# ActiveVisionLab/NeFeS

Hardware: AMD Instinct MI355X
Metric: rays/s (fwd+bwd) at 640x480x(64+128) samples, 8x256 MLP (higher is better)
Workload: dtype f32; 1 GPU; BASELINE configs[1]: 7-Scenes-stairs geometry, 64+128 samples, 8x256 MLP + 16-ch feature head; 640x480, random seed-0 weights, fwd + bwd to the 3x4 pose; parallelism=rows/1

## Files before the change

include/nefes_hip.h:

```cpp
#ifndef NEFES_HIP_H
#define NEFES_HIP_H
#include <stddef.h>
#include <stdint.h>

#ifdef __cplusplus
extern "C" {
#endif

#define NEFES_ABI_VERSION 15

#define NEFES_E_BADARG (-1)
#define NEFES_E_UNSUPPORTED (-2)
#define NEFES_E_BADBLOB (-3)

typedef struct NefesNetDesc {
    int32_t width;
    int32_t feat_dim;
    int32_t has_transient;
    int32_t xyz_encoding;
} NefesNetDesc;
#define NEFES_XYZ_FREQ10 0
#define NEFES_XYZ_EXTERNAL32 1

typedef struct NefesStreamInfo {
    uint64_t slab_off;
    uint32_t n_slabs;
    uint32_t bias_floats;
    uint64_t bias_off;
    uint32_t scale_off;
    uint32_t scale_count;
} NefesStreamInfo;

typedef struct NefesBlobInfo {
    uint64_t total_bytes;
    NefesStreamInfo stream[13];
} NefesBlobInfo;

#define NEFES_COMP_TRANSIENT 1u
#define NEFES_COMP_STATIC_ONLY 2u
#define NEFES_COMP_SIGMA_ONLY 4u
#define NEFES_COMP_WHITE_BKGD 8u
#define NEFES_COMP_FEAT_WEIGHTS_ONLY 16u

#define NEFES_FIELD_SIGMA 0
#define NEFES_FIELD_STATIC 1
#define NEFES_FIELD_FULL 2

int nefes_version(void);

int nefes_blob_info(const NefesNetDesc* desc, NefesBlobInfo* info);
size_t nefes_stream_slab_bytes(const NefesNetDesc* desc, int stream);
int nefes_pack_weights(const NefesNetDesc* desc, const float* const* tensors, int n_tensors, void* blob,
// ... 194 lines not shown
```

nefes_amd/csrc/field_bwd_h3.hip:

```cpp
#if defined(NEFES_TU_PART) && NEFES_TU_PART >= 2 && NEFES_TU_PART % 2 == 0
#define NEFES_SLAB_KIB 16
#define NEFES_ASM_READS_ACC
#define NEFES_ACC_VGPR_FORM
#define NEFES_FENCE_TILES
#else
#define NEFES_SLAB_KIB 32
#if !defined(NEFES_TU_PART) || NEFES_TU_PART == 0 || NEFES_TU_PART == 1 || NEFES_TU_PART == 5
#define H3B_WIDE
#define H3_ACC_READ_ASM
#define NEFES_ASM_READS_ACC
#define NEFES_FENCE_TILES
#define H3_WIDE_ENTRY_FENCE
#else
#define NEFES_H3_WIDE_MIN 99
#endif
#endif
#define NEFES_B_BATCH 2
#define NEFES_B_BATCH_NT8 4
#include "field_common.h"
#include "field_x6.h"
#include "field_h3.h"
#include "hashgrid.h"
#include "../../include/nefes_hip.h"
#define NEFES_XYZ_HASHGRID_FUSED 2
// ... 33 lines not shown
};

template <class Inner>
struct StoringSplitH {
    Inner in;
    float* p;
    float inv;
    __device__ __forceinline__ void stage_a(PairRegs& s, int q, int pp) const {
        in.stage_a(s, q, pp);
        const int e = 8 * q + 2 * pp;
#ifndef NEFES_TRAIN_NO_STORES
        __builtin_nontemporal_store(s.x0 * inv, &p[(e >> 4) * 4096 + nefes_rho(0, e & 15) * 16]);
        __builtin_nontemporal_store(s.x1 * inv, &p[((e + 1) >> 4) * 4096 + nefes_rho(0, (e + 1) & 15) * 16]);
#endif
    }
    __device__ __forceinline__ void stage_b(PairRegs& s) const { in.stage_b(s); }
    template <bool NOP>
    __device__ __forceinline__ void stage_c(Split2& o, int pp, const PairRegs& s) const { in.template stage_c<NOP>(o, pp, s); }
    __device__ __forceinline__ void stage_c1(Split2& o, int pp, const PairRegs& s) const { in.stage_c1(o, pp, s); }
    template <bool NOP>
    __device__ __forceinline__ void stage_c2(Split2& o, int pp, const PairRegs& s) const { in.template stage_c2<NOP>(o, pp, s); }
};
template <bool ON, class Inner>
__device__ __forceinline__ auto wrap_store_h3(const Inner& in, float* p, float inv) {
    if constexpr (ON) return StoringSplitH<Inner>{in, p, inv};
    else return in;
}

template <typename T>
__device__ __forceinline__ T ld_stream(const T* p) {
    return __builtin_nontemporal_load(p);
}

template <int W, int KR16, int ENC, bool HAS_T = true, bool TRAIN = false, bool FH = false>
__global__ __launch_bounds__(256, NEFES_H3B_WG_PER_CU(W)) void field_bwd_h3_kernel(FieldBwdH3Args a) {
    constexpr int NTW = W / 32, NTH = W / 64, HS = W / 2, GS = W / 4;
    constexpr int MW = 8 * (W / 64) + 4 * (W / 128);
    constexpr int WT = (NTW + 1) / 2, WH = (NTH + 1) / 2;
    constexpr int MW_TRUNK = 8 * WT;
    constexpr int NTR = KR16 <= 2 ? 1 : 5;
    constexpr int WIDE_LAYERS = ENC == NEFES_XYZ_HASHGRID_FUSED ? 0 : H3B_WIDE_LAYERS;
    static_assert(KR16 == 2 || KR16 == 9, "head classes of layout.h (nefes_head_kr16 / nefes_head_ntr)");
    const int C3 = 3 + a.C;
    static_assert(MW % 4 == 0, "mask words are staged as 16-byte groups");
    extern __shared__ __attribute__((aligned(16))) char smem[];
    const int lane = threadIdx.x & 63;
    const int wave = __builtin_amdgcn_readfirstlane(threadIdx.x >> 6);
    const int j = lane & 31, h = lane >> 5;
    constexpr int SX = ENC == NEFES_XYZ_HASHGRID_FUSED ? 24 : 8;
    int* tab_i = (int*)(smem + NEFES_H3B_SLOTS * NEFES_SLAB_BYTES + (size_t)4 * (MW + SX) * 256);
    const float* tab_f = (const float*)tab_i;
    if (threadIdx.x < 2 * (HAS_T ? NEFES_H3B_N : NEFES_H3B_N_STATIC)) tab_i[threadIdx.x] = a.tab[threadIdx.x];
    HgGeom* hg_lds = (HgGeom*)(tab_i + 64);
    if constexpr (ENC == NEFES_XYZ_HASHGRID_FUSED) {
        if (threadIdx.x == 0) *hg_lds = a.hg;
    }
    auto wexp = [&](int seg) { return tab_i[nefes_h3_tab_exp(nefes_h3b_seg(HAS_T, seg))]; };
    auto rowb = [&](int seg) { return tab_f[nefes_h3_tab_bound(nefes_h3b_seg(HAS_T, seg))]; };
    StagedRing ring;
    ring.init(a.stream, a.n_slabs, smem, wave, lane);
    const char* ring_lane = smem + lane * 16;
    ring.prime(ring_lane);
    uint32_t* mlds = (uint32_t*)(smem + NEFES_H3B_SLOTS * NEFES_SLAB_BYTES) + wave * ((MW + SX) * 64) + lane * 4;
    auto MASKW = [&](int w) { return mlds[(w >> 2) * 256 + (w & 3)]; };
    float* stash = (float*)mlds;
    auto STASH = [&](int k) -> float& { return stash[((MW + k) >> 2) * 256 + ((MW + k) & 3)]; };

#pragma unroll 1
    for (int tile = blockIdx.x; tile < a.n_tiles; tile += gridDim.x) {
        const long long m_raw = (long long)tile * 128 + wave * 32 + j;
        const bool valid = m_raw < a.M;
        const long long m = valid ? m_raw : a.M - 1;
        const int ray = (int)(m / a.S);
        const int smp = (int)(m - (long long)ray * a.S);
        const size_t chan0 = (size_t)ray * a.R * a.S + smp;

        float in_o[3] = {0.f, 0.f, 0.f}, in_d[3] = {0.f, 0.f, 0.f}, in_z = 0.f, v[3];
        if constexpr (ENC == NEFES_XYZ_EXTERNAL32) {
        } else if (a.pts) {
#pragma unroll
            for (int c = 0; c < 3; ++c) in_o[c] = a.pts[m * 3 + c];
        } else {
            in_z = a.z[m];
#pragma unroll
            for (int c = 0; c < 3; ++c) { in_o[c] = a.rays_o[ray * 3 + c]; in_d[c] = a.rays_d[ray * 3 + c]; }
        }
#pragma unroll
        for (int c = 0; c < 3; ++c) v[c] = a.viewdirs[ray * 3 + c];
        const int cT = C3 + 1;
        float y_th[3] = {0.f, 0.f, 0.f}, g_th[3] = {0.f, 0.f, 0.f}, y_sg, g_sg, dr[8 * KR16];
        if constexpr (HAS_T) {
// ... 123 lines not shown
            M_dg = pair_max(array_max(tmp));
        }
        int es_g2;
        {
            const int ew = wexp(NEFES_H3B_RGB), tau = tau_of(M_dr, ew);
            es_g2 = tau + ew;
            mma_run_h3<NTH, KR16, 0, true>(ring, ring_lane, ArraySplitH<8 * KR16>{dr, pow2i(tau)}, ZeroInit{}, G2);
        }
        const float M_g2 = rowb(NEFES_H3B_RGB) * M_dr + M_dg;
        float M = 0.f;
        int es3 = 0;
        if constexpr (HAS_T) {
        mma_run<NTH, 3, 0, true>(ring, ring_lane, ArrayIn<3>{dth}, ZeroInit{}, T3);
        M = rowb(NEFES_H3B_TH) * pair_max(array_max(dth));
        int es4;
        {
            load_bits(bh, MW_TRUNK + 3 * WH, WH);
            const int ew = wexp(NEFES_H3B_T2), tau = tau_of(M, ew);
            float mx = 0.f;
            es4 = tau + ew;
            mma_run_h3<NTH, GS / 8, 0, true>(ring, ring_lane, wrap_store_h3<TRAIN>(MaskedSplitH<NTH, WH, 0>{T3, bh, pow2i(tau), mx}, gptr(NEFES_TB_T2), 1.f), ZeroInit{}, T4);
            M = rowb(NEFES_H3B_T2) * pair_max(mx);
        }
        {
            load_bits(bh, MW_TRUNK + 2 * WH, WH);
            const int ew = wexp(NEFES_H3B_T1), tau = tau_of(M, ew);
            float mx = 0.f;
            es3 = tau + ew;
            mma_run_h3<NTH, GS / 8, 0, true>(ring, ring_lane, wrap_store_h3<TRAIN>(MaskedSplitH<NTH, WH, 0>{T4, bh, pow2i(tau - es4), mx}, gptr(NEFES_TB_T1), pow2i(-es4)), ZeroInit{}, T3);
            M = rowb(NEFES_H3B_T1) * (pair_max(mx) * pow2i(-es4));
        }
        }
        f32x16 XA[NTW + 2], XB[NTW + 2];
        int es_dt;
        {
            const int ew = wexp(NEFES_H3B_DIR);
            const int tau = tau_of(HAS_T ? fmaxf(M, M_g2) : M_g2, ew);
            float mt = 0.f, mg = 0.f;
            es_dt = tau + ew;
            float dgv[FH ? 16 * NTH : 1];
            load_dg(dgv);
            if constexpr (HAS_T) {
                load_bits(bh, MW_TRUNK + WH, WH);
                mma_run_h3<NTW + 1, GS / 8, 1, true>(ring, ring_lane, wrap_store_h3<TRAIN>(MaskedSplitH<NTH, WH, 0>{T3, bh, pow2i(tau - es3), mt}, gptr(NEFES_TB_T0), pow2i(-es3)), ZeroInit{}, XA);
            }
            load_bits(bh, MW_TRUNK, WH);
#ifdef NEFES_FH_VARIANT_VALU_UPDATE
            if constexpr (FH) {
#pragma unroll
                for (int e = 0; e < 16 * NTH; ++e) G2[e >> 4][e & 15] += dgv[e] * pow2i(es_g2);
                mma_run_h3<NTW + 1, GS / 8, 1, !HAS_T>(ring, ring_lane, MaskedSplitH<NTH, WH, 0>{G2, bh, pow2i(tau - es_g2), mg}, ZeroInit{}, XA);
            } else
#else
            if constexpr (FH)
                mma_run_h3<NTW + 1, GS / 8, 1, !HAS_T>(ring, ring_lane, MaskedAddSplitH<NTH, WH, 0, 16 * NTH>{G2, bh, pow2i(tau - es_g2), mg, dgv, pow2i(es_g2)}, ZeroInit{}, XA);
            else
#endif
            mma_run_h3<NTW + 1, GS / 8, 1, !HAS_T>(ring, ring_lane, wrap_store_h3<TRAIN>(MaskedSplitH<NTH, WH, 0>{G2, bh, pow2i(tau - es_g2), mg}, gptr(NEFES_TB_DIR), pow2i(-es_g2)), ZeroInit{}, XA);
            M = (HAS_T ? rowb(NEFES_H3B_T0) * (pair_max(mt) * pow2i(-es3)) : 0.f) + rowb(NEFES_H3B_DIR) * (pair_max(mg) * pow2i(-es_g2));
        }
        float gv[3];
        {
            float dDv[16], v3[3];
            const float inv = pow2i(-es_dt);
#pragma unroll
            for (int r = 0; r < 16; ++r) dDv[r] = XA[1][r] * inv;
#pragma unroll
            for (int c = 0; c < 3; ++c) v3[c] = STASH(3 + c);
            embed_slots_bwd<NEFES_N_FREQ_DIR>(gv, dDv, v3, h);
            if constexpr (ENC == NEFES_XYZ_HASHGRID_FUSED) {
#pragma unroll
                for (int c = 0; c < 3; ++c) STASH(3 + c) = gv[c];
            }
        }
        int es_b;
        {
            const int ew = wexp(NEFES_H3B_FINAL), tau = tau_of(M, ew);
            float mx = 0.f;
            es_b = tau + ew;
            mma_run_h3<NTW, W / 16, 2, true, 2, (WIDE_LAYERS & 1) != 0>(ring, ring_lane, wrap_store_h3<TRAIN>(IdentSplitH<NTW + 2, 2>{XA, pow2i(tau - es_dt), mx}, gptr(NEFES_TB_FINAL), pow2i(-es_dt)), ZeroInit{}, XB);
            const float dsig = STASH(6);
            float dsg[1];
            dsg[0] = dsig * pow2i(es_b);
#if defined(H3B_WIDE) && defined(H3_WIDE_ENTRY_FENCE)
            mma_run<NTW, 1, 2, false, ((WIDE_LAYERS >> 8) & 1) == 0 || (NTW < NEFES_H3_WIDE_MIN)>(ring, ring_lane, ArrayIn<1>{dsg}, ZeroInit{}, XB);
#else
            mma_run<NTW, 1, 2, false>(ring, ring_lane, ArrayIn<1>{dsg}, ZeroInit{}, XB);
#endif
            M = rowb(NEFES_H3B_FINAL) * (pair_max(mx) * pow2i(-es_dt)) + rowb(NEFES_H3B_SIG) * pair_max(fabsf(dsig));
        }
        int es_a = 0, es_e = 0;
#define NEFES_BWD_LAYER(L, SRC, DST, ES_SRC, ES_DST, NTILES, T0)                                                       \
        {                                                                                                           \
            load_bits(bt, ((L) - 1) * WT, WT);                                                                      \
            const int ew = wexp(NEFES_H3B_L8 + 8 - (L)), tau = tau_of(M, ew);                                       \
            float mx = 0.f;                                                                                         \
            ES_DST = tau + ew;                                                                                      \
            mma_run_h3<NTILES, W / 16, T0, true, 2, ((WIDE_LAYERS >> (L)) & 1) != 0>(ring, ring_lane, wrap_store_h3<TRAIN>(MaskedSplitH<NTW + 2, WT, 2>{SRC, bt, pow2i(tau - ES_SRC), mx}, gptr(NEFES_TB_L1 + (L) - 1), pow2i(-(ES_SRC))), ZeroInit{}, DST); \
            M = rowb(NEFES_H3B_L8 + 8 - (L)) * (pair_max(mx) * pow2i(-(ES_SRC)));                                   \
        }
        NEFES_BWD_LAYER(8, XB, XA, es_b, es_a, NTW, 2)
        NEFES_BWD_LAYER(7, XA, XB, es_a, es_b, NTW, 2)
        NEFES_BWD_LAYER(6, XB, XA, es_b, es_a, NTW, 2)
        NEFES_BWD_LAYER(5, XA, XB, es_a, es_b, NTW + 2, 0)
        es_e = es_b;
        float gx[3] = {0.f, 0.f, 0.f};
        float ge[ENC != NEFES_XYZ_FREQ10 ? NEFES_X_STEPS : 1];
        {
            const float inv = pow2i(-es_e);
// ... 42 lines not shown
                float* gp = a.g_enc + m * 32 + h;
#pragma unroll
                for (int s_ = 0; s_ < NEFES_X_STEPS; ++s_) gp[2 * s_] = ge[s_];
            }
        } else {
            float dE[32], x3[3], g1[3];
#pragma unroll
            for (int t = 0; t < 2; ++t)
#pragma unroll
                for (int r = 0; r < 16; ++r) dE[t * 16 + r] = XB[t][r] * inv1;
#pragma unroll
            for (int c = 0; c < 3; ++c) x3[c] = STASH(c);
            embed_slots_bwd<NEFES_N_FREQ_XYZ>(g1, dE, x3, h);
#pragma unroll
            for (int c = 0; c < 3; ++c) gx[c] += g1[c];
        }
#pragma unroll
        for (int c = 0; c < 3; ++c) {
            gx[c] += __shfl_xor(gx[c], 32);
            gv[c] += __shfl_xor(gv[c], 32);
        }
        if (valid && h == 0) {
#pragma unroll
            for (int c = 0; c < 3; ++c) {
                if (ENC != NEFES_XYZ_EXTERNAL32) a.g_pts[m * 3 + c] = gx[c];
                a.g_vs[m * 3 + c] = gv[c];
            }
        }
    }
    ring.drain();
}

template <int W, int KR16, int ENC, bool HAS_T = true, bool TRAIN = false, bool FH = false>
static int launch_bwd_h3(const FieldBwdH3Args& a, hipStream_t st) {
    const size_t lds = (size_t)NEFES_H3B_SLOTS * NEFES_SLAB_BYTES
                       + (size_t)4 * (8 * (W / 64) + 4 * (W / 128) + (ENC == NEFES_XYZ_HASHGRID_FUSED ? 24 : 8)) * 256 + 256
                       + (ENC == NEFES_XYZ_HASHGRID_FUSED ? 512 : 0);
    static_assert(sizeof(HgGeom) <= 512 && 2 * NEFES_H3B_N <= 64, "scale table (256 bytes) + the level geometry's LDS slot");
    auto k = field_bwd_h3_kernel<W, KR16, ENC, HAS_T, TRAIN, FH>;
    hipError_t e = hipFuncSetAttribute((const void*)k, hipFuncAttributeMaxDynamicSharedMemorySize, (int)lds);
    if (e != hipSuccess) return (int)e;
    int dev = 0, cus = 256;
    (void)hipGetDevice(&dev);
    (void)hipDeviceGetAttribute(&cus, hipDeviceAttributeMultiprocessorCount, dev);
    const int slots = cus * NEFES_H3B_WG_PER_CU(W);
    int grid = a.n_tiles < slots ? a.n_tiles : slots;
    if (grid < 1) grid = 1;
    hipLaunchKernelGGL(k, dim3(grid), dim3(256), lds, st, a);
    return (int)hipGetLastError();
}

#ifndef NEFES_TU_PART
#define NEFES_TU_PART 0
#endif
enum { BWD_H3_EXT = 0, BWD_H3_FULL, BWD_H3_TRAIN_STATIC, BWD_H3_TRAIN_FULL, BWD_H3_STATIC, BWD_H3_HG, BWD_H3_FH, BWD_H3_TRAIN_EXT_STATIC,
       BWD_H3_TRAIN_EXT_FULL };
int nefes_bwd_h3_launch_part1(int which, const FieldBwdH3Args& a, hipStream_t st);
int nefes_bwd_h3_launch_part2(int which, const FieldBwdH3Args& a, hipStream_t st);
int nefes_bwd_h3_launch_part3(int which, const FieldBwdH3Args& a, hipStream_t st);
int nefes_bwd_h3_launch_part4(int which, const FieldBwdH3Args& a, hipStream_t st);
int nefes_bwd_h3_launch_part5(int which, const FieldBwdH3Args& a, hipStream_t st);
int nefes_bwd_h3_launch_part6(int which, const FieldBwdH3Args& a, hipStream_t st);
int nefes_bwd_h3_launch_part7(int which, const FieldBwdH3Args& a, hipStream_t st);
int nefes_bwd_h3_launch_part8(int which, const FieldBwdH3Args& a, hipStream_t st);

#if NEFES_TU_PART == 1
int nefes_bwd_h3_launch_part1(int which, const FieldBwdH3Args& a, hipStream_t st) {
    if (which == BWD_H3_EXT) return launch_bwd_h3<256, 2, NEFES_XYZ_EXTERNAL32>(a, st);
    if (which == BWD_H3_STATIC) return launch_bwd_h3<256, 2, NEFES_XYZ_FREQ10, false>(a, st);
    if (which == BWD_H3_HG) return launch_bwd_h3<256, 2, NEFES_XYZ_HASHGRID_FUSED>(a, st);
    return NEFES_E_UNSUPPORTED;
}
#elif NEFES_TU_PART == 2
int nefes_bwd_h3_launch_part2(int which, const FieldBwdH3Args& a, hipStream_t st) {
    if (which == BWD_H3_FULL) return launch_bwd_h3<128, 9, NEFES_XYZ_FREQ10>(a, st);
    if (which == BWD_H3_STATIC) return launch_bwd_h3<128, 9, NEFES_XYZ_FREQ10, false>(a, st);
    return NEFES_E_UNSUPPORTED;
}
#elif NEFES_TU_PART == 3
int nefes_bwd_h3_launch_part3(int which, const FieldBwdH3Args& a, hipStream_t st) {
    if (which == BWD_H3_TRAIN_STATIC) return launch_bwd_h3<256, 2, NEFES_XYZ_FREQ10, false, true>(a, st);
    if (which == BWD_H3_TRAIN_FULL) return launch_bwd_h3<256, 2, NEFES_XYZ_FREQ10, true, true>(a, st);
    if (which == BWD_H3_TRAIN_EXT_STATIC) return launch_bwd_h3<256, 2, NEFES_XYZ_EXTERNAL32, false, true>(a, st);
    if (which == BWD_H3_TRAIN_EXT_FULL) return launch_bwd_h3<256, 2, NEFES_XYZ_EXTERNAL32, true, true>(a, st);
    return NEFES_E_UNSUPPORTED;
}
#elif NEFES_TU_PART == 4
int nefes_bwd_h3_launch_part4(int which, const FieldBwdH3Args& a, hipStream_t st) {
    if (which == BWD_H3_TRAIN_STATIC) return launch_bwd_h3<128, 9, NEFES_XYZ_FREQ10, false, true>(a, st);
    if (which == BWD_H3_TRAIN_FULL) return launch_bwd_h3<128, 9, NEFES_XYZ_FREQ10, true, true>(a, st);
    return NEFES_E_UNSUPPORTED;
}
#elif NEFES_TU_PART == 5
int nefes_bwd_h3_launch_part5(int which, const FieldBwdH3Args& a, hipStream_t st) {
    if (which == BWD_H3_FULL) return launch_bwd_h3<256, 9, NEFES_XYZ_FREQ10>(a, st);
    if (which == BWD_H3_STATIC) return launch_bwd_h3<256, 9, NEFES_XYZ_FREQ10, false>(a, st);
    return NEFES_E_UNSUPPORTED;
}
#elif NEFES_TU_PART == 6
int nefes_bwd_h3_launch_part6(int which, const FieldBwdH3Args& a, hipStream_t st) {
    if (which == BWD_H3_FULL) return launch_bwd_h3<128, 2, NEFES_XYZ_FREQ10>(a, st);
    if (which == BWD_H3_STATIC) return launch_bwd_h3<128, 2, NEFES_XYZ_FREQ10, false>(a, st);
    if (which == BWD_H3_FH) return launch_bwd_h3<128, 2, NEFES_XYZ_FREQ10, true, false, true>(a, st);
    return NEFES_E_UNSUPPORTED;
}
#elif NEFES_TU_PART == 7
int nefes_bwd_h3_launch_part7(int which, const FieldBwdH3Args& a, hipStream_t st) {
    if (which == BWD_H3_TRAIN_STATIC) return launch_bwd_h3<256, 9, NEFES_XYZ_FREQ10, false, true>(a, st);
    if (which == BWD_H3_TRAIN_FULL) return launch_bwd_h3<256, 9, NEFES_XYZ_FREQ10, true, true>(a, st);
    return NEFES_E_UNSUPPORTED;
}
#elif NEFES_TU_PART == 8
int nefes_bwd_h3_launch_part8(int which, const FieldBwdH3Args& a, hipStream_t st) {
    if (which == BWD_H3_TRAIN_STATIC) return launch_bwd_h3<128, 2, NEFES_XYZ_FREQ10, false, true>(a, st);
    if (which == BWD_H3_TRAIN_FULL) return launch_bwd_h3<128, 2, NEFES_XYZ_FREQ10, true, true>(a, st);
    return NEFES_E_UNSUPPORTED;
}
#else

extern "C" int nefes_field_bwd_train_h3(const NefesNetDesc* desc, const void* packed, int mode, int N, int S, const float* rays_o,
                                        const float* rays_d, const float* z, const float* viewdirs, const float* raw_t,
                                        const float* g_raw_t, const uint32_t* masks, float* dacts, float* g_pts,
                                        float* g_viewdirs_s, void* stream) {
    if (!desc || !packed || !viewdirs || !raw_t || !g_raw_t || !masks || !dacts || !g_pts || !g_viewdirs_s || N <= 0 || S <= 0)
        return NEFES_E_BADARG;
    if (!(rays_o && rays_d && z)) return NEFES_E_BADARG;
    if (mode != NEFES_FIELD_STATIC && mode != NEFES_FIELD_FULL) return NEFES_E_BADARG;
    const bool full = mode == NEFES_FIELD_FULL;
    if (full && !desc->has_transient) return NEFES_E_UNSUPPORTED;
    const int cls = nefes_head_class(desc->feat_dim);
    if ((desc->width != 256 && desc->width != 128) || cls < 0 || desc->xyz_encoding != NEFES_XYZ_FREQ10) return NEFES_E_UNSUPPORTED;
    NefesBlobInfo info;
    int rc = nefes_blob_info(desc, &info);
    if (rc) return rc;
    const NefesStreamInfo& si = info.stream[full ? NEFES_STREAM_BWD_FULL_H3 : NEFES_STREAM_BWD_STATIC_H3];
    if (si.n_slabs == 0 || si.scale_count < 2 * (uint32_t)(full ? NEFES_H3B_N : NEFES_H3B_N_STATIC)) return NEFES_E_UNSUPPORTED;
    FieldBwdH3Args a;
    a.stream = (const char*)packed + si.slab_off;
    a.tab = (const int*)((const char*)packed + si.bias_off) + si.scale_off;
    a.n_slabs = si.n_slabs;
    a.rays_o = rays_o; a.rays_d = rays_d; a.z = z; a.pts = nullptr; a.viewdirs = viewdirs;
    a.raw_t = raw_t; a.g_raw_t = g_raw_t; a.masks = masks; a.g_pts = g_pts; a.g_enc = nullptr; a.g_vs = g_viewdirs_s;
    a.N = N; a.S = S; a.C = desc->feat_dim; a.R = 3 + a.C + (full ? 6 : 1);
    a.M = (long long)N * S;
    a.n_tiles = (int)((a.M + 127) / 128);
    a.dacts = dacts; a.gout = 0; a.hg_table = nullptr; a.g_gmap = nullptr;
    a.rows = nefes_train_row(desc->width, desc->feat_dim, NEFES_TB_END);
    const int which = full ? BWD_H3_TRAIN_FULL : BWD_H3_TRAIN_STATIC;
    hipStream_t st = (hipStream_t)stream;
    if (desc->width == 256) return cls == 0 ? nefes_bwd_h3_launch_part3(which, a, st) : nefes_bwd_h3_launch_part7(which, a, st);
    return cls == 1 ? nefes_bwd_h3_launch_part4(which, a, st) : nefes_bwd_h3_launch_part8(which, a, st);
}

extern "C" int nefes_field_bwd_train_h3_ext(const NefesNetDesc* desc, const void* packed, int mode, int N, int S, const float* viewdirs,
                                            const float* raw_t, const float* g_raw_t, const uint32_t* masks, float* dacts,
                                            float* g_xyz_enc, float* g_viewdirs_s, void* stream) {
    if (!desc || !packed || !viewdirs || !raw_t || !g_raw_t || !masks || !dacts || !g_xyz_enc || !g_viewdirs_s || N <= 0 || S <= 0)
        return NEFES_E_BADARG;
    if (mode != NEFES_FIELD_STATIC && mode != NEFES_FIELD_FULL) return NEFES_E_BADARG;
    const bool full = mode == NEFES_FIELD_FULL;
    if (full && !desc->has_transient) return NEFES_E_UNSUPPORTED;
    if (desc->width != 256 || nefes_head_class(desc->feat_dim) != 0 || desc->xyz_encoding != NEFES_XYZ_EXTERNAL32) return NEFES_E_UNSUPPORTED;
    NefesBlobInfo info;
    int rc = nefes_blob_info(desc, &info);
    if (rc) return rc;
    const NefesStreamInfo& si = info.stream[full ? NEFES_STREAM_BWD_FULL_H3 : NEFES_STREAM_BWD_STATIC_H3];
    if (si.n_slabs == 0 || si.scale_count < 2 * (uint32_t)(full ? NEFES_H3B_N : NEFES_H3B_N_STATIC)) return NEFES_E_UNSUPPORTED;
    FieldBwdH3Args a;
    a.stream = (const char*)packed + si.slab_off;
    a.tab = (const int*)((const char*)packed + si.bias_off) + si.scale_off;
    a.n_slabs = si.n_slabs;
    a.rays_o = nullptr; a.rays_d = nullptr; a.z = nullptr; a.pts = nullptr; a.viewdirs = viewdirs;
    a.raw_t = raw_t; a.g_raw_t = g_raw_t; a.masks = masks; a.g_pts = nullptr; a.g_enc = g_xyz_enc; a.g_vs = g_viewdirs_s;
    a.N = N; a.S = S; a.C = desc->feat_dim; a.R = 3 + a.C + (full ? 6 : 1);
    a.M = (long long)N * S;
    a.n_tiles = (int)((a.M + 127) / 128);
    a.dacts = dacts; a.gout = 0; a.hg_table = nullptr; a.g_gmap = nullptr;
    a.rows = nefes_train_row(desc->width, desc->feat_dim, NEFES_TB_END);
    return nefes_bwd_h3_launch_part3(full ? BWD_H3_TRAIN_EXT_FULL : BWD_H3_TRAIN_EXT_STATIC, a, (hipStream_t)stream);
}

extern "C" int nefes_field_bwd_static_h3(const NefesNetDesc* desc, const void* packed, int N, int S, const float* rays_o,
                                         const float* rays_d, const float* z, const float* pts, const float* viewdirs,
                                         const float* raw_t, const float* g_raw_t, const uint32_t* masks, float* g_pts,
                                         float* g_viewdirs_s, void* stream) {
    if (!desc || !packed || !viewdirs || !raw_t || !g_raw_t || !masks || !g_pts || !g_viewdirs_s || N <= 0 || S <= 0)
        return NEFES_E_BADARG;
    if (!pts && !(rays_o && rays_d && z)) return NEFES_E_BADARG;
    const int cls = nefes_head_class(desc->feat_dim);
    if ((desc->width != 256 && desc->width != 128) || cls < 0 || desc->xyz_encoding != NEFES_XYZ_FREQ10) return NEFES_E_UNSUPPORTED;
    NefesBlobInfo info;
    int rc = nefes_blob_info(desc, &info);
    if (rc) return rc;
    const NefesStreamInfo& si = info.stream[NEFES_STREAM_BWD_STATIC_H3];
    if (si.n_slabs == 0 || si.scale_count < 2 * (uint32_t)NEFES_H3B_N_STATIC) return NEFES_E_UNSUPPORTED;
    FieldBwdH3Args a;
    a.stream = (const char*)packed + si.slab_off;
    a.tab = (const int*)((const char*)packed + si.bias_off) + si.scale_off;
    a.n_slabs = si.n_slabs;
    a.rays_o = rays_o; a.rays_d = rays_d; a.z = z; a.pts = pts; a.viewdirs = viewdirs;
    a.raw_t = raw_t; a.g_raw_t = g_raw_t; a.masks = masks; a.g_pts = g_pts; a.g_enc = nullptr; a.g_vs = g_viewdirs_s;
    a.N = N; a.S = S; a.C = desc->feat_dim; a.R = 3 + a.C + 1;
    a.M = (long long)N * S;
    a.n_tiles = (int)((a.M + 127) / 128);
    a.dacts = nullptr; a.rows = 0; a.gout = 0; a.hg_table = nullptr; a.g_gmap = nullptr;
    hipStream_t st = (hipStream_t)stream;
    if (desc->width == 256) return cls == 0 ? nefes_bwd_h3_launch_part1(BWD_H3_STATIC, a, st) : nefes_bwd_h3_launch_part5(BWD_H3_STATIC, a, st);
    return cls == 1 ? nefes_bwd_h3_launch_part2(BWD_H3_STATIC, a, st) : nefes_bwd_h3_launch_part6(BWD_H3_STATIC, a, st);
}

static int field_bwd_h3_impl(const NefesNetDesc* desc, const void* packed, int N, int S, const float* rays_o,
                                  const float* rays_d, const float* z, const float* pts, const float* viewdirs,
                                  const float* raw_t, const float* g_raw_t, const uint32_t* masks, float* g_pts,
                                  float* g_xyz_enc, float* g_viewdirs_s, void* stream, const NefesHashGridDesc* grid, const float* table,
                                  bool fh = false, const float* g_gmap = nullptr) {
    if (!desc || !packed || !viewdirs || !raw_t || !g_raw_t || !masks || !g_viewdirs_s || N <= 0 || S <= 0)
        return NEFES_E_BADARG;
    const bool ext = desc->xyz_encoding == NEFES_XYZ_EXTERNAL32;
    const bool fused_grid = ext && table != nullptr;
    if (fused_grid ? !(g_pts && grid && rays_o && rays_d && z) : (ext ? !g_xyz_enc : (!g_pts || (!pts && !(rays_o && rays_d && z))))) return NEFES_E_BADARG;
    if (!desc->has_transient) return NEFES_E_UNSUPPORTED;
    NefesBlobInfo info;
    int rc = nefes_blob_info(desc, &info);
    if (rc) return rc;
    const NefesStreamInfo& si = info.stream[NEFES_STREAM_BWD_FULL_H3];
    if (si.n_slabs == 0 || si.scale_count < 2 * NEFES_H3B_N) return NEFES_E_UNSUPPORTED;
    FieldBwdH3Args a;
    a.stream = (const char*)packed + si.slab_off;
    a.tab = (const int*)((const char*)packed + si.bias_off) + si.scale_off;
    a.n_slabs = si.n_slabs;
    a.rays_o = rays_o; a.rays_d = rays_d; a.z = z; a.pts = pts; a.viewdirs = viewdirs;
    a.raw_t = raw_t; a.g_raw_t = g_raw_t; a.masks = masks; a.g_pts = g_pts; a.g_enc = g_xyz_enc; a.g_vs = g_viewdirs_s;
    a.N = N; a.S = S; a.C = desc->feat_dim; a.R = 3 + a.C + 6;
    a.gout = 0; a.g_gmap = g_gmap;
    if (fh) {
        if (desc->feat_dim != 0 || desc->width != 128 || ext) return NEFES_E_UNSUPPORTED;
        a.gout = desc->width / 2;
        a.C = a.gout + 1;
        a.R = 3 + a.C + 6;
    }
    a.M = (long long)N * S;
    a.n_tiles = (int)((a.M + 127) / 128);
    a.dacts = nullptr; a.rows = 0;
    a.hg_table = (const float2*)table;
    if (fused_grid) {
        rc = hg_geometry(grid, &a.hg, nullptr);
        if (rc) return rc;
        if (a.hg.n_levels != 16) return NEFES_E_UNSUPPORTED;
    }
    hipStream_t st = (hipStream_t)stream;
    const int cls = nefes_head_class(desc->feat_dim);
    if (cls < 0) return NEFES_E_UNSUPPORTED;
    if (fh) return nefes_bwd_h3_launch_part6(BWD_H3_FH, a, st);
    if (desc->width == 256 && fused_grid) return cls == 0 ? nefes_bwd_h3_launch_part1(BWD_H3_HG, a, st) : NEFES_E_UNSUPPORTED;
    if (desc->width == 256 && ext) return cls == 0 ? nefes_bwd_h3_launch_part1(BWD_H3_EXT, a, st) : NEFES_E_UNSUPPORTED;
    if (desc->width == 256) return cls == 0 ? launch_bwd_h3<256, 2, NEFES_XYZ_FREQ10>(a, st) : nefes_bwd_h3_launch_part5(BWD_H3_FULL, a, st);
    if (desc->width == 128 && !ext) return cls == 1 ? nefes_bwd_h3_launch_part2(BWD_H3_FULL, a, st) : nefes_bwd_h3_launch_part6(BWD_H3_FULL, a, st);
    return NEFES_E_UNSUPPORTED;
}

extern "C" int nefes_field_bwd_h3(const NefesNetDesc* desc, const void* packed, int N, int S, const float* rays_o,
                                  const float* rays_d, const float* z, const float* pts, const float* viewdirs,
                                  const float* raw_t, const float* g_raw_t, const uint32_t* masks, float* g_pts,
                                  float* g_xyz_enc, float* g_viewdirs_s, void* stream) {
    return field_bwd_h3_impl(desc, packed, N, S, rays_o, rays_d, z, pts, viewdirs, raw_t, g_raw_t, masks, g_pts, g_xyz_enc, g_viewdirs_s, stream,
                             nullptr, nullptr);
}

extern "C" int nefes_field_bwd_h3_fh(const NefesNetDesc* desc, const void* packed, int N, int S, const float* rays_o, const float* rays_d,
                                     const float* z, const float* viewdirs, const float* raw_t, const float* g_raw_t, const float* g_gmap,
                                     const uint32_t* masks, float* g_pts, float* g_viewdirs_s, void* stream) {
    if (!rays_o || !rays_d || !z) return NEFES_E_BADARG;
    return field_bwd_h3_impl(desc, packed, N, S, rays_o, rays_d, z, nullptr, viewdirs, raw_t, g_raw_t, masks, g_pts, nullptr, g_viewdirs_s, stream,
                             nullptr, nullptr, true, g_gmap);
}

extern "C" int nefes_field_bwd_h3_hashgrid(const NefesNetDesc* desc, const void* packed, const NefesHashGridDesc* grid,
                                           const float* table, int N, int S, const float* rays_o, const float* rays_d, const float* z,
                                           const float* viewdirs, const float* raw_t, const float* g_raw_t, const uint32_t* masks,
                                           float* g_pts, float* g_viewdirs_s, void* stream) {
    if (!desc || desc->xyz_encoding != NEFES_XYZ_EXTERNAL32 || !grid || !table) return NEFES_E_BADARG;
    return field_bwd_h3_impl(desc, packed, N, S, rays_o, rays_d, z, nullptr, viewdirs, raw_t, g_raw_t, masks, g_pts, nullptr, g_viewdirs_s, stream,
                             grid, table);
}
#endif
```

nefes_amd/csrc/field_fwd_h3.hip:

```cpp
#if defined(NEFES_TU_PART) && NEFES_TU_PART >= 2 && NEFES_TU_PART % 2 == 0
#define NEFES_TU_W128
#define NEFES_SLAB_KIB 16
#else
#define NEFES_SLAB_KIB 32
#endif
#include <stdlib.h>
#if defined(NEFES_TU_W128) || !defined(H3_NO_ACC_READ_ASM)
#define NEFES_ASM_READS_ACC
#define NEFES_FENCE_TILES
#endif
#if defined(NEFES_TU_W128)
#define NEFES_ACC_VGPR_FORM
#endif

#ifndef NEFES_FWD_CONSUMER_BIAS
#define NEFES_FWD_CONSUMER_BIAS 1
#endif
#include "field_common.h"
#include "../../include/nefes_hip.h"

#include "field_x6.h"
#include "hashgrid.h"
#define NEFES_XYZ_HASHGRID_FUSED 2
#if !defined(NEFES_TU_W128) && !defined(H3_NO_ACC_READ_ASM)
// ... 9 lines not shown
    const float* rays_o;
    const float* rays_d;
    const float* z;
    const float* pts;
    const float* xyz_enc;
    const float* viewdirs;
    float* raw_t;
    uint32_t* masks;
    int N, S, R, C;
    long long M;
    int n_tiles;
    uint32_t s_magic, s_shift;
    float* acts;
    int rows;
    int z_row;
    const float2* hg_table;
    HgGeom hg;
    int gout;
};

template <int NT, int T0, int NX>
__device__ __forceinline__ void train_save_h3(float* tile_base, uint32_t voff, int row0, const f32x16 (&X)[NX], float inv) {
    float* p = tile_base + (size_t)(row0 >> 5) * 4096 + voff;
#pragma unroll
    for (int t = 0; t < NT; ++t)
#pragma unroll
        for (int r = 0; r < 16; ++r) {
#ifndef NEFES_TRAIN_NO_STORES
            __builtin_nontemporal_store(X[T0 + t][r] * inv, &p[t * 4096 + nefes_rho(0, r) * 16]);
#endif
        }
}

template <int MODE, int ENC, int W = 256, int NTR = 1, bool TRAIN = false, bool FH = false>
__global__ __launch_bounds__(256, W == 128 ? 2 : 1) void field_fwd_h3_kernel(FieldFwdH3Args a) {
    static_assert(NEFES_SLAB_KIB == (W == 128 ? NEFES_H3_FWD_SLAB_KIB_128 : NEFES_H3_FWD_SLAB_KIB), "ring slab size != the packer's for this width");
    constexpr int NTW = W / 32, NTH = W / 64;
    constexpr int ES = ENC != NEFES_XYZ_FREQ10 ? NEFES_X_STEPS : NEFES_E_STEPS;
    constexpr int MW = 8 * (W / 64) + 4 * (W / 128), WT = (NTW + 1) / 2, WH = (NTH + 1) / 2;
    constexpr int NSEG = MODE == NEFES_FIELD_SIGMA ? NEFES_H3F_SIG + 1 : (MODE == NEFES_FIELD_STATIC ? NEFES_H3F_N_STATIC : NEFES_H3F_N);
    extern __shared__ __attribute__((aligned(16))) char smem[];
    char* ring_base = smem;
    float* bias_lds = (float*)(smem + NEFES_H3_SLOTS * NEFES_SLAB_BYTES);
    float* e_lds = bias_lds + ((a.bias_floats + 63) / 64) * 64 + (threadIdx.x >> 6) * (ES * 64) + (threadIdx.x & 63);
    const int lane = threadIdx.x & 63;
    const int wave = __builtin_amdgcn_readfirstlane(threadIdx.x >> 6);
    const int j = lane & 31, h = lane >> 5;
    for (uint32_t i = threadIdx.x; i < a.bias_floats; i += 256) bias_lds[i] = a.bias[i];
    HgGeom* hg_lds = (HgGeom*)(bias_lds + ((a.bias_floats + 63) / 64) * 64 + 4 * ES * 64);
    if constexpr (ENC == NEFES_XYZ_HASHGRID_FUSED) {
        if (threadIdx.x == 0) *hg_lds = a.hg;
    }
    StagedRing ring;
    ring.init(a.stream, a.n_slabs, ring_base, wave, lane);
    const char* ring_lane = ring_base + lane * 16;
    const char* bias_half = (const char*)bias_lds + 16 * h;
    const int* tab_i = (const int*)(bias_lds + a.scale_off);
    const float* tab_f = bias_lds + a.scale_off;
    auto wexp = [&](int seg) { return tab_i[nefes_h3_tab_exp(seg)]; };
    auto rowb = [&](int seg) { return tab_f[nefes_h3_tab_bound(seg)]; };
    auto bmax = [&](int blk) { return tab_f[nefes_h3_tab_bias(NSEG, blk)]; };
    ring.prime(ring_lane);
    constexpr int B_SIG = 8 * W, B_FINAL = B_SIG + 32, B_DIR = B_FINAL + W, B_RGB = B_DIR + W / 2,
                  B_T0 = B_RGB + 32 * NTR, B_T1 = B_T0 + W / 2, B_T2 = B_T1 + W / 2, B_TH = B_T2 + W / 2;
#pragma unroll 1
    for (int tile = blockIdx.x; tile < a.n_tiles; tile += gridDim.x) {
        auto locate = [&](uint32_t& m, uint32_t& ray, uint32_t& smp) {
            const uint32_t m_raw = (uint32_t)tile * 128u + (uint32_t)(wave * 32 + j);
            const bool ok = m_raw < (uint32_t)a.M;
            m = ok ? m_raw : (uint32_t)a.M - 1u;
            ray = a.s_magic ? __umulhi(m, a.s_magic) >> a.s_shift : m;
            smp = m - ray * (uint32_t)a.S;
            return ok;
        };
        uint32_t m, ray, smp;
        locate(m, ray, smp);
        float in_o[3] = {0.f, 0.f, 0.f}, in_d[3] = {0.f, 0.f, 0.f}, in_z = 0.f;
        float E[ES];
        if constexpr (ENC == NEFES_XYZ_EXTERNAL32) {
#pragma unroll
            for (int s = 0; s < ES; ++s) E[s] = a.xyz_enc[(size_t)m * 32 + 2 * s + h];
        } else if (ENC != NEFES_XYZ_HASHGRID_FUSED && a.pts) {
#pragma unroll
            for (int c = 0; c < 3; ++c) in_o[c] = a.pts[(size_t)m * 3 + c];
        } else {
            in_z = a.z[a.z_row ? smp : m];
#pragma unroll
            for (int c = 0; c < 3; ++c) { in_o[c] = a.rays_o[ray * 3 + c]; in_d[c] = a.rays_d[ray * 3 + c]; }
        }
        float mE;
        if constexpr (ENC == NEFES_XYZ_EXTERNAL32) {
            mE = pair_max(array_max(E));
        } else if constexpr (ENC == NEFES_XYZ_HASHGRID_FUSED) {
            float x[3];
#pragma unroll
            for (int c = 0; c < 3; ++c) x[c] = add_rn(in_o[c], mul_rn(in_d[c], in_z));
// ... 63 lines not shown
                const int ch = (MODE == NEFES_FIELD_SIGMA) ? 0 : 3 + a.C;
                __builtin_nontemporal_store(softplus_ref(sg[0][0] * pow2i(-es)), &col[(size_t)ch * a.S]);
            }
        };
        int es_a, es_b = 0;
        float M;
        {
            const int tau = tau_of(mE, wexp(NEFES_H3F_L1));
            es_a = tau + wexp(NEFES_H3F_L1);
            if constexpr (CB) mma_run_h3<NTW, ES / 8, 0, true>(ring, ring_lane, LdsSplitH{e_lds, pow2i(tau)}, ZeroInit{}, A);
            else mma_run_h3<NTW, ES / 8, 0, true>(ring, ring_lane, LdsSplitH{e_lds, pow2i(tau)}, bias_at(0, es_a), A);
            M = rowb(NEFES_H3F_L1) * mE + bmax(NEFES_H3BB_L1);
            save_trunk(1, A, es_a);
        }
#define NEFES_FWD_EVEN_LAYER(L1_, SEG1_)                                                                                       \
        clear_bits();                                                                                                          \
        {                                                                                                                      \
            const int ew = wexp(SEG1_), tau = tau_of(M, ew);                                                                   \
            const float rb_ = rowb(SEG1_), bm_ = bmax((L1_) - 1);           \
            float mx = 0.f;                                                                                                    \
            if constexpr (CB) {                                                                                                \
                const char* bps = bias_half + ((L1_) - 2) * W * 4;                           \
                nbias = ReluBiasSplitH<CAP, NTW, WT>::prime(bps);                                                              \
                mma_run_h3<NTW, W / 16, 0, true>(ring, ring_lane, ReluBiasSplitH<CAP, NTW, WT>{A, bits, pow2i(tau - es_a), mx, bps, pow2i(es_a), nbias}, \
                                                 ZeroInit{}, B);                                                               \
            } else                                                                                                             \
            mma_run_h3<NTW, W / 16, 0, true>(ring, ring_lane, ReluSplitH<CAP, NTW, WT>{A, bits, pow2i(tau - es_a), mx},        \
                                             bias_at(((L1_) - 1) * W, tau + ew), B);                                           \
            M = rb_ * (pair_max(mx) * pow2i(-es_a)) + bm_;                                                                     \
            es_b = tau + ew;                                                                                                   \
            save_trunk(L1_, B, es_b);                                                                                          \
        }                                                                                                                      \
        put_masks(bits, WT);
        constexpr int NPAIRS = MODE == NEFES_FIELD_SIGMA ? 3 : 4;
#pragma unroll 1
        for (int p = 0; p < NPAIRS; ++p) {
            const int l1 = 2 + 2 * p, l2 = l1 + 1;
            const int seg1 = l1 <= 5 ? l1 - 1 : l1;
            const int seg2 = l2 <= 5 ? l2 - 1 : (l2 <= 8 ? l2 : NEFES_H3F_FINAL);
            NEFES_FWD_EVEN_LAYER(l1, seg1)
            clear_bits();
            {
                const int ew = wexp(seg2);
                const int tau = tau_of(p == 1 ? fmaxf(M, mE) : M, ew);
                if (p == 3) sigma_head(B, es_b, tau_of(M, wexp(NEFES_H3F_SIG)));
                const float rb_ = rowb(seg2), bm_ = bmax(l2 <= 8 ? l2 - 1 : NEFES_H3BB_FINAL);
                const float rbe_ = p == 1 ? rowb(NEFES_H3F_L5E) : 0.f;
                float mx = 0.f;
                if constexpr (CB) {
                    const char* bps = bias_half + (l1 - 1) * W * 4;
                    nbias = ReluBiasSplitH<CAP, NTW, WT>::prime(bps);
                    const ReluBiasSplitH<CAP, NTW, WT> src{B, bits, pow2i(tau - es_b), mx, bps, pow2i(es_b), nbias};
                    mma_run_h3<NTW, W / 16, 0, true>(ring, ring_lane, src, ZeroInit{}, A);
                } else
                mma_run_h3<NTW, W / 16, 0, true>(ring, ring_lane, ReluSplitH<CAP, NTW, WT>{B, bits, pow2i(tau - es_b), mx},
                                                 bias_at(l2 <= 8 ? (l2 - 1) * W : B_FINAL, tau + ew), A);
                if (p == 1) mma_run_h3<NTW, ES / 8, 0, false>(ring, ring_lane, LdsSplitH{e_lds, pow2i(tau)}, ZeroInit{}, A);
                M = rb_ * (pair_max(mx) * pow2i(-es_b)) + (p == 1 ? rbe_ * mE : 0.f) + bm_;
                es_a = tau + ew;
                save_trunk(l2, A, es_a);
            }
            put_masks(bits, WT);
        }
        if constexpr (MODE == NEFES_FIELD_SIGMA) { NEFES_FWD_EVEN_LAYER(8, NEFES_H3F_L8) }
#undef NEFES_FWD_EVEN_LAYER
        if constexpr (MODE == NEFES_FIELD_SIGMA) sigma_head(B, es_b, tau_of(M, wexp(NEFES_H3F_SIG)));
        if constexpr (MODE != NEFES_FIELD_SIGMA) {
            constexpr bool FULL = MODE == NEFES_FIELD_FULL;
            constexpr int NDT = FULL ? 2 * NTH : NTH;
            float v[3];
            {
                uint32_t mm, rr, ss;
                locate(mm, rr, ss);
#pragma unroll
                for (int c = 0; c < 3; ++c) v[c] = a.viewdirs[(size_t)rr * 3 + c];
            }
            float Dv[16];
            {
                float d14[NEFES_D_STEPS];
                embed_slots<NEFES_N_FREQ_DIR>(d14, v, h);
#pragma unroll
                for (int s = 0; s < 16; ++s) Dv[s] = s < NEFES_D_STEPS ? d14[s] : 0.f;
            }
            if constexpr (TRAIN) {
                float* pd = act_tile + (size_t)(nefes_train_row(W, 0, NEFES_TB_DV) >> 5) * 4096 + emb_off;
#pragma unroll
                for (int s = 0; s < NEFES_D_STEPS; ++s) __builtin_nontemporal_store(Dv[s], &pd[2 * s * 16]);
            }
            f32x16 dt[NDT];
            uint32_t bits2[WH];
            auto clear2 = [&]() {
#pragma unroll
                for (int w = 0; w < WH; ++w) bits2[w] = 0u;
            };
            struct Bias2 {
                BiasInitScaled a, b;
                __device__ __forceinline__ f32x16 operator()(int t) const { return t < NTH ? a(t) : b(t - NTH); }
            };
            int es_dt;
            {
                const int ew = wexp(NEFES_H3F_DT_H);
                const float mD = pair_max(array_max(Dv));
                const int tau = tau_of(fmaxf(M, mD), ew);
                float mx = 0.f;
                es_dt = tau + ew;
                if constexpr (CB) {
                    const char* bpf = bias_half + B_FINAL * 4;
                    nbias = ReluBiasSplitH<false, 1, 1>::prime(bpf);
                    const IdentBiasSplitH<NTW> srcf{A, pow2i(tau - es_a), mx, bpf, pow2i(es_a), nbias};
                    if constexpr (FULL) mma_run_h3<NDT, W / 16, 0, true>(ring, ring_lane, srcf, Bias2{bias_at(B_DIR, es_dt), bias_at(B_T0, es_dt)}, dt);
                    else mma_run_h3<NDT, W / 16, 0, true>(ring, ring_lane, srcf, bias_at(B_DIR, es_dt), dt);
                } else if constexpr (FULL)
                    mma_run_h3<NDT, W / 16, 0, true>(ring, ring_lane, IdentSplitH<NTW, 0>{A, pow2i(tau - es_a), mx},
                                                     Bias2{bias_at(B_DIR, es_dt), bias_at(B_T0, es_dt)}, dt);
                else
                    mma_run_h3<NDT, W / 16, 0, true>(ring, ring_lane, IdentSplitH<NTW, 0>{A, pow2i(tau - es_a), mx}, bias_at(B_DIR, es_dt), dt);
                mma_run_h3<NDT, 2, 0, false>(ring, ring_lane, ArraySplitH<16>{Dv, pow2i(tau)}, ZeroInit{}, dt);
                M = rowb(NEFES_H3F_DT_H) * (pair_max(mx) * pow2i(-es_a)) + rowb(NEFES_H3F_DT_D) * mD
                    + (FULL ? fmaxf(bmax(NEFES_H3BB_DIR), bmax(NEFES_H3BB_T0)) : bmax(NEFES_H3BB_DIR));
                if constexpr (TRAIN) {
                    train_save_h3<NTH, 0>(act_tile, act_voff, nefes_train_row(W, 0, NEFES_TB_DIR), dt, pow2i(-es_dt));
                    if constexpr (FULL) train_save_h3<NTH, NTH>(act_tile, act_voff, nefes_train_row(W, 0, NEFES_TB_T0), dt, pow2i(-es_dt));
                }
            }
            if constexpr (FH) {
                float* col = raw_col();
                if (col) {
                    int S_g = a.S;
                    asm volatile("" : "+s"(S_g));
                    const float inv = pow2i(-es_dt);
                    float* pg = col + (size_t)(3 + 4 * h) * S_g;
#pragma unroll
                    for (int t = 0; t < NTH; ++t)
#pragma unroll
                        for (int r = 0; r < 16; ++r)
                            __builtin_nontemporal_store(fmaxf(dt[t][r] * inv, 0.f), &pg[(size_t)(32 * t + nefes_rho(0, r)) * S_g]);
                    if (h == 0) __builtin_nontemporal_store(1.f, &col[(size_t)(3 + W / 2) * S_g]);
                }
            }
            {
                f32x16 ar[NTR];
                clear2();
                const int ew = wexp(NEFES_H3F_RGB), tau = tau_of(M, ew), es = tau + ew;
                float mdummy = 0.f;
                mma_run_h3<NTR, W / 32, 0, true>(ring, ring_lane, ReluSplitH<true, NDT, WH>{dt, bits2, pow2i(tau - es_dt), mdummy},
                                                 bias_at(B_RGB, es), ar);
                put_masks(bits2, WH);
                float* col = raw_col();
                if (col) {
                    float* ph = col + (size_t)(4 * h) * a.S;
                    const float inv = pow2i(-es);
// ... 39 lines not shown
                                                 bias_at(B_T2, es2), acc2);
                M = rowb(NEFES_H3F_T2) * (pair_max(mx) * pow2i(-es3)) + bmax(NEFES_H3BB_T2);
                if constexpr (TRAIN) train_save_h3<NTH, 0>(act_tile, act_voff, nefes_train_row(W, 0, NEFES_TB_T2), acc2, pow2i(-es2));
            }
            put_masks(bits2, WH);
            f32x16 th[1];
            clear2();
            {
                const int ew = wexp(NEFES_H3F_TH), tau = tau_of(M, ew);
                float mdummy = 0.f;
                es_th = tau + ew;
                mma_run_h3<1, W / 32, 0, true>(ring, ring_lane, ReluSplitH<true, NTH, WH>{acc2, bits2, pow2i(tau - es2), mdummy},
                                               bias_at(B_TH, es_th), th);
            }
            put_masks(bits2, WH);
            float* col = raw_col();
            if (col) {
                float* o = col + (size_t)(3 + a.C + 1) * a.S;
                const float inv = pow2i(-es_th);
                if (h == 0) {
                    __builtin_nontemporal_store(sigmoid_ref(th[0][0] * inv), &o[0]);
                    __builtin_nontemporal_store(sigmoid_ref(th[0][1] * inv), &o[(size_t)a.S]);
                    __builtin_nontemporal_store(sigmoid_ref(th[0][2] * inv), &o[(size_t)2 * a.S]);
                    __builtin_nontemporal_store(softplus_ref(th[0][3] * inv), &o[(size_t)3 * a.S]);
                } else {
                    __builtin_nontemporal_store(softplus_ref(th[0][0] * inv), &o[(size_t)4 * a.S]);
                }
            }
            }
        }
    }
}

static void magic_div(uint32_t d, uint32_t& magic, uint32_t& shift) {
    if (d == 1) { magic = 0; shift = 0; return; }
    uint32_t l = 0;
    while ((1ull << l) < d) ++l;
    const uint64_t p = 31 + l;
    magic = (uint32_t)(((1ull << p) + d - 1) / d);
    shift = (uint32_t)(p - 32);
}

template <int MODE, int ENC, int W = 256, int NTR = 1, bool TRAIN = false, bool FH = false>
static int launch_h3(const FieldFwdH3Args& a, hipStream_t st) {
    constexpr int ES_ = ENC != NEFES_XYZ_FREQ10 ? NEFES_X_STEPS : NEFES_E_STEPS;
    const size_t lds = (size_t)NEFES_H3_SLOTS * NEFES_SLAB_BYTES + ((a.bias_floats + 63) / 64) * 256 + (size_t)4 * ES_ * 64 * 4
                       + (ENC == NEFES_XYZ_HASHGRID_FUSED ? 512 : 0);
    static_assert(sizeof(HgGeom) <= 512, "the level geometry's LDS slot");
    auto k = field_fwd_h3_kernel<MODE, ENC, W, NTR, TRAIN, FH>;
    hipError_t e = hipFuncSetAttribute((const void*)k, hipFuncAttributeMaxDynamicSharedMemorySize, (int)lds);
    if (e != hipSuccess) return (int)e;
    int dev = 0, cus = 256;
    (void)hipGetDevice(&dev);
    (void)hipDeviceGetAttribute(&cus, hipDeviceAttributeMultiprocessorCount, dev);
    const int per_cu = W == 128 ? 2 : 1;
    int grid = a.n_tiles < cus * per_cu ? a.n_tiles : cus * per_cu;
    if (const char* cap = getenv("NEFES_DEBUG_MAX_GRID")) {
        const int c = atoi(cap);
        if (c > 0 && c < grid) grid = c;
    }
    hipLaunchKernelGGL(k, dim3(grid), dim3(256), lds, st, a);
    return (int)hipGetLastError();
}

#ifndef NEFES_TU_PART
#define NEFES_TU_PART 0
#endif
enum { H3_EXT_SIGMA = 0, H3_EXT_FULL, H3_SIGMA, H3_FULL, H3_TRAIN_STATIC, H3_TRAIN_FULL, H3_STATIC, H3_HG_SIGMA, H3_HG_FULL, H3_FH_FULL,
       H3_TRAIN_EXT_STATIC, H3_TRAIN_EXT_FULL };
int nefes_fwd_h3_launch_part1(int which, const FieldFwdH3Args& a, hipStream_t st);
int nefes_fwd_h3_launch_part2(int which, const FieldFwdH3Args& a, hipStream_t st);
int nefes_fwd_h3_launch_part3(int which, const FieldFwdH3Args& a, hipStream_t st);
int nefes_fwd_h3_launch_part4(int which, const FieldFwdH3Args& a, hipStream_t st);
int nefes_fwd_h3_launch_part5(int which, const FieldFwdH3Args& a, hipStream_t st);
int nefes_fwd_h3_launch_part6(int which, const FieldFwdH3Args& a, hipStream_t st);
int nefes_fwd_h3_launch_part7(int which, const FieldFwdH3Args& a, hipStream_t st);
int nefes_fwd_h3_launch_part8(int which, const FieldFwdH3Args& a, hipStream_t st);


#if NEFES_TU_PART == 1
int nefes_fwd_h3_launch_part1(int which, const FieldFwdH3Args& a, hipStream_t st) {
    switch (which) {
        case H3_EXT_SIGMA: return launch_h3<NEFES_FIELD_SIGMA, NEFES_XYZ_EXTERNAL32>(a, st);
        case H3_EXT_FULL: return launch_h3<NEFES_FIELD_FULL, NEFES_XYZ_EXTERNAL32>(a, st);
        case H3_STATIC: return launch_h3<NEFES_FIELD_STATIC, NEFES_XYZ_FREQ10, 256, 1>(a, st);
        case H3_HG_SIGMA: return launch_h3<NEFES_FIELD_SIGMA, NEFES_XYZ_HASHGRID_FUSED>(a, st);
        case H3_HG_FULL: return launch_h3<NEFES_FIELD_FULL, NEFES_XYZ_HASHGRID_FUSED>(a, st);
    }
    return NEFES_E_UNSUPPORTED;
}
#elif NEFES_TU_PART == 2
int nefes_fwd_h3_launch_part2(int which, const FieldFwdH3Args& a, hipStream_t st) {
    switch (which) {
        case H3_SIGMA: return launch_h3<NEFES_FIELD_SIGMA, NEFES_XYZ_FREQ10, 128, 5>(a, st);
        case H3_FULL: return launch_h3<NEFES_FIELD_FULL, NEFES_XYZ_FREQ10, 128, 5>(a, st);
        case H3_STATIC: return launch_h3<NEFES_FIELD_STATIC, NEFES_XYZ_FREQ10, 128, 5>(a, st);
    }
    return NEFES_E_UNSUPPORTED;
}
#elif NEFES_TU_PART == 3
int nefes_fwd_h3_launch_part3(int which, const FieldFwdH3Args& a, hipStream_t st) {
    switch (which) {
        case H3_TRAIN_STATIC: return launch_h3<NEFES_FIELD_STATIC, NEFES_XYZ_FREQ10, 256, 1, true>(a, st);
        case H3_TRAIN_FULL: return launch_h3<NEFES_FIELD_FULL, NEFES_XYZ_FREQ10, 256, 1, true>(a, st);
        case H3_TRAIN_EXT_STATIC: return launch_h3<NEFES_FIELD_STATIC, NEFES_XYZ_EXTERNAL32, 256, 1, true>(a, st);
        case H3_TRAIN_EXT_FULL: return launch_h3<NEFES_FIELD_FULL, NEFES_XYZ_EXTERNAL32, 256, 1, true>(a, st);
    }
    return NEFES_E_UNSUPPORTED;
}
#elif NEFES_TU_PART == 4
int nefes_fwd_h3_launch_part4(int which, const FieldFwdH3Args& a, hipStream_t st) {
    switch (which) {
        case H3_TRAIN_STATIC: return launch_h3<NEFES_FIELD_STATIC, NEFES_XYZ_FREQ10, 128, 5, true>(a, st);
        case H3_TRAIN_FULL: return launch_h3<NEFES_FIELD_FULL, NEFES_XYZ_FREQ10, 128, 5, true>(a, st);
    }
    return NEFES_E_UNSUPPORTED;
}
#elif NEFES_TU_PART == 5
int nefes_fwd_h3_launch_part5(int which, const FieldFwdH3Args& a, hipStream_t st) {
    if (which == H3_FULL) return launch_h3<NEFES_FIELD_FULL, NEFES_XYZ_FREQ10, 256, 5>(a, st);
    if (which == H3_STATIC) return launch_h3<NEFES_FIELD_STATIC, NEFES_XYZ_FREQ10, 256, 5>(a, st);
    return NEFES_E_UNSUPPORTED;
}
#elif NEFES_TU_PART == 6
int nefes_fwd_h3_launch_part6(int which, const FieldFwdH3Args& a, hipStream_t st) {
    if (which == H3_FULL) return launch_h3<NEFES_FIELD_FULL, NEFES_XYZ_FREQ10, 128, 1>(a, st);
    if (which == H3_STATIC) return launch_h3<NEFES_FIELD_STATIC, NEFES_XYZ_FREQ10, 128, 1>(a, st);
    if (which == H3_FH_FULL) return launch_h3<NEFES_FIELD_FULL, NEFES_XYZ_FREQ10, 128, 1, false, true>(a, st);
    return NEFES_E_UNSUPPORTED;
}
#elif NEFES_TU_PART == 7
int nefes_fwd_h3_launch_part7(int which, const FieldFwdH3Args& a, hipStream_t st) {
    switch (which) {
        case H3_TRAIN_STATIC: return launch_h3<NEFES_FIELD_STATIC, NEFES_XYZ_FREQ10, 256, 5, true>(a, st);
        case H3_TRAIN_FULL: return launch_h3<NEFES_FIELD_FULL, NEFES_XYZ_FREQ10, 256, 5, true>(a, st);
    }
    return NEFES_E_UNSUPPORTED;
}
#elif NEFES_TU_PART == 8
int nefes_fwd_h3_launch_part8(int which, const FieldFwdH3Args& a, hipStream_t st) {
    switch (which) {
        case H3_TRAIN_STATIC: return launch_h3<NEFES_FIELD_STATIC, NEFES_XYZ_FREQ10, 128, 1, true>(a, st);
        case H3_TRAIN_FULL: return launch_h3<NEFES_FIELD_FULL, NEFES_XYZ_FREQ10, 128, 1, true>(a, st);
    }
    return NEFES_E_UNSUPPORTED;
}
#else

extern "C" int nefes_field_fwd_train_h3(const NefesNetDesc* desc, const void* packed, int mode, int N, int S, const float* rays_o,
                                        const float* rays_d, const float* z, const float* pts, const float* viewdirs,
                                        float* raw_t, float* acts, uint32_t* masks, void* stream) {
    if (!desc || !packed || !raw_t || !acts || !viewdirs || N <= 0 || S <= 0) return NEFES_E_BADARG;
    if (!pts && !(rays_o && rays_d && z)) return NEFES_E_BADARG;
    if (mode != NEFES_FIELD_STATIC && mode != NEFES_FIELD_FULL) return NEFES_E_UNSUPPORTED;
    if (mode == NEFES_FIELD_FULL && !desc->has_transient) return NEFES_E_BADARG;
    const int cls = nefes_head_class(desc->feat_dim);
    if ((desc->width != 256 && desc->width != 128) || cls < 0 || desc->xyz_encoding != NEFES_XYZ_FREQ10) return NEFES_E_UNSUPPORTED;
    NefesBlobInfo info;
    int rc = nefes_blob_info(desc, &info);
    if (rc) return rc;
    const NefesStreamInfo& si = info.stream[mode == NEFES_FIELD_STATIC ? NEFES_STREAM_FWD_STATIC_H3 : NEFES_STREAM_FWD_FULL_H3];
    if (si.n_slabs == 0) return NEFES_E_UNSUPPORTED;
    FieldFwdH3Args a;
    a.stream = (const char*)packed + si.slab_off;
    a.bias = (const float*)((const char*)packed + si.bias_off);
    a.n_slabs = si.n_slabs; a.bias_floats = si.bias_floats; a.scale_off = si.scale_off;
    a.rays_o = rays_o; a.rays_d = rays_d; a.z = z; a.pts = pts; a.xyz_enc = nullptr; a.viewdirs = viewdirs; a.raw_t = raw_t; a.masks = masks;
    a.N = N; a.S = S; a.C = desc->feat_dim; a.R = 3 + a.C + (mode == NEFES_FIELD_STATIC ? 1 : 6);
    a.M = (long long)N * S;
    if (a.M >= (1ll << 31) - 256) return NEFES_E_UNSUPPORTED;
    a.n_tiles = (int)((a.M + 127) / 128);
    a.acts = acts;
    a.rows = nefes_train_row(desc->width, desc->feat_dim, NEFES_TB_END);
    a.z_row = 0; a.gout = 0; a.hg_table = nullptr;
    magic_div((uint32_t)S, a.s_magic, a.s_shift);
    const int which = mode == NEFES_FIELD_STATIC ? H3_TRAIN_STATIC : H3_TRAIN_FULL;
    hipStream_t st = (hipStream_t)stream;
    if (desc->width == 256) return cls == 0 ? nefes_fwd_h3_launch_part3(which, a, st) : nefes_fwd_h3_launch_part7(which, a, st);
    return cls == 1 ? nefes_fwd_h3_launch_part4(which, a, st) : nefes_fwd_h3_launch_part8(which, a, st);
}

extern "C" int nefes_field_fwd_train_h3_ext(const NefesNetDesc* desc, const void* packed, int mode, int N, int S, const float* xyz_enc,
                                            const float* viewdirs, float* raw_t, float* acts, uint32_t* masks, void* stream) {
    if (!desc || !packed || !xyz_enc || !raw_t || !acts || !viewdirs || N <= 0 || S <= 0) return NEFES_E_BADARG;
    if (mode != NEFES_FIELD_STATIC && mode != NEFES_FIELD_FULL) return NEFES_E_UNSUPPORTED;
    if (mode == NEFES_FIELD_FULL && !desc->has_transient) return NEFES_E_BADARG;
    if (desc->width != 256 || nefes_head_class(desc->feat_dim) != 0 || desc->xyz_encoding != NEFES_XYZ_EXTERNAL32) return NEFES_E_UNSUPPORTED;
    NefesBlobInfo info;
    int rc = nefes_blob_info(desc, &info);
    if (rc) return rc;
    const NefesStreamInfo& si = info.stream[mode == NEFES_FIELD_STATIC ? NEFES_STREAM_FWD_STATIC_H3 : NEFES_STREAM_FWD_FULL_H3];
    if (si.n_slabs == 0) return NEFES_E_UNSUPPORTED;
    FieldFwdH3Args a;
    a.stream = (const char*)packed + si.slab_off;
    a.bias = (const float*)((const char*)packed + si.bias_off);
    a.n_slabs = si.n_slabs; a.bias_floats = si.bias_floats; a.scale_off = si.scale_off;
    a.rays_o = nullptr; a.rays_d = nullptr; a.z = nullptr; a.pts = nullptr; a.xyz_enc = xyz_enc; a.viewdirs = viewdirs; a.raw_t = raw_t;
    a.masks = masks;
    a.N = N; a.S = S; a.C = desc->feat_dim; a.R = 3 + a.C + (mode == NEFES_FIELD_STATIC ? 1 : 6);
    a.M = (long long)N * S;
    if (a.M >= (1ll << 31) - 256) return NEFES_E_UNSUPPORTED;
    a.n_tiles = (int)((a.M + 127) / 128);
    a.acts = acts;
    a.rows = nefes_train_row(desc->width, desc->feat_dim, NEFES_TB_END);
    a.z_row = 0; a.gout = 0; a.hg_table = nullptr;
    magic_div((uint32_t)S, a.s_magic, a.s_shift);
    return nefes_fwd_h3_launch_part3(mode == NEFES_FIELD_STATIC ? H3_TRAIN_EXT_STATIC : H3_TRAIN_EXT_FULL, a, (hipStream_t)stream);
}

static int field_fwd_h3_impl(const NefesNetDesc* desc, const void* packed, int mode, int N, int S, const float* rays_o,
                             const float* rays_d, const float* z, int z_row, const float* pts, const float* xyz_enc,
                             const float* viewdirs, float* raw_t, uint32_t* masks, void* stream,
                             const NefesHashGridDesc* grid = nullptr, const float* table = nullptr, bool fh = false) {
    if (!desc || !packed || !raw_t || N <= 0 || S <= 0) return NEFES_E_BADARG;
    const bool ext = desc->xyz_encoding == NEFES_XYZ_EXTERNAL32;
    const bool fused_grid = ext && table != nullptr;
    if (fused_grid ? !(rays_o && rays_d && z && grid) : (ext ? !xyz_enc : (!pts && !(rays_o && rays_d && z)))) return NEFES_E_BADARG;
    if (mode != NEFES_FIELD_SIGMA && mode != NEFES_FIELD_FULL && mode != NEFES_FIELD_STATIC) return NEFES_E_UNSUPPORTED;
// ... 3 lines not shown
    const bool big = desc->width == 256, small = desc->width == 128 && !ext;
    if (!(big || small) || cls < 0 || (ext && cls != 0) || (desc->xyz_encoding != NEFES_XYZ_FREQ10 && !ext)) return NEFES_E_UNSUPPORTED;
    NefesBlobInfo info;
    int rc = nefes_blob_info(desc, &info);
    if (rc) return rc;
    const NefesStreamInfo& si = info.stream[mode == NEFES_FIELD_SIGMA ? NEFES_STREAM_FWD_SIGMA_H3
                                            : (mode == NEFES_FIELD_STATIC ? NEFES_STREAM_FWD_STATIC_H3 : NEFES_STREAM_FWD_FULL_H3)];
    if (si.n_slabs == 0) return NEFES_E_UNSUPPORTED;
    FieldFwdH3Args a;
    a.stream = (const char*)packed + si.slab_off;
    a.bias = (const float*)((const char*)packed + si.bias_off);
    a.n_slabs = si.n_slabs; a.bias_floats = si.bias_floats; a.scale_off = si.scale_off;
    a.rays_o = rays_o; a.rays_d = rays_d; a.z = z; a.pts = pts; a.xyz_enc = xyz_enc; a.viewdirs = viewdirs; a.raw_t = raw_t; a.masks = masks;
    a.acts = nullptr; a.rows = 0; a.z_row = z_row;
    a.hg_table = (const float2*)table;
    if (fused_grid) {
        rc = hg_geometry(grid, &a.hg, nullptr);
        if (rc) return rc;
        if (a.hg.n_levels != 16) return NEFES_E_UNSUPPORTED;
    }
    a.N = N; a.S = S; a.C = desc->feat_dim; a.R = mode == NEFES_FIELD_SIGMA ? 1 : 3 + a.C + (mode == NEFES_FIELD_STATIC ? 1 : 6);
    a.gout = 0;
    if (fh) {
        if (desc->feat_dim != 0 || desc->width != 128 || ext || mode != NEFES_FIELD_FULL) return NEFES_E_UNSUPPORTED;
        a.gout = desc->width / 2;
        a.C = a.gout + 1;
        a.R = 3 + a.C + 6;
    }
    a.M = (long long)N * S;
    if (a.M >= (1ll << 31) - 256) return NEFES_E_UNSUPPORTED;
    a.n_tiles = (int)((a.M + 127) / 128);
    magic_div((uint32_t)S, a.s_magic, a.s_shift);
    hipStream_t st = (hipStream_t)stream;
    if (fh) return nefes_fwd_h3_launch_part6(H3_FH_FULL, a, st);
    if (mode == NEFES_FIELD_STATIC) {
        if (big) return cls == 0 ? nefes_fwd_h3_launch_part1(H3_STATIC, a, st) : nefes_fwd_h3_launch_part5(H3_STATIC, a, st);
        return cls == 1 ? nefes_fwd_h3_launch_part2(H3_STATIC, a, st) : nefes_fwd_h3_launch_part6(H3_STATIC, a, st);
    }
    if (fused_grid) return nefes_fwd_h3_launch_part1(mode == NEFES_FIELD_SIGMA ? H3_HG_SIGMA : H3_HG_FULL, a, st);
    if (ext) return nefes_fwd_h3_launch_part1(mode == NEFES_FIELD_SIGMA ? H3_EXT_SIGMA : H3_EXT_FULL, a, st);
    if (small) {
        if (mode == NEFES_FIELD_SIGMA) return nefes_fwd_h3_launch_part2(H3_SIGMA, a, st);
        return cls == 1 ? nefes_fwd_h3_launch_part2(H3_FULL, a, st) : nefes_fwd_h3_launch_part6(H3_FULL, a, st);
    }
    if (mode == NEFES_FIELD_SIGMA) return launch_h3<NEFES_FIELD_SIGMA, NEFES_XYZ_FREQ10>(a, st);
    return cls == 0 ? launch_h3<NEFES_FIELD_FULL, NEFES_XYZ_FREQ10>(a, st) : nefes_fwd_h3_launch_part5(H3_FULL, a, st);
}

extern "C" int nefes_field_fwd_h3(const NefesNetDesc* desc, const void* packed, int mode, int N, int S, const float* rays_o,
                                  const float* rays_d, const float* z, const float* pts, const float* xyz_enc,
                                  const float* viewdirs, float* raw_t, uint32_t* masks, void* stream) {
    return field_fwd_h3_impl(desc, packed, mode, N, S, rays_o, rays_d, z, 0, pts, xyz_enc, viewdirs, raw_t, masks, stream);
}

extern "C" int nefes_field_fwd_h3_hashgrid(const NefesNetDesc* desc, const void* packed, const NefesHashGridDesc* grid,
                                           const float* table, int mode, int N, int S, const float* rays_o, const float* rays_d,
                                           const float* z, int z_is_row, const float* viewdirs, float* raw_t, uint32_t* masks,
                                           void* stream) {
    if (!desc || desc->xyz_encoding != NEFES_XYZ_EXTERNAL32 || !grid || !table) return NEFES_E_BADARG;
    return field_fwd_h3_impl(desc, packed, mode, N, S, rays_o, rays_d, z, z_is_row ? 1 : 0, nullptr, nullptr, viewdirs, raw_t, masks, stream,
                             grid, table);
}

extern "C" int nefes_field_fwd_h3_fh(const NefesNetDesc* desc, const void* packed, int mode, int N, int S, const float* rays_o,
                                     const float* rays_d, const float* z, const float* viewdirs, float* raw_t, uint32_t* masks,
                                     void* stream) {
    if (!rays_o || !rays_d || !z) return NEFES_E_BADARG;
    return field_fwd_h3_impl(desc, packed, mode, N, S, rays_o, rays_d, z, 0, nullptr, nullptr, viewdirs, raw_t, masks, stream, nullptr, nullptr, true);
}

extern "C" int nefes_field_fwd_h3_zrow(const NefesNetDesc* desc, const void* packed, int mode, int N, int S, const float* rays_o,
                                       const float* rays_d, const float* z_row, const float* viewdirs, float* raw_t, uint32_t* masks,
                                       void* stream) {
    if (!rays_o || !rays_d || !z_row) return NEFES_E_BADARG;
    if (desc && desc->xyz_encoding != NEFES_XYZ_FREQ10) return NEFES_E_UNSUPPORTED;
    return field_fwd_h3_impl(desc, packed, mode, N, S, rays_o, rays_d, z_row, 1, nullptr, nullptr, viewdirs, raw_t, masks, stream);
}
#endif
```

nefes_amd/csrc/layout.h:

```cpp
#pragma once
#include <stdint.h>

#if defined(__HIP__)
#define NEFES_HD __host__ __device__ inline __attribute__((always_inline))
#else
#define NEFES_HD inline
#endif

#ifndef NEFES_FWD_SLAB_KIB
#define NEFES_FWD_SLAB_KIB 32
#endif
#ifndef NEFES_BWD_SLAB_KIB
#define NEFES_BWD_SLAB_KIB 32
#endif
#define NEFES_FRAGS_OF_KIB(kib) ((kib) * 4)
#define NEFES_SLAB_BYTES (NEFES_SLAB_KIB * 1024)
#define NEFES_SLAB_FRAGS NEFES_FRAGS_OF_KIB(NEFES_SLAB_KIB)
#define NEFES_SLAB_PIECES (NEFES_SLAB_BYTES / 4096)
#define NEFES_RING_SLOTS (128 / NEFES_FWD_SLAB_KIB)
#define NEFES_BWD_SLOTS (96 / NEFES_BWD_SLAB_KIB)
#define NEFES_N_FREQ_XYZ 10
#define NEFES_N_FREQ_DIR 4
#define NEFES_E_STEPS 32
#define NEFES_D_STEPS 14
// ... 23 lines not shown
       NEFES_STREAM_FWD_SIGMA_X6 = 4, NEFES_STREAM_FWD_FULL_X6 = 5, NEFES_STREAM_BWD_FULL_X6 = 6, NEFES_STREAM_BWD_STATIC = 7,
       NEFES_STREAM_FWD_SIGMA_H3 = 8, NEFES_STREAM_FWD_FULL_H3 = 9, NEFES_STREAM_BWD_FULL_H3 = 10,
       NEFES_STREAM_FWD_STATIC_H3 = 11, NEFES_STREAM_BWD_STATIC_H3 = 12,
       NEFES_N_STREAMS = 13 };
#define NEFES_X6_SLAB_KIB 48
#define NEFES_H3_FWD_SLAB_KIB 32
#define NEFES_H3_FWD_SLAB_KIB_128 16
#define NEFES_H3_BWD_SLAB_KIB 32
#define NEFES_H3_BWD_SLAB_KIB_128 16
#define NEFES_H3_TARGET_EXP 14
NEFES_HD int nefes_stream_slab_kib(int stream, int width) {
    if (stream == NEFES_STREAM_BWD_FULL || stream == NEFES_STREAM_BWD_FULL_X6 || stream == NEFES_STREAM_BWD_STATIC) return NEFES_BWD_SLAB_KIB;
    if (stream == NEFES_STREAM_BWD_FULL_H3 || stream == NEFES_STREAM_BWD_STATIC_H3) return width == 128 ? NEFES_H3_BWD_SLAB_KIB_128 : NEFES_H3_BWD_SLAB_KIB;
    if (stream == NEFES_STREAM_FWD_SIGMA_H3 || stream == NEFES_STREAM_FWD_FULL_H3 || stream == NEFES_STREAM_FWD_STATIC_H3)
        return width == 128 ? NEFES_H3_FWD_SLAB_KIB_128 : NEFES_H3_FWD_SLAB_KIB;
    return stream >= NEFES_STREAM_FWD_SIGMA_X6 ? NEFES_X6_SLAB_KIB : NEFES_FWD_SLAB_KIB;
}
#define NEFES_PACK_KEEP 0xffffffffu
#define NEFES_BLOB_HEADER_BYTES 512

enum { NEFES_H3F_L1 = 0, NEFES_H3F_L2, NEFES_H3F_L3, NEFES_H3F_L4, NEFES_H3F_L5H, NEFES_H3F_L5E, NEFES_H3F_L6, NEFES_H3F_L7,
       NEFES_H3F_L8, NEFES_H3F_SIG, NEFES_H3F_FINAL, NEFES_H3F_DT_H, NEFES_H3F_DT_D, NEFES_H3F_RGB, NEFES_H3F_T1, NEFES_H3F_T2,
       NEFES_H3F_TH, NEFES_H3F_N };
NEFES_HD int nefes_h3_tab_exp(int seg) { return 2 * seg; }
NEFES_HD int nefes_h3_tab_bound(int seg) { return 2 * seg + 1; }
NEFES_HD int nefes_h3_tab_bias(int n_segs, int block) { return 2 * n_segs + block; }
enum { NEFES_H3BB_L1 = 0, NEFES_H3BB_SIG = 8, NEFES_H3BB_FINAL, NEFES_H3BB_DIR, NEFES_H3BB_RGB, NEFES_H3BB_T0, NEFES_H3BB_T1,
       NEFES_H3BB_T2, NEFES_H3BB_TH };
enum { NEFES_H3B_RGB = 0, NEFES_H3B_TH, NEFES_H3B_T2, NEFES_H3B_T1, NEFES_H3B_T0, NEFES_H3B_DIR, NEFES_H3B_FINAL, NEFES_H3B_SIG,
       NEFES_H3B_L8, NEFES_H3B_L7, NEFES_H3B_L6, NEFES_H3B_L5, NEFES_H3B_L4, NEFES_H3B_L3, NEFES_H3B_L2, NEFES_H3B_L1,
       NEFES_H3B_N };
#define NEFES_H3F_N_STATIC (NEFES_H3F_RGB + 1)
#define NEFES_H3B_N_STATIC (NEFES_H3B_N - 4)
NEFES_HD int nefes_h3b_seg(int has_transient, int seg) { return (has_transient || seg == NEFES_H3B_RGB) ? seg : seg - 4; }

NEFES_HD int nefes_mask_words(int W) { return 8 * (W / 64) + 4 * (W / 128); }

enum { NEFES_TB_E = 0, NEFES_TB_DV = 1, NEFES_TB_L1 = 2 , NEFES_TB_FINAL = 10, NEFES_TB_DIR = 11,
       NEFES_TB_T0 = 12, NEFES_TB_T1 = 13, NEFES_TB_T2 = 14, NEFES_TB_RGB = 15, NEFES_TB_SIG = 16, NEFES_TB_TH = 17,
       NEFES_TB_END = 18 };
NEFES_HD size_t nefes_train_off(int row, int sample) {
    return ((size_t)(row >> 5) * 8 + (size_t)(sample >> 4)) * 512 + (size_t)(row & 31) * 16 + (size_t)(sample & 15);
}
NEFES_HD uint32_t nefes_train_lane_off(int wave, int j, int h) { return (uint32_t)(((wave * 32 + j) >> 4) * 512 + 4 * h * 16 + (j & 15)); }
NEFES_HD int nefes_train_row(int W, int C, int block) {
    const int ntr = nefes_head_ntr(C);
    int r = 0;
    if (block == NEFES_TB_E) return r;
    r += 2 * NEFES_E_STEPS;
    if (block == NEFES_TB_DV) return r;
    r += 32;
    if (block >= NEFES_TB_L1 && block <= NEFES_TB_FINAL) return r + (block - NEFES_TB_L1) * W;
    r += 9 * W;
    if (block >= NEFES_TB_DIR && block <= NEFES_TB_T2) return r + (block - NEFES_TB_DIR) * (W / 2);
    r += 4 * (W / 2);
    if (block == NEFES_TB_RGB) return r;
    r += 32 * ntr;
    if (block == NEFES_TB_SIG) return r;
    r += 32;
    if (block == NEFES_TB_TH) return r;
    return r + 32;
}
```

nefes_amd/csrc/pack.cpp:

```cpp
#include <math.h>
#include <string.h>

#include <vector>

#include "../../include/nefes_hip.h"
#include "layout.h"

namespace {

enum { L_XYZ1 = 0, L_FINAL = 8, L_DIR = 9, L_SIGMA = 10, L_RGB = 11, L_T0 = 12, L_T1 = 13, L_T2 = 14, L_TSIGMA = 15,
       L_TRGB = 16, L_TBETA = 17 };

struct Seg {
    int nt = 0, ks = 0;
    std::vector<int> kidx;
    std::vector<int> ridx;
    const float* W = nullptr;
    int ld = 0;
    bool transposed = false;
    bool x6 = false;
    bool h3 = false;
    int wexp = 0;
    float at(int s, int t, int lane) const {
        const int i = lane & 31, h = lane >> 5;
// ... 120 lines not shown
    return k;
}
std::vector<int> k_emb(int L, int ks, int base) {
    std::vector<int> k(ks * 2);
    for (int s = 0; s < ks; ++s)
        for (int h = 0; h < 2; ++h) {
            const int e = nefes_emb_slot(L, s, h);
            k[s * 2 + h] = e < 0 ? -1 : base + e;
        }
    return k;
}
std::vector<int> k_compact(int ks, int limit) {
    std::vector<int> k(ks * 2);
    for (int i = 0; i < ks * 2; ++i) k[i] = i < limit ? i : -1;
    return k;
}
std::vector<int> rows_emb(int L, int ntiles, int base) {
    std::vector<int> r(ntiles * 32);
    for (int t = 0; t < ntiles; ++t)
        for (int i = 0; i < 32; ++i) {
            const int e = nefes_emb_slot(L, 16 * t + nefes_row_reg(i), nefes_row_half(i));
            r[t * 32 + i] = e < 0 ? -1 : base + e;
        }
    return r;
}
std::vector<int> concat(std::vector<int> a, const std::vector<int>& b) {
    a.insert(a.end(), b.begin(), b.end());
    return a;
}

struct Net {
    int W, W2, C, NTW, NTH, NTR;
    bool transient;
    bool ext;
    int in_xyz, e_steps;
    const float* const* t;
    std::vector<float> th_w, th_b;
    std::vector<float> dt_w;
    const float* w(int l) const { return t[2 * l]; }
    const float* b(int l) const { return t[2 * l + 1]; }
};

Seg seg(int nt, int ks, std::vector<int> kidx, std::vector<int> ridx, const float* W, int ld, bool tr = false) {
    Seg s;
    s.nt = nt; s.ks = ks; s.kidx = std::move(kidx); s.ridx = std::move(ridx); s.W = W; s.ld = ld; s.transposed = tr;
    return s;
}

std::vector<int> k_xyz(const Net& n, int base) {
    return n.ext ? [&] { auto k = k_compact(n.e_steps, n.in_xyz); for (auto& v : k) if (v >= 0) v += base; return k; }()
                 : k_emb(10, n.e_steps, base);
}
std::vector<int> rows_xyz(const Net& n, int base) {
    if (!n.ext) return rows_emb(10, 2, base);
    std::vector<int> r(64, -1);
    for (int i = 0; i < 32; ++i) r[i] = base + 2 * nefes_row_reg(i) + nefes_row_half(i);
    return r;
}

static void mark(Seg& s, int kind) {
    s.x6 = kind != 0;
    s.h3 = kind == 2;
}

void add_trunk(const Net& n, Stream& st, int x6 = 0) {
    const int W = n.W, NT = n.NTW;
// ... 2 lines not shown
            st.segs.push_back(seg(NT, n.e_steps, k_xyz(n, 0), rows_natural(NT, W), n.w(0), n.in_xyz));
            mark(st.segs.back(), x6);
        } else if (l == 4) {
            st.segs.push_back(seg(NT, W / 2, k_natural(W / 2, n.in_xyz), rows_natural(NT, W), n.w(4), n.in_xyz + W));
            mark(st.segs.back(), x6);
            st.segs.push_back(seg(NT, n.e_steps, k_xyz(n, 0), rows_natural(NT, W), n.w(4), n.in_xyz + W));
            mark(st.segs.back(), x6);
        } else {
            st.segs.push_back(seg(NT, W / 2, k_natural(W / 2, 0), rows_natural(NT, W), n.w(l), W));
            mark(st.segs.back(), x6);
        }
        st.bias.push_back({n.b(l), rows_natural(NT, W)});
    }
    st.segs.push_back(seg(1, W / 2, k_natural(W / 2, 0), rows_natural(1, 1), n.w(L_SIGMA), W));
    mark(st.segs.back(), x6);
    st.bias.push_back({n.b(L_SIGMA), rows_natural(1, 1)});
}

void add_static_head(const Net& n, Stream& st, int x6 = 0) {
    const int W = n.W, W2 = n.W2;
    st.segs.push_back(seg(n.NTW, W / 2, k_natural(W / 2, 0), rows_natural(n.NTW, W), n.w(L_FINAL), W));
    mark(st.segs.back(), x6);
    st.bias.push_back({n.b(L_FINAL), rows_natural(n.NTW, W)});
    st.segs.push_back(seg(n.NTH, W / 2, k_natural(W / 2, 0), rows_natural(n.NTH, W2), n.w(L_DIR), W + 27));
    mark(st.segs.back(), x6);
    st.segs.push_back(seg(n.NTH, NEFES_D_STEPS, k_emb(4, NEFES_D_STEPS, W), rows_natural(n.NTH, W2), n.w(L_DIR), W + 27));
    st.bias.push_back({n.b(L_DIR), rows_natural(n.NTH, W2)});
    st.segs.push_back(seg(n.NTR, W2 / 2, k_natural(W2 / 2, 0), rows_natural(n.NTR, 3 + n.C), n.w(L_RGB), W2));
    st.bias.push_back({n.b(L_RGB), rows_natural(n.NTR, 3 + n.C)});
}

void add_static_head_h3(const Net& n, Stream& st) {
    const int W = n.W, W2 = n.W2;
    st.segs.push_back(seg(n.NTW, W / 2, k_natural(W / 2, 0), rows_natural(n.NTW, W), n.w(L_FINAL), W));
    mark(st.segs.back(), 2);
    st.bias.push_back({n.b(L_FINAL), rows_natural(n.NTW, W)});
    st.segs.push_back(seg(n.NTH, W / 2, k_natural(W / 2, 0), rows_natural(n.NTH, W2), n.w(L_DIR), W + 27));
    mark(st.segs.back(), 2);
    st.segs.push_back(seg(n.NTH, 16, k_emb(4, 16, W), rows_natural(n.NTH, W2), n.w(L_DIR), W + 27));
    mark(st.segs.back(), 2);
    st.bias.push_back({n.b(L_DIR), rows_natural(n.NTH, W2)});
    st.segs.push_back(seg(n.NTR, W2 / 2, k_natural(W2 / 2, 0), rows_natural(n.NTR, 3 + n.C), n.w(L_RGB), W2));
    mark(st.segs.back(), 2);
    st.bias.push_back({n.b(L_RGB), rows_natural(n.NTR, 3 + n.C)});
}

void add_heads_x6(const Net& n, Stream& st, int kind = 1) {
    const int W = n.W, W2 = n.W2;
    st.segs.push_back(seg(n.NTW, W / 2, k_natural(W / 2, 0), rows_natural(n.NTW, W), n.w(L_FINAL), W));
    mark(st.segs.back(), kind);
    st.bias.push_back({n.b(L_FINAL), rows_natural(n.NTW, W)});
    st.segs.push_back(seg(2 * n.NTH, W / 2, k_natural(W / 2, 0), rows_natural(2 * n.NTH, 2 * W2), n.dt_w.data(), W + 27));
    mark(st.segs.back(), kind);
    st.segs.push_back(seg(2 * n.NTH, 16, k_emb(4, 16, W), rows_natural(2 * n.NTH, 2 * W2), n.dt_w.data(), W + 27));
    mark(st.segs.back(), kind);
    st.bias.push_back({n.b(L_DIR), rows_natural(n.NTH, W2)});
    st.segs.push_back(seg(n.NTR, W2 / 2, k_natural(W2 / 2, 0), rows_natural(n.NTR, 3 + n.C), n.w(L_RGB), W2));
    mark(st.segs.back(), kind);
    st.bias.push_back({n.b(L_RGB), rows_natural(n.NTR, 3 + n.C)});
    st.bias.push_back({n.b(L_T0), rows_natural(n.NTH, W2)});
    for (int l = L_T1; l <= L_T2; ++l) {
        st.segs.push_back(seg(n.NTH, W2 / 2, k_natural(W2 / 2, 0), rows_natural(n.NTH, W2), n.w(l), W2));
        mark(st.segs.back(), kind);
        st.bias.push_back({n.b(l), rows_natural(n.NTH, W2)});
    }
    st.segs.push_back(seg(1, W2 / 2, k_natural(W2 / 2, 0), rows_natural(1, 5), n.th_w.data(), W2));
    mark(st.segs.back(), kind);
    st.bias.push_back({n.th_b.data(), rows_natural(1, 5)});
}

void add_transient_head(const Net& n, Stream& st, int x6 = 0) {
    const int W = n.W, W2 = n.W2;
    st.segs.push_back(seg(n.NTH, W / 2, k_natural(W / 2, 0), rows_natural(n.NTH, W2), n.w(L_T0), W + 27));
    st.segs.push_back(seg(n.NTH, NEFES_D_STEPS, k_emb(4, NEFES_D_STEPS, W), rows_natural(n.NTH, W2), n.w(L_T0), W + 27));
    st.bias.push_back({n.b(L_T0), rows_natural(n.NTH, W2)});
    for (int l = L_T1; l <= L_T2; ++l) {
        st.segs.push_back(seg(n.NTH, W2 / 2, k_natural(W2 / 2, 0), rows_natural(n.NTH, W2), n.w(l), W2));
        mark(st.segs.back(), x6);
        st.bias.push_back({n.b(l), rows_natural(n.NTH, W2)});
    }
    st.segs.push_back(seg(1, W2 / 2, k_natural(W2 / 2, 0), rows_natural(1, 5), n.th_w.data(), W2));
    st.bias.push_back({n.th_b.data(), rows_natural(1, 5)});
}

void add_backward(const Net& n, Stream& st, int x6 = 0, bool transient = true) {
    const int W = n.W, W2 = n.W2, NTW = n.NTW, NTH = n.NTH;
    if (x6 == 2) {
        const int ks = 8 * nefes_head_kr16(n.C);
        std::vector<int> k = k_natural(ks, 0);
        for (auto& v : k) if (v >= 3 + n.C) v = -1;
        st.segs.push_back(seg(NTH, ks, k, rows_natural(NTH, W2), n.w(L_RGB), W2, true));
        mark(st.segs.back(), 2);
    } else {
        const int kr = (3 + n.C + 1) / 2;
        st.segs.push_back(seg(NTH, kr, k_compact(kr, 3 + n.C), rows_natural(NTH, W2), n.w(L_RGB), W2, true));
    }
    if (transient) {
    st.segs.push_back(seg(NTH, 3, k_compact(3, 5), rows_natural(NTH, W2), n.th_w.data(), W2, true));
    st.segs.push_back(seg(NTH, W2 / 2, k_natural(W2 / 2, 0), rows_natural(NTH, W2), n.w(L_T2), W2, true));
    mark(st.segs.back(), x6);
    st.segs.push_back(seg(NTH, W2 / 2, k_natural(W2 / 2, 0), rows_natural(NTH, W2), n.w(L_T1), W2, true));
    mark(st.segs.back(), x6);
    }
    std::vector<int> rows_fd = concat(rows_emb(4, 1, W), rows_natural(NTW, W));
    if (transient) {
        st.segs.push_back(seg(NTW + 1, W2 / 2, k_natural(W2 / 2, 0), rows_fd, n.w(L_T0), W + 27, true));
        mark(st.segs.back(), x6);
    }
    st.segs.push_back(seg(NTW + 1, W2 / 2, k_natural(W2 / 2, 0), rows_fd, n.w(L_DIR), W + 27, true));
    mark(st.segs.back(), x6);
    st.segs.push_back(seg(NTW, W / 2, k_natural(W / 2, 0), rows_natural(NTW, W), n.w(L_FINAL), W, true));
    mark(st.segs.back(), x6);
    st.segs.push_back(seg(NTW, 1, k_compact(1, 1), rows_natural(NTW, W), n.w(L_SIGMA), W, true));
    for (int l = 7; l >= 0; --l) {
        if (l == 4) {
            const std::vector<int> re = rows_xyz(n, 0);
            std::vector<int> rows = concat(re, rows_natural(NTW, W));
            for (int i = (int)re.size(); i < (int)rows.size(); ++i) rows[i] += n.in_xyz;
            st.segs.push_back(seg(NTW + (int)re.size() / 32, W / 2, k_natural(W / 2, 0), rows, n.w(4), n.in_xyz + W, true));
            mark(st.segs.back(), x6);
        } else if (l == 0) {
            const std::vector<int> re = rows_xyz(n, 0);
            st.segs.push_back(seg((int)re.size() / 32, W / 2, k_natural(W / 2, 0), re, n.w(0), n.in_xyz, true));
            mark(st.segs.back(), x6);
        } else {
            st.segs.push_back(seg(NTW, W / 2, k_natural(W / 2, 0), rows_natural(NTW, W), n.w(l), W, true));
            mark(st.segs.back(), x6);
        }
    }
}

static size_t matrix_elems(const Net& n, const float* Wm) {
    if (Wm == n.th_w.data()) return n.th_w.size();
    if (Wm == n.dt_w.data()) return n.dt_w.size();
    const int W = n.W, W2 = n.W2;
    for (int l = 0; l < 18; ++l) {
        if (n.t[2 * l] != Wm) continue;
        if (l < 8) return (size_t)W * (l == 0 ? n.in_xyz : (l == 4 ? n.in_xyz + W : W));
        if (l == L_FINAL) return (size_t)W * W;
        if (l == L_DIR || l == L_T0) return (size_t)W2 * (W + 27);
        if (l == L_SIGMA) return (size_t)W;
        if (l == L_RGB) return (size_t)(3 + n.C) * W2;
        if (l == L_T1 || l == L_T2) return (size_t)W2 * W2;
        if (l == L_TRGB) return (size_t)3 * W2;
        return (size_t)W2;
// ... 5 lines not shown
    for (size_t i = 0; i < cnt; ++i) {
        const float a = fabsf(p[i]);
        if (a > m) m = a;
    }
    return m;
}
static void assign_weight_exponents(const Net& n, Stream (&st)[NEFES_N_STREAMS]) {
    const int e_dt = n.transient ? scale_exp(abs_max(n.dt_w.data(), n.dt_w.size())) : 0;
    for (auto& stream : st)
        for (auto& sg : stream.segs) {
            if (!sg.h3 || !sg.W) continue;
            const bool dt = sg.W == n.dt_w.data() || (n.transient && (sg.W == n.w(L_DIR) || sg.W == n.w(L_T0)));
            sg.wexp = dt ? e_dt : scale_exp(abs_max(sg.W, matrix_elems(n, sg.W)));
        }
}

static int group_of(const Net& n, const float* Wm) {
    if (!Wm) return -1;
    if (Wm == n.th_w.data()) return L_TRGB;
    if (Wm == n.dt_w.data()) return L_DIR;
    for (int l = 0; l < 18; ++l)
        if (n.t[2 * l] == Wm) return (n.transient && l == L_T0) ? (int)L_DIR : ((l == L_TSIGMA || l == L_TBETA) ? (int)L_TRGB : l);
    return -1;
}

bool build(const NefesNetDesc* d, const float* const* tensors, Net& n, Stream (&st)[NEFES_N_STREAMS]) {
    if (!d) return false;
    if (d->width != 128 && d->width != 256) return false;
    if (nefes_head_class(d->feat_dim) < 0) return false;
    n.W = d->width; n.W2 = n.W / 2; n.C = d->feat_dim;
    n.NTW = n.W / 32; n.NTH = n.W2 / 32; n.NTR = nefes_head_ntr(n.C);
    n.transient = d->has_transient != 0;
    n.ext = d->xyz_encoding == NEFES_XYZ_EXTERNAL32;
    if (d->xyz_encoding != NEFES_XYZ_FREQ10 && !n.ext) return false;
    n.in_xyz = n.ext ? 32 : 63;
    n.e_steps = n.ext ? NEFES_X_STEPS : NEFES_E_STEPS;
    n.t = tensors;
    if (tensors && n.transient) {
        n.th_w.assign((size_t)5 * n.W2, 0.f);
        n.th_b.assign(5, 0.f);
        memcpy(&n.th_w[0], n.w(L_TRGB), sizeof(float) * 3 * n.W2);
        memcpy(&n.th_w[(size_t)3 * n.W2], n.w(L_TSIGMA), sizeof(float) * n.W2);
        memcpy(&n.th_w[(size_t)4 * n.W2], n.w(L_TBETA), sizeof(float) * n.W2);
        memcpy(&n.th_b[0], n.b(L_TRGB), sizeof(float) * 3);
        n.th_b[3] = n.b(L_TSIGMA)[0];
        n.th_b[4] = n.b(L_TBETA)[0];
        n.dt_w.resize((size_t)2 * n.W2 * (n.W + 27));
        memcpy(&n.dt_w[0], n.w(L_DIR), sizeof(float) * n.W2 * (n.W + 27));
        memcpy(&n.dt_w[(size_t)n.W2 * (n.W + 27)], n.w(L_T0), sizeof(float) * n.W2 * (n.W + 27));
    } else {
        n.dt_w.assign((size_t)2 * n.W2 * (n.W + 27), 0.f);
        n.th_w.assign((size_t)5 * n.W2, 0.f);
        n.th_b.assign(5, 0.f);
    }
    static const float* dummy[36] = {nullptr};
    if (!tensors) n.t = dummy;
    add_trunk(n, st[NEFES_STREAM_FWD_SIGMA]);
    add_trunk(n, st[NEFES_STREAM_FWD_STATIC]);
    add_static_head(n, st[NEFES_STREAM_FWD_STATIC]);
    add_backward(n, st[NEFES_STREAM_BWD_STATIC], false, false);
    if (n.transient) {
        add_trunk(n, st[NEFES_STREAM_FWD_FULL]);
        add_static_head(n, st[NEFES_STREAM_FWD_FULL]);
        add_transient_head(n, st[NEFES_STREAM_FWD_FULL]);
        add_backward(n, st[NEFES_STREAM_BWD_FULL]);
    }
    const bool big = n.W == 256, small = n.W == 128 && n.C == 128 && !n.ext;
    const bool h3_shape = !n.ext || (n.W == 256 && nefes_head_class(n.C) == 0);
    if (big || small) add_trunk(n, st[NEFES_STREAM_FWD_SIGMA_X6], 1);
    if (n.transient && (big || small) && (small || n.C == 16)) {
        add_trunk(n, st[NEFES_STREAM_FWD_FULL_X6], 1);
        add_heads_x6(n, st[NEFES_STREAM_FWD_FULL_X6]);
        add_backward(n, st[NEFES_STREAM_BWD_FULL_X6], 1);
    }
    if (h3_shape) {
        add_trunk(n, st[NEFES_STREAM_FWD_SIGMA_H3], 2);
        st[NEFES_STREAM_FWD_SIGMA_H3].h3 = true;
        {
            add_trunk(n, st[NEFES_STREAM_FWD_STATIC_H3], 2);
            add_static_head_h3(n, st[NEFES_STREAM_FWD_STATIC_H3]);
            add_backward(n, st[NEFES_STREAM_BWD_STATIC_H3], 2, false);
            st[NEFES_STREAM_FWD_STATIC_H3].h3 = st[NEFES_STREAM_BWD_STATIC_H3].h3 = true;
        }
        if (n.transient) {
            add_trunk(n, st[NEFES_STREAM_FWD_FULL_H3], 2);
            add_heads_x6(n, st[NEFES_STREAM_FWD_FULL_H3], 2);
            add_backward(n, st[NEFES_STREAM_BWD_FULL_H3], 2);
            st[NEFES_STREAM_FWD_FULL_H3].h3 = st[NEFES_STREAM_BWD_FULL_H3].h3 = true;
        }
    }
    if (tensors) assign_weight_exponents(n, st);
    return true;
}

const uint64_t kHeaderBytes = NEFES_BLOB_HEADER_BYTES;
static_assert(sizeof(NefesBlobInfo) <= NEFES_BLOB_HEADER_BYTES, "blob header too small");
uint64_t align_up(uint64_t x, uint64_t a) { return (x + a - 1) / a * a; }

void fill_info(const Stream (&st)[NEFES_N_STREAMS], int width, NefesBlobInfo* info) {
    uint64_t off = kHeaderBytes;
    for (int k = 0; k < NEFES_N_STREAMS; ++k) {
        NefesStreamInfo& si = info->stream[k];
        const int kib = nefes_stream_slab_kib(k, width);
        si.n_slabs = (uint32_t)st[k].n_slabs(NEFES_FRAGS_OF_KIB(kib));
        si.bias_floats = (uint32_t)st[k].bias_floats();
        si.scale_off = (uint32_t)st[k].bias_only();
// ... 178 lines not shown
    const float* ptrs[36] = {nullptr};
    int64_t off[37] = {0};
    int need = 0;
    Net n;
    Stream st[NEFES_N_STREAMS];
    NefesBlobInfo info;
};
static int build_indexed(const NefesNetDesc* desc, Indexed& x, int64_t* tensor_elems_out) {
    {
        Stream tmp[NEFES_N_STREAMS];
        if (!build(desc, nullptr, x.n, tmp)) return NEFES_E_UNSUPPORTED;
    }
    x.need = desc->has_transient ? 36 : 24;
    x.idx.resize(x.need);
    int64_t flat = 0;
    for (int i = 0; i < x.need; ++i) {
        const int64_t ne = tensor_elems(x.n, i);
        if (tensor_elems_out) tensor_elems_out[i] = ne;
        x.idx[i].resize((size_t)ne);
        for (int64_t e = 0; e < ne; ++e) x.idx[i][(size_t)e] = (float)(flat + e + 1);
        x.off[i] = flat;
        flat += ne;
        x.ptrs[i] = x.idx[i].data();
    }
    x.off[x.need] = flat;
    if (flat + 1 >= (1 << 24)) return NEFES_E_UNSUPPORTED;
    if (!build(desc, x.ptrs, x.n, x.st)) return NEFES_E_UNSUPPORTED;
    fill_info(x.st, desc->width, &x.info);
    return 0;
}

extern "C" int nefes_pack_map(const NefesNetDesc* desc, uint32_t* map, size_t n_entries, int64_t* tensor_elems_out) {
    if (!desc || !map) return NEFES_E_BADARG;
    Indexed x;
    const int rc = build_indexed(desc, x, tensor_elems_out);
    if (rc) return rc;
    if (n_entries < x.info.total_bytes / 2) return NEFES_E_BADBLOB;
    memset(map, 0, sizeof(uint32_t) * (x.info.total_bytes / 2));
    return pack_walk(desc, x.n, nullptr, map, x.info, x.st);
}

extern "C" int nefes_pack_h3_plan(const NefesNetDesc* desc, int32_t* plan, size_t n_ints, size_t* needed) {
    if (!desc) return NEFES_E_BADARG;
    Indexed x;
    const int rc = build_indexed(desc, x, nullptr);
    if (rc) return rc;
    const Net& n = x.n;
    std::vector<int32_t> jobs, pool;
    auto job = [&](int kind, int out, const int (&arg)[6]) {
        jobs.push_back(kind); jobs.push_back(out);
        for (int v : arg) jobs.push_back(v);
    };
    const int n_layers = x.need / 2;
    for (int g = 0; g < n_layers; ++g) {
        if (group_of(n, n.t[2 * g]) != g) continue;
        int arg[6] = {0, 0, 0, 0, 0, 0}, cnt = 0;
        for (int l = 0; l < n_layers && cnt < 3; ++l)
            if (group_of(n, n.t[2 * l]) == g) { arg[2 * cnt] = (int)x.off[2 * l]; arg[2 * cnt + 1] = (int)(x.off[2 * l + 1] - x.off[2 * l]); ++cnt; }
        job(0, g, arg);
    }
    auto tensor_range = [&](const float* p, int& o, int& c) {
        for (int i = 0; i < x.need; ++i)
            if (n.t[i] == p) { o = (int)x.off[i]; c = (int)(x.off[i + 1] - x.off[i]); return true; }
        return false;
    };
    for (int k = 0; k < NEFES_N_STREAMS; ++k) {
        const NefesStreamInfo& si = x.info.stream[k];
        if (!x.st[k].h3 || si.n_slabs == 0) continue;
        const int ns = (int)x.st[k].segs.size(), nb = (int)x.st[k].bias.size();
        const int tab = (int)(si.bias_off / 4) + (int)si.scale_off;
        for (int i = 0; i < ns; ++i) {
            const Seg& sg = x.st[k].segs[i];
            int arg[6] = {0, 0, (int)pool.size(), 0, 0, 0};
            std::vector<int> rows, ks;
            for (int r : sg.ridx) if (r >= 0) rows.push_back(r);
            for (int kk : sg.kidx) if (kk >= 0) ks.push_back(kk);
// ... 33 lines not shown
```

nefes_amd/field.py:

```python
import os

import torch
import torch.nn as nn

from . import lib as L
from . import ops

FEATURE_DIM = 128


class FusionNet(nn.Module):
    mean = [0.485, 0.456, 0.406]
    std = [0.229, 0.224, 0.225]

    def __init__(self, f_dim, fusion_residule=False, no_BN=False):
        super().__init__()
        self.fusion_residule, self.no_BN = fusion_residule, no_BN
        layers = [nn.Conv2d(3 + f_dim, 64, 3, 1, 1), nn.ReLU(), nn.Conv2d(64, 64, 3, 1, 1), nn.ReLU(),
                  nn.Conv2d(64, 64, 3, 1, 1), nn.ReLU(), nn.Conv2d(64, f_dim, 5, 1, 2)]
        if not no_BN:
            layers.append(nn.BatchNorm2d(f_dim))
        self.net = nn.Sequential(*layers)
        self._norm = {}

# ... 172 lines not shown

    def invalidate_packed(self):
        self._pk_key = None

    def packed(self) -> ops.PackedField:
        if not self._supported():
            raise RuntimeError(f"nefes_amd: the HIP field kernels are built for D=8, skips=[4], frequency encodings of up to 10 / 4 "
                               f"octaves (3 + 6k inputs, k <= 10 / 4) and a feature head (f_dim>0); got D={self.D}, skips={self.skips}, "
                               f"W={self.W}, f_dim={self.W_features}, in_channels_xyz={self.in_channels_xyz}, "
                               f"in_channels_dir={self.in_channels_dir}.  Compiled: {ops.COMPILED_SET}")
        names = ops.PackedField.LAYERS_FINE if self.encode_transient else ops.PackedField.LAYERS_COARSE
        sd = dict(self.named_parameters())
        prm = [sd[n + s] for n in names for s in (".weight", ".bias")]
        key = tuple((p.data_ptr(), p._version, str(p.device)) for p in prm)
        pad = bool(self._embedding_columns())
        if os.environ.get("NEFES_DEBUG_PACK_CHECKSUM", "0") == "1":
            key += (float(sum(p.detach().double().sum() for p in prm)),)
        if (self._pk is not None and key != self._pk_key and any(p.requires_grad for p in prm)
                and all(p.is_cuda and p.device == self._pk.blob.device for p in prm)):
            if pad:
                ksd = self._kernel_params(sd)
                self._pk.repack([ksd[n + s_] for n in names for s_ in (".weight", ".bias")])
            else:
                self._pk.repack(prm)
            self._pk_key = key
        elif self._pk is None or key != self._pk_key:
            dev = prm[0].device if prm[0].is_cuda else torch.device("cuda")
            enc = L.XYZ_EXTERNAL32 if self.in_channels_xyz == 32 else L.XYZ_FREQ10
            self._pk = ops.PackedField(self._kernel_params({n: p.detach() for n, p in sd.items()}), self.W, self.W_features,
                                       self.encode_transient, dev, enc)
            self._pk_key = key
        return self._pk

    def factored_head_ok(self):
        return (ops.FACTORED_HEAD and self.encode_transient and self.W == 128 and self.in_channels_xyz != 32 and self._supported()
                and 3 + self.W_features > 3 + self.W // 2 + 1 and ops.SPLIT == "h3"
                and not any(p.requires_grad for n, p in self.named_parameters()
                            if not n.startswith(("fusion_net", "exposure_embedding"))))

    def packed_fh(self):
        names = ops.PackedField.LAYERS_FINE
        sd = dict(self.named_parameters())
        prm = [sd[n + s] for n in names for s in (".weight", ".bias")]
        key = tuple((p.data_ptr(), p._version, str(p.device)) for p in prm)
        if getattr(self, "_pk_fh", None) is None or key != self._pk_fh_key:
            dev = prm[0].device if prm[0].is_cuda else torch.device("cuda")
            ksd = dict(self._kernel_params({n: p.detach() for n, p in sd.items()}))
            w, b = ksd["static_rgb.0.weight"], ksd["static_rgb.0.bias"]
            ksd["static_rgb.0.weight"], ksd["static_rgb.0.bias"] = w[:3].contiguous(), b[:3].contiguous()
            pk = ops.PackedField(ksd, self.W, 0, True, dev, L.XYZ_FREQ10)
            w_f = w[3:].to(dev, torch.float32).contiguous()
            self._pk_fh = (pk, w_f, w_f.t().contiguous(), b[3:].to(dev, torch.float32).contiguous())
            self._pk_fh_key = key
        return self._pk_fh

    def forward(self, x, sigma_only=False, output_transient=True):
        if sigma_only:
            input_xyz = x
        else:
            input_xyz, input_dir_a = torch.split(x, [self.in_channels_xyz, self.in_channels_dir], dim=-1)
        h = input_xyz
        for i in range(self.D):
            if i in self.skips:
                h = torch.cat([input_xyz, h], 1)
            h = getattr(self, f"xyz_encoding_{i + 1}")(h)
        static_sigma = self.static_sigma(h)
        if sigma_only:
            return static_sigma
        final = self.xyz_encoding_final(h)
        head_in = torch.cat([final, input_dir_a], 1)
        static = torch.cat([self.static_rgb(self.dir_encoding(head_in)), static_sigma], 1)
        if not output_transient:
            return static
        t = self.transient_encoding(head_in)
        return torch.cat([static, self.transient_rgb(t), self.transient_sigma(t), self.transient_beta(t)], 1)

    def run_fusion_net(self, rgb, feature, H, W, B, per_image_norm=False):
        render_rgb = rgb.reshape(B, H, W, 3).permute(0, 3, 1, 2)
        render_feature = feature.reshape(B, H, W, self.W_features).permute(0, 3, 1, 2)
        fused = self.fusion_net.forward_parts(render_rgb, render_feature, per_image_norm)
        return render_rgb, render_feature, fused

    def exposure_coefficients(self, hist):
        return self.exposure_embedding(hist.long()).float()

    def apply_affine(self, a_embedded, rgb, batch_size):
        kernel = a_embedded[:, :9].reshape(-1, 3, 3)
        bias = a_embedded[:, 9:].reshape(-1, 3, 1)
        rgb = rgb.reshape(batch_size, -1, 3)
        rgb = torch.bmm(kernel, rgb.transpose(1, 2)) + bias
        return self.sigmoid(rgb.transpose(1, 2).reshape(-1, 3))

    def affine_color_transform(self, args, rgb, hist, batch_size):
        assert args.encode_hist and self.typ == 'coarse'
        self.a_embedded = self.exposure_coefficients(hist)
        return self.apply_affine(self.a_embedded, rgb, batch_size)


def run_network_NeRFH_NFF(inputs, viewdirs, ts, fn, embed_fn=None, embeddirs_fn=None, typ='coarse', output_transient=False,
                          netchunk=1024 * 64, test_time=False, store_rgb=False):
    pk = fn.packed()
    if typ == 'coarse' and test_time:
        mode = L.FIELD_SIGMA
    elif typ == 'coarse' or not output_transient:
        mode = L.FIELD_STATIC
    else:
        mode = L.FIELD_FULL
    dev = pk.blob.device
    raw_t = ops.FieldFromPoints.apply(inputs.to(dev), None if viewdirs is None else viewdirs.to(dev), pk, mode)
    return raw_t.permute(0, 2, 1)


class _Embedder:

    def __init__(self, num_freqs, max_freq_log2=None):
        max_freq_log2 = num_freqs - 1 if max_freq_log2 is None else max_freq_log2
        self.N_freqs, self.max_freq_log2 = num_freqs, max_freq_log2
        self.freq_bands = 2. ** torch.linspace(0., max_freq_log2, steps=num_freqs) if num_freqs > 0 else torch.zeros(0)
        self.out_dim = 3 * (1 + 2 * num_freqs)

    def embed(self, x):
        if self.max_freq_log2 == 0:
            return x
        parts = [x]
        for f in self.freq_bands:
            parts += [torch.sin(x * f), torch.cos(x * f)]
        return torch.cat(parts, -1)


def get_embedder(multires, i=0, reduce_mode=-1, epochToMaxFreq=-1):
    if i == -1:
        return nn.Identity(), 3
    if reduce_mode == 2:
        raise NotImplementedError("nefes_amd: reduce_embedding=2 (DNeRF window) is not built; the reference's NeRFH_NFF path cannot "
                                  "run it either (embed_fn is called without the epoch argument, nerfh_nff.py:197)")
    if reduce_mode == 0:
        eo = _Embedder(multires // 2, (multires - 1) // 2)
    elif reduce_mode == 1:
        eo = _Embedder(0, 0)
    else:
# ... 6 lines not shown
```

nefes_amd/lib.py:

```python
import ctypes as C
import os

import torch

_HERE = os.path.dirname(os.path.abspath(__file__))
LIB_PATH = os.environ.get("NEFES_HIP_LIB") or os.path.join(_HERE, "libnefes_hip.so")


class NefesNetDesc(C.Structure):
    _fields_ = [("width", C.c_int32), ("feat_dim", C.c_int32), ("has_transient", C.c_int32), ("xyz_encoding", C.c_int32)]


class NefesStreamInfo(C.Structure):
    _fields_ = [("slab_off", C.c_uint64), ("n_slabs", C.c_uint32), ("bias_floats", C.c_uint32), ("bias_off", C.c_uint64),
                ("scale_off", C.c_uint32), ("scale_count", C.c_uint32)]


class NefesBlobInfo(C.Structure):
    _fields_ = [("total_bytes", C.c_uint64), ("stream", NefesStreamInfo * 13)]


class NefesHashGridDesc(C.Structure):
    _fields_ = [("n_levels", C.c_int32), ("n_features", C.c_int32), ("log2_hashmap_size", C.c_int32),
                ("base_resolution", C.c_int32), ("per_level_scale", C.c_float), ("bound", C.c_float)]


ABI_VERSION = 15
STREAM_FWD_SIGMA, STREAM_FWD_STATIC, STREAM_FWD_FULL, STREAM_BWD_FULL, STREAM_FWD_SIGMA_X6, STREAM_FWD_FULL_X6, STREAM_BWD_FULL_X6, STREAM_BWD_STATIC = 0, 1, 2, 3, 4, 5, 6, 7
STREAM_FWD_SIGMA_H3, STREAM_FWD_FULL_H3, STREAM_BWD_FULL_H3, STREAM_FWD_STATIC_H3, STREAM_BWD_STATIC_H3 = 8, 9, 10, 11, 12
FIELD_SIGMA, FIELD_STATIC, FIELD_FULL = 0, 1, 2
XYZ_FREQ10, XYZ_EXTERNAL32 = 0, 1
(TB_E, TB_DV, TB_L1, TB_FINAL, TB_DIR, TB_T0, TB_T1, TB_T2, TB_RGB, TB_SIG, TB_TH, TB_END) = (0, 1, 2, 10, 11, 12, 13, 14, 15, 16,
                                                                                              17, 18)
COMP_TRANSIENT, COMP_STATIC_ONLY, COMP_SIGMA_ONLY, COMP_WHITE_BKGD, COMP_FEAT_WEIGHTS_ONLY = 1, 2, 4, 8, 16

_p, _i, _f, _u32, _sz = C.c_void_p, C.c_int, C.c_float, C.c_uint32, C.c_size_t
_desc = C.POINTER(NefesNetDesc)

SIGNATURES = {
    "nefes_version": (_i, []),
    "nefes_blob_info": (_i, [_desc, C.POINTER(NefesBlobInfo)]),
    "nefes_stream_slab_bytes": (_sz, [_desc, _i]),
    "nefes_fusion_input_fwd": (_i, [_i, _i, _i, _p, _p, _p, C.POINTER(_f), C.POINTER(_f), _p, _p, _p]),
    "nefes_fusion_input_bwd": (_i, [_i, _i, _i, _p, _p, _p, C.POINTER(_f), _p, _p, _p]),
    "nefes_upcos_loss_fwd": (_i, [_i, _i, _i, _i, _i, _i, _p, _p, _p, _p, _p]),
    "nefes_upcos_loss_bwd": (_i, [_i, _i, _i, _i, _i, _i, _p, _p, _p, _p, _p, _p, _p, _p, _p, _p, _i, _p, _p, _p]),
    "nefes_bicubic_gather_table": (_i, [_i, _i, _i, _i, _i, _p, _p, _p, _p]),
    "nefes_bicubic_gram": (_i, [_i, _i, _i, _i, _p, _p]),
    "nefes_bn_train_fwd": (_i, [_i, _i, C.c_int64, _i, _p, _p, _p, C.c_double, C.c_double, _p, _p, _p, _p, _p, _p]),
    "nefes_bn_train_bwd": (_i, [_i, _i, C.c_int64, _i, _p, _p, _p, _p, _p, _p]),
    "nefes_svd_reg_fwd": (_i, [_i, _p, _p, _p, _p]),
    "nefes_svd_reg_bwd": (_i, [_i, _p, _p, _p, _p]),
    "nefes_regressed_pose_fwd": (_i, [_i, _p, _i, _f, _f, _f, _f, _p, _p, _p]),
    "nefes_regressed_pose_bwd": (_i, [_i, _p, _i, _f, _p, _p, _p]),
    "nefes_upcos_prepare": (_i, [_i, _i, _i, _i, _i, _i, _p, _p, _p, _p, _p, _p, _p, _i, _p, _p, _p, _p]),
    "nefes_upcos_gram_fwd": (_i, [_i, _i, _i, _p, _p, _p, _p, _p, _i, _p, _p, _p, _p]),
    "nefes_upcos_gram_bwd": (_i, [_i, _i, _i, _p, _p, _p, _p, _p, _p]),
    "nefes_upcos_gram_lds_bytes": (_sz, [_i, _i, _i]),
    "nefes_adam_step": (_i, [_i, _p, _p, _p, _p, _p, _p, C.c_double, C.c_double, C.c_double, _p]),
    "nefes_pack_weights": (_i, [_desc, C.POINTER(_p), _i, _p, _sz]),
# ... 97 lines not shown
```

nefes_amd/ops.py:

```python
import ctypes as C
from typing import Optional

import os

import torch

from . import lib as L


def _stream():
    return C.c_void_p(torch.cuda.current_stream().cuda_stream)


TIMERS = None


class _timed:
    def __init__(self, name):
        self.name = name

    def __enter__(self):
        if TIMERS is not None:
            self.t0 = torch.cuda.Event(enable_timing=True)
            self.t1 = torch.cuda.Event(enable_timing=True)
# ... 169 lines not shown
    with _timed("field_fwd[sigma,h3]"):
        L.check(L.load().nefes_field_fwd_h3_zrow(pk.desc, _chk(pk.blob, "blob", torch.uint8), L.FIELD_SIGMA, N, S, _chk(rays_o, "rays_o"),
                                                 _chk(rays_d, "rays_d"), _chk(z_row, "z_row"), None, _chk(raw_t, "raw_t"), None, _stream()),
                "nefes_field_fwd_h3_zrow")
    return raw_t


def coarse_sample(sigma, z, Ni, u=None, want_samples=True, want_weights=False):
    sigma, z = _f32(sigma), _f32(z)
    N, Nc = sigma.shape[0], sigma.shape[-1]
    dev = sigma.device
    if u is None:
        u = _linspace01(Ni, dev)
    u = _f32(u)
    z_fine = torch.empty(N, Nc + Ni, device=dev)
    z_samples = torch.empty(N, Ni, device=dev) if want_samples else None
    weights = torch.empty(N, Nc, device=dev) if want_weights else None
    with _timed("coarse_sample"):
        L.check(L.load().nefes_coarse_sample(N, Nc, Ni, _chk(sigma, "sigma"), _chk(z, "z"), 1 if z.dim() == 1 else 0, _chk(u, "u"),
                                             1 if u.dim() == 2 else 0, _chk(z_fine, "z_fine"), _chk(z_samples, "z_samples"),
                                             _chk(weights, "weights"), _stream()), "nefes_coarse_sample")
    _tap("z_fine", z_fine)
    _tap("z_samples", z_samples)
    return (z_fine, z_samples, weights) if want_weights else (z_fine, z_samples)


class PackedField:

    LAYERS_COARSE = [f"xyz_encoding_{i}.0" for i in range(1, 9)] + ["xyz_encoding_final", "dir_encoding.0",
                                                                    "static_sigma.0", "static_rgb.0"]
    LAYERS_FINE = LAYERS_COARSE + ["transient_encoding.0", "transient_encoding.2", "transient_encoding.4",
                                   "transient_sigma.0", "transient_rgb.0", "transient_beta.0"]

    def __init__(self, state_dict, width, feat_dim, has_transient, device, xyz_encoding=0):
        lib = L.load()
        self.desc = L.NefesNetDesc(int(width), int(feat_dim), 1 if has_transient else 0, int(xyz_encoding))
        self.xyz_encoding = int(xyz_encoding)
        self.width, self.feat_dim, self.has_transient = int(width), int(feat_dim), bool(has_transient)
        info = L.NefesBlobInfo()
        L.check(lib.nefes_blob_info(self.desc, info), "nefes_blob_info")
        names = self.LAYERS_FINE if has_transient else self.LAYERS_COARSE
        host = []
        for n in names:
            host.append(state_dict[n + ".weight"].detach().to("cpu", torch.float32).contiguous())
            host.append(state_dict[n + ".bias"].detach().to("cpu", torch.float32).contiguous())
        ptrs = (C.c_void_p * len(host))(*[t.data_ptr() for t in host])
        blob = torch.zeros(info.total_bytes, dtype=torch.uint8)
        L.check(lib.nefes_pack_weights(self.desc, ptrs, len(host), C.c_void_p(blob.data_ptr()), blob.numel()),
                "nefes_pack_weights")
        self.blob = blob.to(device)
        self.info = info
        self.generation = 0
        self.h3_valid = True
        self._map = None

    def repack(self, params):
        lib = L.load()
        if self._map is None:
            n = self.info.total_bytes // 2
            host_map = torch.zeros(n, dtype=torch.int32)
            elems = (C.c_int64 * 36)()
            L.check(lib.nefes_pack_map(self.desc, C.c_void_p(host_map.data_ptr()), n, C.cast(elems, C.c_void_p)), "nefes_pack_map")
            self._map = host_map.to(self.blob.device)
            self._elems = list(elems)[:36 if self.has_transient else 24]
            need = C.c_size_t(0)
            L.check(lib.nefes_pack_h3_plan(self.desc, None, 0, C.byref(need)), "nefes_pack_h3_plan")
            plan = torch.zeros(int(need.value), dtype=torch.int32)
            L.check(lib.nefes_pack_h3_plan(self.desc, C.c_void_p(plan.data_ptr()), plan.numel(), None), "nefes_pack_h3_plan")
            self._plan_jobs = int(plan[0])
            self._plan = plan.to(self.blob.device)
            self._plan_scratch = torch.zeros(32, dtype=torch.int32, device=self.blob.device)
        if [int(p.numel()) for p in params] != self._elems:
            raise RuntimeError("nefes_amd: parameter shapes do not match the packed network description")
        flat = torch.cat([p.detach().reshape(-1) for p in params]).to(torch.float32)
        h3 = REPACK_H3 and self._plan_jobs > 0
        L.check(lib.nefes_pack_device(flat.data_ptr(), flat.numel(), self._map.data_ptr(), self._map.numel(),
                                      self._plan.data_ptr() if h3 else None, self._plan_jobs if h3 else 0,
                                      self._plan_scratch.data_ptr() if h3 else None, self.blob.data_ptr(), _stream()),
                "nefes_pack_device")
        self.generation += 1
        if not h3:
            self.h3_valid = False

    def h3_byte_ranges(self):
        out = []
        for k in (L.STREAM_FWD_SIGMA_H3, L.STREAM_FWD_FULL_H3, L.STREAM_BWD_FULL_H3, L.STREAM_FWD_STATIC_H3, L.STREAM_BWD_STATIC_H3):
            si = self.info.stream[k]
            if si.n_slabs:
                slab = int(L.load().nefes_stream_slab_bytes(self.desc, k))
                out.append((int(si.slab_off), int(si.slab_off + si.n_slabs * slab)))
                out.append((int(si.bias_off + 4 * si.scale_off), int(si.bias_off + 4 * si.bias_floats)))
        return out

    def check_generation(self, gen):
        if gen != self.generation:
            raise RuntimeError("nefes_amd: the network weights were modified (re-packed) between this forward pass and its "
                               "backward pass")

    def mask_bytes(self, M):
        return L.load().nefes_field_mask_bytes(self.desc, M)

    def n_raw(self, mode):
        return 1 if mode == L.FIELD_SIGMA else (3 + self.feat_dim + (1 if mode == L.FIELD_STATIC else 6))


def field_fwd(pk: PackedField, mode, N, S, rays_o=None, rays_d=None, z=None, pts=None, viewdirs=None, want_masks=False,
              xyz_enc=None):
    dev = pk.blob.device
    if not canonical_shape(pk):
        raise RuntimeError(f"nefes_amd: the {('sigma', 'static', 'full')[mode]} forward of W={pk.width}, f_dim={pk.feat_dim} was routed to "
                           f"the fp32-MFMA instances (NEFES_SPLIT={SPLIT}; or a frozen network's static head with test_time=False), "
                           f"which exist for the canonical shapes only.  Compiled: {COMPILED_SET}")
    raw_t = torch.empty(N, pk.n_raw(mode), S, device=dev)
    masks = torch.empty(pk.mask_bytes(N * S) // 4, dtype=torch.int32, device=dev) if want_masks else None
    with _timed(f"field_fwd[{('sigma', 'static', 'full')[mode]}]"):
      L.check(L.load().nefes_field_fwd(pk.desc, _chk(pk.blob, "blob", torch.uint8), mode, N, S, _chk(rays_o, "rays_o"),
                                     _chk(rays_d, "rays_d"), _chk(z, "z"), _chk(pts, "pts"), _chk(xyz_enc, "xyz_enc"),
                                     _chk(viewdirs, "viewdirs"), _chk(raw_t, "raw_t"), _chk(masks, "masks", torch.int32),
                                     _stream()), "nefes_field_fwd")
    if masks is not None:
        _tap("masks", (masks, N, S, pk.width, mode))
    return raw_t, masks


SPLIT = os.environ.get("NEFES_SPLIT", "h3")
REPACK_H3 = os.environ.get("NEFES_REPACK_H3", "1") != "0"
USE_X6 = os.environ.get("NEFES_X6", "1") != "0"
FUSED_COARSE = os.environ.get("NEFES_FUSED_COARSE", "1") != "0"


HEAD_MAX_C = 141
COMPILED_SET = L.COMPILED_SET


def head_class(C):
    return -1 if C < 0 else (0 if 3 + C <= 32 else (1 if 3 + C <= 144 else -1))


def canonical_shape(pk: PackedField):
    return (pk.width == 256 and pk.feat_dim == 16) or (pk.width == 128 and pk.feat_dim == 128 and pk.xyz_encoding == L.XYZ_FREQ10)


def h3_shape(pk: PackedField):
    cls = head_class(pk.feat_dim)
    if pk.width not in (128, 256) or cls < 0:
        return False
    return True if pk.xyz_encoding == L.XYZ_FREQ10 else (pk.width == 256 and cls == 0)


def x6_supported(pk: PackedField, mode, forward=True):
    if mode == L.FIELD_STATIC:
        return static_h3(pk)
    ok = canonical_shape(pk) or (_h3(pk) and h3_shape(pk))
    return ok and (mode == L.FIELD_SIGMA or (mode == L.FIELD_FULL and pk.has_transient))


def static_h3(pk: PackedField):
    return _h3(pk) and h3_shape(pk) and pk.xyz_encoding == L.XYZ_FREQ10


def _h3(pk):
    if SPLIT not in ("h3", "x6", "f32"):
        raise ValueError("nefes_amd.ops.SPLIT must be 'h3', 'x6' or 'f32'")
    return SPLIT == "h3" and pk.h3_valid


def require_instance(pk: PackedField, what):
    if canonical_shape(pk) or (_h3(pk) and h3_shape(pk)):
        return
    raise RuntimeError(f"nefes_amd: no kernel instance serves {what} for W={pk.width}, f_dim={pk.feat_dim}, "
                       f"xyz_encoding={pk.xyz_encoding} with NEFES_SPLIT={SPLIT}"
                       f"{'' if pk.h3_valid else ' (fp16 streams stale: NEFES_REPACK_H3=0)'}.  Compiled: {COMPILED_SET}")


def field_fwd_x6(pk: PackedField, mode, N, S, rays_o=None, rays_d=None, z=None, viewdirs=None, want_masks=False, xyz_enc=None,
                 pts=None):
    dev = pk.blob.device
    raw_t = torch.empty(N, pk.n_raw(mode), S, device=dev)
    masks = torch.empty(pk.mask_bytes(N * S) // 4, dtype=torch.int32, device=dev) if want_masks else None
    h3 = _h3(pk) and h3_shape(pk) and N * S < (1 << 31) - 256
    if mode == L.FIELD_STATIC and not h3:
        return field_fwd(pk, mode, N, S, rays_o=rays_o, rays_d=rays_d, z=z, pts=pts, viewdirs=viewdirs, want_masks=want_masks, xyz_enc=xyz_enc)
    if not h3 and not canonical_shape(pk):
        raise RuntimeError(f"nefes_amd: {N * S} samples in one launch exceed the fp16 two-part kernels' 32-bit sample index and "
                           f"W={pk.width}, f_dim={pk.feat_dim} has no other instance; render fewer rays per launch")
    fn = L.load().nefes_field_fwd_h3 if h3 else L.load().nefes_field_fwd_x6
    with _timed(f"field_fwd[{('sigma', 'static', 'full')[mode]},{'h3' if h3 else 'x6'}]"):
        L.check(fn(pk.desc, _chk(pk.blob, "blob", torch.uint8), mode, N, S, _chk(rays_o, "rays_o"),
                                            _chk(rays_d, "rays_d"), _chk(z, "z"), _chk(pts, "pts"), _chk(xyz_enc, "xyz_enc"),
                                            _chk(viewdirs, "viewdirs"),
                                            _chk(raw_t, "raw_t"), _chk(masks, "masks", torch.int32), _stream()),
                "nefes_field_fwd_x6")
    if masks is not None:
        _tap("masks", (masks, N, S, pk.width, mode))
    return raw_t, masks


def field_bwd(pk: PackedField, N, S, raw_t, g_raw_t, masks, rays_o=None, rays_d=None, z=None, pts=None, viewdirs=None,
              mode=L.FIELD_FULL):
    dev = pk.blob.device
    ext = pk.xyz_encoding == L.XYZ_EXTERNAL32
    if mode == L.FIELD_STATIC and USE_X6 and SPLIT != "f32" and static_h3(pk) and N * S < (1 << 31) - 256:
        g_pts, g_vs = torch.empty(N * S, 3, device=dev), torch.empty(N * S, 3, device=dev)
        with _timed("field_bwd[static,h3]"):
            L.check(L.load().nefes_field_bwd_static_h3(pk.desc, _chk(pk.blob, "blob", torch.uint8), N, S, _chk(rays_o, "rays_o"),
                                                       _chk(rays_d, "rays_d"), _chk(z, "z"), _chk(pts, "pts"), _chk(viewdirs, "viewdirs"),
                                                       _chk(raw_t, "raw_t"), _chk(g_raw_t, "g_raw_t"), _chk(masks, "masks", torch.int32),
                                                       _chk(g_pts, "g_pts"), _chk(g_vs, "g_vs"), _stream()), "nefes_field_bwd_static_h3")
        return g_pts, g_vs
    if mode == L.FIELD_STATIC:
        if not canonical_shape(pk):
            raise RuntimeError(f"nefes_amd: the static-head backward of W={pk.width}, f_dim={pk.feat_dim} was routed to the fp32-MFMA "
                               f"instances (NEFES_SPLIT={SPLIT}), which exist for the canonical shapes only.  Compiled: {COMPILED_SET}")
# ... 83 lines not shown
        ctx.F1 = F1
        return feat

    @staticmethod
    def backward(ctx, g_feat):
        w, b = ctx.saved_tensors
        g_feat = _f32(g_feat)
        N, C = g_feat.shape
        g_gmap = torch.empty(N, ctx.F1, device=g_feat.device)
        with _timed("feat_head_bwd"):
            L.check(L.load().nefes_feat_head_bwd(N, C, ctx.F1 - 1, _chk(g_feat, "g_feat"), _chk(w, "w"), _chk(b, "b"), _chk(g_gmap, "g_gmap"),
                                                 _stream()), "nefes_feat_head_bwd")
        return g_gmap, None, None, None


class FieldFromRaysFH(torch.autograd.Function):

    @staticmethod
    def forward(ctx, rays_o, rays_d, viewdirs, z, pk):
        rays_o, rays_d, viewdirs, z = _f32(rays_o), _f32(rays_d), _f32(viewdirs), _f32(z)
        N, S = z.shape
        if N * S >= (1 << 31) - 256:
            raise RuntimeError("nefes_amd: too many samples for one launch of the fp16 two-part kernels (32-bit sample index)")
        need = any(ctx.needs_input_grad[:3])
        R = 3 + pk.width // 2 + 1 + 6
        raw_t = torch.empty(N, R, S, device=z.device)
        masks = torch.empty(pk.mask_bytes(N * S) // 4, dtype=torch.int32, device=z.device) if need else None
        with _timed("field_fwd[full,h3,fh]"):
            L.check(L.load().nefes_field_fwd_h3_fh(pk.desc, _chk(pk.blob, "blob", torch.uint8), L.FIELD_FULL, N, S, _chk(rays_o, "rays_o"),
                                                   _chk(rays_d, "rays_d"), _chk(z, "z"), _chk(viewdirs, "viewdirs"), _chk(raw_t, "raw_t"),
                                                   _chk(masks, "masks", torch.int32), _stream()), "nefes_field_fwd_h3_fh")
        if masks is not None:
            _tap("masks", (masks, N, S, pk.width, L.FIELD_FULL))
        ctx.pk, ctx.have, ctx.pk_gen = pk, need, pk.generation
        if need:
            ctx.save_for_backward(rays_o, rays_d, viewdirs, z, raw_t, masks)
        return raw_t

    @staticmethod
    def backward(ctx, g_raw_t):
        if not ctx.have:
            return None, None, None, None, None
        rays_o, rays_d, viewdirs, z, raw_t, masks = ctx.saved_tensors
        N, S = z.shape
        pk = ctx.pk
        pk.check_generation(ctx.pk_gen)
        g_pts, g_vs = torch.empty(N * S, 3, device=z.device), torch.empty(N * S, 3, device=z.device)
        with _timed("field_bwd[h3,fh]"):
            L.check(L.load().nefes_field_bwd_h3_fh(pk.desc, _chk(pk.blob, "blob", torch.uint8), N, S, _chk(rays_o, "rays_o"),
                                                   _chk(rays_d, "rays_d"), _chk(z, "z"), _chk(viewdirs, "viewdirs"), _chk(raw_t, "raw_t"),
                                                   _chk(_f32(g_raw_t), "g_raw_t"), None, _chk(masks, "masks", torch.int32), _chk(g_pts, "g_pts"),
                                                   _chk(g_vs, "g_vs"), _stream()), "nefes_field_bwd_h3_fh")
        g_o, g_d, g_v = ray_grad_reduce(N, S, z, g_pts, g_vs)
        return g_o, g_d, g_v, None, None


class RenderFineFH(torch.autograd.Function):

    @staticmethod
    def forward(ctx, rays_o, rays_d, viewdirs, z, pk, w_f, w_f_t, b_f, flags, beta_min, emit_gmap=False):
        rays_o, rays_d, viewdirs, z = _f32(rays_o), _f32(rays_d), _f32(viewdirs), _f32(z)
        N, S = z.shape
        need = any(ctx.needs_input_grad[:3])
        Cg = pk.width // 2
        raw_t = torch.empty(N, 3 + Cg + 1 + 6, S, device=z.device)
        masks = torch.empty(pk.mask_bytes(N * S) // 4, dtype=torch.int32, device=z.device) if need else None
        with _timed("field_fwd[full,h3,fh]"):
            L.check(L.load().nefes_field_fwd_h3_fh(pk.desc, _chk(pk.blob, "blob", torch.uint8), L.FIELD_FULL, N, S, _chk(rays_o, "rays_o"),
                                                   _chk(rays_d, "rays_d"), _chk(z, "z"), _chk(viewdirs, "viewdirs"), _chk(raw_t, "raw_t"),
                                                   _chk(masks, "masks", torch.int32), _stream()), "nefes_field_fwd_h3_fh")
        if masks is not None:
            _tap("masks", (masks, N, S, pk.width, L.FIELD_FULL))
        rgb, gmap, disp, acc, _, _, _ = composite_fwd(raw_t, z, Cg + 1, flags, beta_min)
        if emit_gmap:
            feat = gmap
        else:
            C = w_f.shape[0]
            feat = torch.empty(N, C, device=z.device)
            with _timed("feat_head_fwd"):
                L.check(L.load().nefes_feat_head_fwd(N, C, Cg, _chk(gmap, "gmap"), _chk(w_f_t, "w_t"), _chk(b_f, "b"), _chk(feat, "feat"), _stream()),
                        "nefes_feat_head_fwd")
        ctx.set_materialize_grads(False)
        ctx.pk, ctx.have, ctx.pk_gen, ctx.cfg, ctx.emit_gmap = pk, need, pk.generation, (Cg, int(flags)), bool(emit_gmap)
        if need:
            ctx.save_for_backward(rays_o, rays_d, viewdirs, z, raw_t, masks, w_f, b_f)
        return rgb, feat, disp, acc

    @staticmethod
    def backward(ctx, g_rgb, g_feat, g_disp, g_acc):
        if not ctx.have:
            return (None,) * 11
        rays_o, rays_d, viewdirs, z, raw_t, masks, w_f, b_f = ctx.saved_tensors
        N, S = z.shape
        pk = ctx.pk
        pk.check_generation(ctx.pk_gen)
        Cg, flags = ctx.cfg
        fix = lambda g: None if (g is None or g.numel() == 0) else _f32(g)
        g_rgb, g_feat, g_disp, g_acc = fix(g_rgb), fix(g_feat), fix(g_disp), fix(g_acc)
        g_gmap = None
        if g_feat is not None and ctx.emit_gmap:
            g_gmap = g_feat
        elif g_feat is not None:
            g_gmap = torch.empty(N, Cg + 1, device=z.device)
            with _timed("feat_head_bwd"):
                L.check(L.load().nefes_feat_head_bwd(N, w_f.shape[0], Cg, _chk(g_feat, "g_feat"), _chk(w_f, "w"), _chk(b_f, "b"),
# ... 184 lines not shown
    @property
    def trainable(self):
        return torch.is_grad_enabled() and self.table.requires_grad


FUSED_HASHGRID = os.environ.get("NEFES_FUSED_HASHGRID", "1") != "0"


def hashgrid_fused_ok(pk, grid):
    return (FUSED_HASHGRID and isinstance(grid, HashGrid) and _h3(pk) and pk.xyz_encoding == L.XYZ_EXTERNAL32 and pk.width == 256
            and head_class(pk.feat_dim) == 0 and grid.desc.n_levels == 16 and grid.desc.n_features == 2)


class FieldFromRaysHashGrid(torch.autograd.Function):

    @staticmethod
    def forward(ctx, rays_o, rays_d, viewdirs, z, pk, mode, grid):
        rays_o, rays_d, viewdirs, z = _f32(rays_o), _f32(rays_d), _f32(viewdirs), _f32(z)
        N, S = z.shape
        if N * S >= (1 << 31) - 256:
            raise RuntimeError("nefes_amd: too many samples for one launch of the fp16 two-part kernels (32-bit sample index)")
        if mode not in (L.FIELD_SIGMA, L.FIELD_FULL):
            raise NotImplementedError("nefes_amd: the hash-grid field kernels evaluate the sigma-only or the full head")
        need = mode == L.FIELD_FULL and any(ctx.needs_input_grad[:3])
        raw_t = torch.empty(N, pk.n_raw(mode), S, device=z.device)
        masks = torch.empty(pk.mask_bytes(N * S) // 4, dtype=torch.int32, device=z.device) if need else None
        with _timed(f"field_fwd[{('sigma', 'static', 'full')[mode]},h3,hashgrid]"):
            L.check(L.load().nefes_field_fwd_h3_hashgrid(pk.desc, _chk(pk.blob, "blob", torch.uint8), grid.desc, _chk(grid.table, "table"), mode, N, S,
                                                         _chk(rays_o, "rays_o"), _chk(rays_d, "rays_d"), _chk(z, "z"), 0, _chk(viewdirs, "viewdirs"),
                                                         _chk(raw_t, "raw_t"), _chk(masks, "masks", torch.int32), _stream()),
                    "nefes_field_fwd_h3_hashgrid")
        if masks is not None:
            _tap("masks", (masks, N, S, pk.width, mode))
        ctx.pk, ctx.grid, ctx.have, ctx.pk_gen = pk, grid, need, pk.generation
        if need:
            ctx.save_for_backward(rays_o, rays_d, viewdirs, z, raw_t, masks)
        return raw_t

    @staticmethod
    def backward(ctx, g_raw_t):
        if not ctx.have:
            raise NotImplementedError("nefes_amd: the sigma-only field pass has no backward (nerfh_nff.py:192-202 runs it without gradients)")
        rays_o, rays_d, viewdirs, z, raw_t, masks = ctx.saved_tensors
        N, S = z.shape
        pk, grid = ctx.pk, ctx.grid
        pk.check_generation(ctx.pk_gen)
        g_pts, g_vs = torch.empty(N * S, 3, device=z.device), torch.empty(N * S, 3, device=z.device)
        with _timed("field_bwd[h3,hashgrid]"):
            L.check(L.load().nefes_field_bwd_h3_hashgrid(pk.desc, _chk(pk.blob, "blob", torch.uint8), grid.desc, _chk(grid.table, "table"), N, S,
                                                         _chk(rays_o, "rays_o"), _chk(rays_d, "rays_d"), _chk(z, "z"), _chk(viewdirs, "viewdirs"),
                                                         _chk(raw_t, "raw_t"), _chk(_f32(g_raw_t), "g_raw_t"), _chk(masks, "masks", torch.int32),
                                                         _chk(g_pts, "g_pts"), _chk(g_vs, "g_vs"), _stream()), "nefes_field_bwd_h3_hashgrid")
        g_o, g_d, g_v = ray_grad_reduce(N, S, z, g_pts, g_vs)
        return g_o, g_d, g_v, None, None, None, None


def hashgrid_bwd_table(grid, x, g_enc, g_table=None):
    lib = L.load()
    if g_table is None:
        g_table = torch.zeros_like(grid.table, dtype=torch.float32)
    ws = torch.empty(max(1, int(lib.nefes_hashgrid_bwd_table_workspace(grid.desc))), dtype=torch.uint8, device=g_table.device)
    with _timed("hashgrid_bwd_table"):
        L.check(lib.nefes_hashgrid_bwd_table(grid.desc, x.shape[0], _chk(x, "x"), _chk(g_enc, "g_enc"), _chk(g_table, "g_table"),
                                             C.c_void_p(ws.data_ptr()), _stream()), "nefes_hashgrid_bwd_table")
    return g_table

# ... 544 lines not shown
```

nefes_amd/render.py:

```python
import types

import torch

from . import lib as L
from . import ops

_DEV = "cuda"
MAX_RAYS_PER_LAUNCH = 1 << 22
MEMORY_FRACTION = 0.6


_STEP = {}
_PER_RAY = {}


def rays_per_launch(cfg, network_fn, network_fine, device, train=False):
    net = network_fine if (network_fine is not None and cfg.N_importance > 0) else network_fn
    S = cfg.N_samples + cfg.N_importance if not cfg.use_fine_only or cfg.N_importance == 0 else cfg.N_importance
    Wd, C = net.W, net.W_features
    dev = torch.device(device)
    key = (Wd, C, S, cfg.N_samples, bool(train), dev.type, dev.index)
    if key in _STEP:
        return _STEP[key]
    R = 3 + C + 6
# ... 42 lines not shown
def _trainable(net):
    return (torch.is_grad_enabled() and net is not None
            and any(p.requires_grad for n, p in net.named_parameters()
                    if not n.startswith(("fusion_net", "exposure_embedding"))))


def _grid_trainable(xyz_encoder):
    return xyz_encoder is not None and bool(getattr(xyz_encoder, "trainable", False))


def _field(pk, mode, rays_o, rays_d, viewdirs, z, xyz_encoder):
    if xyz_encoder is None:
        return ops.FieldFromRays.apply(rays_o, rays_d, viewdirs, z, pk, mode)
    if (mode != L.FIELD_STATIC and ops.hashgrid_fused_ok(pk, xyz_encoder) and z.shape[0] * z.shape[1] < (1 << 31) - 256
            and not _grid_trainable(xyz_encoder)):
        return ops.FieldFromRaysHashGrid.apply(rays_o, rays_d, viewdirs, z, pk, mode, xyz_encoder)
    pts = rays_o[:, None, :] + rays_d[:, None, :] * z[..., None]
    return ops.FieldFromEncoding.apply(xyz_encoder(pts), viewdirs, pk, mode)


def _render_core(rays_o, rays_d, viewdirs, near, far, network_fn, network_fine, cfg, bounds=None):
    N = rays_o.shape[0]
    dev = rays_o.device
    Nc, Ni = cfg.N_samples, cfg.N_importance
    trainable = _trainable

    def field(net, pk, mode, z_):
        grid_static = mode == L.FIELD_STATIC and _grid_trainable(cfg.xyz_encoder)
        if (trainable(net) or grid_static) and mode != L.FIELD_SIGMA:
            from . import train as T
            if cfg.xyz_encoder is not None:
                return T.field_train_encoded(net, mode, cfg.xyz_encoder, rays_o, rays_d, viewdirs, z_)
            return T.field_train(net, mode, rays_o, rays_d, viewdirs, z_)
        return _field(pk, mode, rays_o, rays_d, viewdirs, z_, cfg.xyz_encoder)

    pk_c = network_fn.packed()
    C = pk_c.feat_dim
    store_rgb = (Ni == 0)
    if (cfg.test_time and cfg.perturb == 0. and cfg.raw_noise_std == 0. and bounds is None
            and not cfg.use_fine_only and ops.fused_coarse_pass_ok(pk_c, Nc, Ni, N, cfg.xyz_encoder)):
        with torch.no_grad():
            z_row = ops.coarse_depth_row(Nc, near, far, cfg.lindisp, dev)
            raw_c = ops.field_sigma_row(pk_c, rays_o.detach(), rays_d.detach(), z_row, cfg.xyz_encoder)
            z_fine, z_samples = ops.coarse_sample(raw_c, z_row, Ni, want_samples=False)
        return _fine_pass(rays_o, rays_d, viewdirs, z_fine, z_samples, network_fine, cfg, C, field, None)
    t_rand = torch.rand(N, Nc, device=dev) if cfg.perturb > 0. else None
    z = ops.coarse_depths(N, Nc, near, far, cfg.lindisp, t_rand, device=dev, bounds=bounds)
    if cfg.test_time:
        with torch.no_grad():
            raw_c = _field(pk_c, L.FIELD_SIGMA, rays_o.detach(), rays_d.detach(), viewdirs.detach(), z, cfg.xyz_encoder)
            if cfg.raw_noise_std > 0.:
                raw_c = raw_c + _noise(raw_c.shape, dev) * cfg.raw_noise_std
            _, _, _, acc0, _, w0, _ = ops.composite_fwd(raw_c, z, C, L.COMP_SIGMA_ONLY)
        rgb0 = feat0 = disp0 = None
    else:
        raw_c = field(network_fn, pk_c, L.FIELD_STATIC, z)
        if cfg.raw_noise_std > 0.:
            raw_c = _with_density_noise(raw_c, C, cfg.raw_noise_std)
        rgb0, feat0, disp0, acc0, _, w0, _ = ops.Composite.apply(raw_c, z, C, 0, 0.1)
    if Ni == 0:
        if cfg.test_time:
            raise NotImplementedError("nefes_amd: N_importance == 0 at test time renders nothing in the reference "
                                      "either (sigma-only coarse branch, rendering.py:116-125)")
        ret = {"rgb_map": rgb0, "disp_map": disp0, "acc_map": acc0}
        if cfg.nerfh_nff:
            ret["feat_map"] = feat0
        return ret
# ... 155 lines not shown
```

Baseline: 713,800 rays/s.

## Fold xyz_encoding_final linear layer into downstream head weights for frozen inference

The linear xyz_encoding_final layer (no activation) is algebraically folded into the dir_encoding and transient_encoding input weights on the host, in double precision, at pack time. This removes one 256x256 matmul from both the forward and backward kernels. The backward feeds the sigma gradient straight into the trunk in place of the final-layer backward GEMM. It applies only to frozen, non-training networks and adds a new packed-blob flag, ABI bump and kernel template instances. It also changes rounding slightly and disables the wide-layer path in the folded backward with transient.

New measurement: 772,200 rays/s, median of 6. 1.08x the previous value.

```diff
diff --git a/include/nefes_hip.h b/include/nefes_hip.h
--- a/include/nefes_hip.h
+++ b/include/nefes_hip.h
@@ -7,7 +7,7 @@
 extern "C" {
 #endif
 
-#define NEFES_ABI_VERSION 15
+#define NEFES_ABI_VERSION 16
 
 #define NEFES_E_BADARG (-1)
 #define NEFES_E_UNSUPPORTED (-2)
@@ -18,6 +18,7 @@
     int32_t feat_dim;
     int32_t has_transient;
     int32_t xyz_encoding;
+    int32_t fold_final;
 } NefesNetDesc;
 #define NEFES_XYZ_FREQ10 0
 #define NEFES_XYZ_EXTERNAL32 1
diff --git a/nefes_amd/csrc/field_bwd_h3.hip b/nefes_amd/csrc/field_bwd_h3.hip
--- a/nefes_amd/csrc/field_bwd_h3.hip
+++ b/nefes_amd/csrc/field_bwd_h3.hip
@@ -89,14 +89,15 @@
     return __builtin_nontemporal_load(p);
 }
 
-template <int W, int KR16, int ENC, bool HAS_T = true, bool TRAIN = false, bool FH = false>
-__global__ __launch_bounds__(256, NEFES_H3B_WG_PER_CU(W)) void field_bwd_h3_kernel(FieldBwdH3Args a) {
+template <int W, int KR16, int ENC, bool HAS_T, bool TRAIN, bool FH, bool FOLD>
+__device__ __forceinline__ void field_bwd_h3_body(const FieldBwdH3Args& a) {
+    static_assert(!FOLD || !TRAIN, "the train-mode instances need both matrices' gradients");
     constexpr int NTW = W / 32, NTH = W / 64, HS = W / 2, GS = W / 4;
     constexpr int MW = 8 * (W / 64) + 4 * (W / 128);
     constexpr int WT = (NTW + 1) / 2, WH = (NTH + 1) / 2;
     constexpr int MW_TRUNK = 8 * WT;
     constexpr int NTR = KR16 <= 2 ? 1 : 5;
-    constexpr int WIDE_LAYERS = ENC == NEFES_XYZ_HASHGRID_FUSED ? 0 : H3B_WIDE_LAYERS;
+    constexpr int WIDE_LAYERS = (ENC == NEFES_XYZ_HASHGRID_FUSED || (FOLD && HAS_T)) ? 0 : H3B_WIDE_LAYERS;
     static_assert(KR16 == 2 || KR16 == 9, "head classes of layout.h (nefes_head_kr16 / nefes_head_ntr)");
     const int C3 = 3 + a.C;
     static_assert(MW % 4 == 0, "mask words are staged as 16-byte groups");
@@ -107,13 +108,13 @@
     constexpr int SX = ENC == NEFES_XYZ_HASHGRID_FUSED ? 24 : 8;
     int* tab_i = (int*)(smem + NEFES_H3B_SLOTS * NEFES_SLAB_BYTES + (size_t)4 * (MW + SX) * 256);
     const float* tab_f = (const float*)tab_i;
-    if (threadIdx.x < 2 * (HAS_T ? NEFES_H3B_N : NEFES_H3B_N_STATIC)) tab_i[threadIdx.x] = a.tab[threadIdx.x];
+    if (threadIdx.x < 2 * ((HAS_T ? NEFES_H3B_N : NEFES_H3B_N_STATIC) - (FOLD ? 1 : 0))) tab_i[threadIdx.x] = a.tab[threadIdx.x];
     HgGeom* hg_lds = (HgGeom*)(tab_i + 64);
     if constexpr (ENC == NEFES_XYZ_HASHGRID_FUSED) {
         if (threadIdx.x == 0) *hg_lds = a.hg;
     }
-    auto wexp = [&](int seg) { return tab_i[nefes_h3_tab_exp(nefes_h3b_seg(HAS_T, seg))]; };
-    auto rowb = [&](int seg) { return tab_f[nefes_h3_tab_bound(nefes_h3b_seg(HAS_T, seg))]; };
+    auto wexp = [&](int seg) { return tab_i[nefes_h3_tab_exp(nefes_h3b_seg(HAS_T, seg, FOLD))]; };
+    auto rowb = [&](int seg) { return tab_f[nefes_h3_tab_bound(nefes_h3b_seg(HAS_T, seg, FOLD))]; };
     StagedRing ring;
     ring.init(a.stream, a.n_slabs, smem, wave, lane);
     const char* ring_lane = smem + lane * 16;
@@ -303,6 +304,7 @@
         }
         }
         f32x16 XA[NTW + 2], XB[NTW + 2];
+        f32x16 (&XD)[NTW + 2] = *(FOLD ? &XB : &XA);
         int es_dt;
         {
             const int ew = wexp(NEFES_H3B_DIR);
@@ -313,21 +315,21 @@
             load_dg(dgv);
             if constexpr (HAS_T) {
                 load_bits(bh, MW_TRUNK + WH, WH);
-                mma_run_h3<NTW + 1, GS / 8, 1, true>(ring, ring_lane, wrap_store_h3<TRAIN>(MaskedSplitH<NTH, WH, 0>{T3, bh, pow2i(tau - es3), mt}, gptr(NEFES_TB_T0), pow2i(-es3)), ZeroInit{}, XA);
+                mma_run_h3<NTW + 1, GS / 8, 1, true>(ring, ring_lane, wrap_store_h3<TRAIN>(MaskedSplitH<NTH, WH, 0>{T3, bh, pow2i(tau - es3), mt}, gptr(NEFES_TB_T0), pow2i(-es3)), ZeroInit{}, XD);
             }
             load_bits(bh, MW_TRUNK, WH);
 #ifdef NEFES_FH_VARIANT_VALU_UPDATE
             if constexpr (FH) {
 #pragma unroll
                 for (int e = 0; e < 16 * NTH; ++e) G2[e >> 4][e & 15] += dgv[e] * pow2i(es_g2);
-                mma_run_h3<NTW + 1, GS / 8, 1, !HAS_T>(ring, ring_lane, MaskedSplitH<NTH, WH, 0>{G2, bh, pow2i(tau - es_g2), mg}, ZeroInit{}, XA);
+                mma_run_h3<NTW + 1, GS / 8, 1, !HAS_T>(ring, ring_lane, MaskedSplitH<NTH, WH, 0>{G2, bh, pow2i(tau - es_g2), mg}, ZeroInit{}, XD);
             } else
 #else
             if constexpr (FH)
-                mma_run_h3<NTW + 1, GS / 8, 1, !HAS_T>(ring, ring_lane, MaskedAddSplitH<NTH, WH, 0, 16 * NTH>{G2, bh, pow2i(tau - es_g2), mg, dgv, pow2i(es_g2)}, ZeroInit{}, XA);
+                mma_run_h3<NTW + 1, GS / 8, 1, !HAS_T>(ring, ring_lane, MaskedAddSplitH<NTH, WH, 0, 16 * NTH>{G2, bh, pow2i(tau - es_g2), mg, dgv, pow2i(es_g2)}, ZeroInit{}, XD);
             else
 #endif
-            mma_run_h3<NTW + 1, GS / 8, 1, !HAS_T>(ring, ring_lane, wrap_store_h3<TRAIN>(MaskedSplitH<NTH, WH, 0>{G2, bh, pow2i(tau - es_g2), mg}, gptr(NEFES_TB_DIR), pow2i(-es_g2)), ZeroInit{}, XA);
+            mma_run_h3<NTW + 1, GS / 8, 1, !HAS_T>(ring, ring_lane, wrap_store_h3<TRAIN>(MaskedSplitH<NTH, WH, 0>{G2, bh, pow2i(tau - es_g2), mg}, gptr(NEFES_TB_DIR), pow2i(-es_g2)), ZeroInit{}, XD);
             M = (HAS_T ? rowb(NEFES_H3B_T0) * (pair_max(mt) * pow2i(-es3)) : 0.f) + rowb(NEFES_H3B_DIR) * (pair_max(mg) * pow2i(-es_g2));
         }
         float gv[3];
@@ -335,7 +337,7 @@
             float dDv[16], v3[3];
             const float inv = pow2i(-es_dt);
 #pragma unroll
-            for (int r = 0; r < 16; ++r) dDv[r] = XA[1][r] * inv;
+            for (int r = 0; r < 16; ++r) dDv[r] = XD[1][r] * inv;
 #pragma unroll
             for (int c = 0; c < 3; ++c) v3[c] = STASH(3 + c);
             embed_slots_bwd<NEFES_N_FREQ_DIR>(gv, dDv, v3, h);
@@ -345,7 +347,18 @@
             }
         }
         int es_b;
-        {
+        if constexpr (FOLD) {
+            es_b = es_dt;
+            const float dsig = STASH(6);
+            float dsg[1];
+            dsg[0] = dsig * pow2i(es_b);
+#if defined(H3B_WIDE) && defined(H3_WIDE_ENTRY_FENCE)
+            mma_run<NTW, 1, 2, false, ((WIDE_LAYERS >> 8) & 1) == 0 || (NTW < NEFES_H3_WIDE_MIN)>(ring, ring_lane, ArrayIn<1>{dsg}, ZeroInit{}, XB);
+#else
+            mma_run<NTW, 1, 2, false>(ring, ring_lane, ArrayIn<1>{dsg}, ZeroInit{}, XB);
+#endif
+            M += rowb(NEFES_H3B_SIG) * pair_max(fabsf(dsig));
+        } else {
             const int ew = wexp(NEFES_H3B_FINAL), tau = tau_of(M, ew);
             float mx = 0.f;
             es_b = tau + ew;
@@ -454,12 +467,23 @@
 }
 
 template <int W, int KR16, int ENC, bool HAS_T = true, bool TRAIN = false, bool FH = false>
+__global__ __launch_bounds__(256, NEFES_H3B_WG_PER_CU(W)) void field_bwd_h3_kernel(FieldBwdH3Args a) {
+    field_bwd_h3_body<W, KR16, ENC, HAS_T, TRAIN, FH, false>(a);
+}
+template <int W, int KR16, int ENC, bool HAS_T = true, bool FH = false>
+__global__ __launch_bounds__(256, NEFES_H3B_WG_PER_CU(W)) void field_bwd_h3_fold_kernel(FieldBwdH3Args a) {
+    field_bwd_h3_body<W, KR16, ENC, HAS_T, false, FH, true>(a);
+}
+
+template <int W, int KR16, int ENC, bool HAS_T = true, bool TRAIN = false, bool FH = false, bool FOLD = false>
 static int launch_bwd_h3(const FieldBwdH3Args& a, hipStream_t st) {
     const size_t lds = (size_t)NEFES_H3B_SLOTS * NEFES_SLAB_BYTES
                        + (size_t)4 * (8 * (W / 64) + 4 * (W / 128) + (ENC == NEFES_XYZ_HASHGRID_FUSED ? 24 : 8)) * 256 + 256
                        + (ENC == NEFES_XYZ_HASHGRID_FUSED ? 512 : 0);
     static_assert(sizeof(HgGeom) <= 512 && 2 * NEFES_H3B_N <= 64, "scale table (256 bytes) + the level geometry's LDS slot");
-    auto k = field_bwd_h3_kernel<W, KR16, ENC, HAS_T, TRAIN, FH>;
+    void (*k)(FieldBwdH3Args);
+    if constexpr (FOLD) k = field_bwd_h3_fold_kernel<W, KR16, ENC, HAS_T, FH>;
+    else k = field_bwd_h3_kernel<W, KR16, ENC, HAS_T, TRAIN, FH>;
     hipError_t e = hipFuncSetAttribute((const void*)k, hipFuncAttributeMaxDynamicSharedMemorySize, (int)lds);
     if (e != hipSuccess) return (int)e;
     int dev = 0, cus = 256;
@@ -476,7 +500,10 @@
 #define NEFES_TU_PART 0
 #endif
 enum { BWD_H3_EXT = 0, BWD_H3_FULL, BWD_H3_TRAIN_STATIC, BWD_H3_TRAIN_FULL, BWD_H3_STATIC, BWD_H3_HG, BWD_H3_FH, BWD_H3_TRAIN_EXT_STATIC,
-       BWD_H3_TRAIN_EXT_FULL };
+       BWD_H3_TRAIN_EXT_FULL,
+       BWD_H3_FOLD = 0x100  };
+#define NEFES_H3B_FOLDED(fold, W, KR16, ENC, HAS_T, FH) \
+    ((fold) ? launch_bwd_h3<W, KR16, ENC, HAS_T, false, FH, true>(a, st) : launch_bwd_h3<W, KR16, ENC, HAS_T, false, FH>(a, st))
 int nefes_bwd_h3_launch_part1(int which, const FieldBwdH3Args& a, hipStream_t st);
 int nefes_bwd_h3_launch_part2(int which, const FieldBwdH3Args& a, hipStream_t st);
 int nefes_bwd_h3_launch_part3(int which, const FieldBwdH3Args& a, hipStream_t st);
@@ -488,15 +515,19 @@
 
 #if NEFES_TU_PART == 1
 int nefes_bwd_h3_launch_part1(int which, const FieldBwdH3Args& a, hipStream_t st) {
-    if (which == BWD_H3_EXT) return launch_bwd_h3<256, 2, NEFES_XYZ_EXTERNAL32>(a, st);
-    if (which == BWD_H3_STATIC) return launch_bwd_h3<256, 2, NEFES_XYZ_FREQ10, false>(a, st);
-    if (which == BWD_H3_HG) return launch_bwd_h3<256, 2, NEFES_XYZ_HASHGRID_FUSED>(a, st);
+    const bool fold = (which & BWD_H3_FOLD) != 0;
+    which &= ~BWD_H3_FOLD;
+    if (which == BWD_H3_EXT) return NEFES_H3B_FOLDED(fold, 256, 2, NEFES_XYZ_EXTERNAL32, true, false);
+    if (which == BWD_H3_STATIC) return NEFES_H3B_FOLDED(fold, 256, 2, NEFES_XYZ_FREQ10, false, false);
+    if (which == BWD_H3_HG) return NEFES_H3B_FOLDED(fold, 256, 2, NEFES_XYZ_HASHGRID_FUSED, true, false);
     return NEFES_E_UNSUPPORTED;
 }
 #elif NEFES_TU_PART == 2
 int nefes_bwd_h3_launch_part2(int which, const FieldBwdH3Args& a, hipStream_t st) {
-    if (which == BWD_H3_FULL) return launch_bwd_h3<128, 9, NEFES_XYZ_FREQ10>(a, st);
-    if (which == BWD_H3_STATIC) return launch_bwd_h3<128, 9, NEFES_XYZ_FREQ10, false>(a, st);
+    const bool fold = (which & BWD_H3_FOLD) != 0;
+    which &= ~BWD_H3_FOLD;
+    if (which == BWD_H3_FULL) return NEFES_H3B_FOLDED(fold, 128, 9, NEFES_XYZ_FREQ10, true, false);
+    if (which == BWD_H3_STATIC) return NEFES_H3B_FOLDED(fold, 128, 9, NEFES_XYZ_FREQ10, false, false);
     return NEFES_E_UNSUPPORTED;
 }
 #elif NEFES_TU_PART == 3
@@ -515,15 +546,19 @@
 }
 #elif NEFES_TU_PART == 5
 int nefes_bwd_h3_launch_part5(int which, const FieldBwdH3Args& a, hipStream_t st) {
-    if (which == BWD_H3_FULL) return launch_bwd_h3<256, 9, NEFES_XYZ_FREQ10>(a, st);
-    if (which == BWD_H3_STATIC) return launch_bwd_h3<256, 9, NEFES_XYZ_FREQ10, false>(a, st);
+    const bool fold = (which & BWD_H3_FOLD) != 0;
+    which &= ~BWD_H3_FOLD;
+    if (which == BWD_H3_FULL) return NEFES_H3B_FOLDED(fold, 256, 9, NEFES_XYZ_FREQ10, true, false);
+    if (which == BWD_H3_STATIC) return NEFES_H3B_FOLDED(fold, 256, 9, NEFES_XYZ_FREQ10, false, false);
     return NEFES_E_UNSUPPORTED;
 }
 #elif NEFES_TU_PART == 6
 int nefes_bwd_h3_launch_part6(int which, const FieldBwdH3Args& a, hipStream_t st) {
-    if (which == BWD_H3_FULL) return launch_bwd_h3<128, 2, NEFES_XYZ_FREQ10>(a, st);
-    if (which == BWD_H3_STATIC) return launch_bwd_h3<128, 2, NEFES_XYZ_FREQ10, false>(a, st);
-    if (which == BWD_H3_FH) return launch_bwd_h3<128, 2, NEFES_XYZ_FREQ10, true, false, true>(a, st);
+    const bool fold = (which & BWD_H3_FOLD) != 0;
+    which &= ~BWD_H3_FOLD;
+    if (which == BWD_H3_FULL) return NEFES_H3B_FOLDED(fold, 128, 2, NEFES_XYZ_FREQ10, true, false);
+    if (which == BWD_H3_STATIC) return NEFES_H3B_FOLDED(fold, 128, 2, NEFES_XYZ_FREQ10, false, false);
+    if (which == BWD_H3_FH) return NEFES_H3B_FOLDED(fold, 128, 2, NEFES_XYZ_FREQ10, true, true);
     return NEFES_E_UNSUPPORTED;
 }
 #elif NEFES_TU_PART == 7
@@ -548,6 +583,7 @@
         return NEFES_E_BADARG;
     if (!(rays_o && rays_d && z)) return NEFES_E_BADARG;
     if (mode != NEFES_FIELD_STATIC && mode != NEFES_FIELD_FULL) return NEFES_E_BADARG;
+    if (desc->fold_final) return NEFES_E_UNSUPPORTED;
     const bool full = mode == NEFES_FIELD_FULL;
     if (full && !desc->has_transient) return NEFES_E_UNSUPPORTED;
     const int cls = nefes_head_class(desc->feat_dim);
@@ -580,6 +616,7 @@
     if (!desc || !packed || !viewdirs || !raw_t || !g_raw_t || !masks || !dacts || !g_xyz_enc || !g_viewdirs_s || N <= 0 || S <= 0)
         return NEFES_E_BADARG;
     if (mode != NEFES_FIELD_STATIC && mode != NEFES_FIELD_FULL) return NEFES_E_BADARG;
+    if (desc->fold_final) return NEFES_E_UNSUPPORTED;
     const bool full = mode == NEFES_FIELD_FULL;
     if (full && !desc->has_transient) return NEFES_E_UNSUPPORTED;
     if (desc->width != 256 || nefes_head_class(desc->feat_dim) != 0 || desc->xyz_encoding != NEFES_XYZ_EXTERNAL32) return NEFES_E_UNSUPPORTED;
@@ -615,7 +652,8 @@
     int rc = nefes_blob_info(desc, &info);
     if (rc) return rc;
     const NefesStreamInfo& si = info.stream[NEFES_STREAM_BWD_STATIC_H3];
-    if (si.n_slabs == 0 || si.scale_count < 2 * (uint32_t)NEFES_H3B_N_STATIC) return NEFES_E_UNSUPPORTED;
+    const int F = desc->fold_final ? BWD_H3_FOLD : 0;
+    if (si.n_slabs == 0 || si.scale_count < 2 * (uint32_t)(NEFES_H3B_N_STATIC - (F ? 1 : 0))) return NEFES_E_UNSUPPORTED;
     FieldBwdH3Args a;
     a.stream = (const char*)packed + si.slab_off;
     a.tab = (const int*)((const char*)packed + si.bias_off) + si.scale_off;
@@ -627,8 +665,8 @@
     a.n_tiles = (int)((a.M + 127) / 128);
     a.dacts = nullptr; a.rows = 0; a.gout = 0; a.hg_table = nullptr; a.g_gmap = nullptr;
     hipStream_t st = (hipStream_t)stream;
-    if (desc->width == 256) return cls == 0 ? nefes_bwd_h3_launch_part1(BWD_H3_STATIC, a, st) : nefes_bwd_h3_launch_part5(BWD_H3_STATIC, a, st);
-    return cls == 1 ? nefes_bwd_h3_launch_part2(BWD_H3_STATIC, a, st) : nefes_bwd_h3_launch_part6(BWD_H3_STATIC, a, st);
+    if (desc->width == 256) return cls == 0 ? nefes_bwd_h3_launch_part1(BWD_H3_STATIC | F, a, st) : nefes_bwd_h3_launch_part5(BWD_H3_STATIC | F, a, st);
+    return cls == 1 ? nefes_bwd_h3_launch_part2(BWD_H3_STATIC | F, a, st) : nefes_bwd_h3_launch_part6(BWD_H3_STATIC | F, a, st);
 }
 
 static int field_bwd_h3_impl(const NefesNetDesc* desc, const void* packed, int N, int S, const float* rays_o,
@@ -646,7 +684,8 @@
     int rc = nefes_blob_info(desc, &info);
     if (rc) return rc;
     const NefesStreamInfo& si = info.stream[NEFES_STREAM_BWD_FULL_H3];
-    if (si.n_slabs == 0 || si.scale_count < 2 * NEFES_H3B_N) return NEFES_E_UNSUPPORTED;
+    const int F = desc->fold_final ? BWD_H3_FOLD : 0;
+    if (si.n_slabs == 0 || si.scale_count < 2 * (uint32_t)(NEFES_H3B_N - (F ? 1 : 0))) return NEFES_E_UNSUPPORTED;
     FieldBwdH3Args a;
     a.stream = (const char*)packed + si.slab_off;
     a.tab = (const int*)((const char*)packed + si.bias_off) + si.scale_off;
@@ -673,11 +712,12 @@
     hipStream_t st = (hipStream_t)stream;
     const int cls = nefes_head_class(desc->feat_dim);
     if (cls < 0) return NEFES_E_UNSUPPORTED;
-    if (fh) return nefes_bwd_h3_launch_part6(BWD_H3_FH, a, st);
-    if (desc->width == 256 && fused_grid) return cls == 0 ? nefes_bwd_h3_launch_part1(BWD_H3_HG, a, st) : NEFES_E_UNSUPPORTED;
-    if (desc->width == 256 && ext) return cls == 0 ? nefes_bwd_h3_launch_part1(BWD_H3_EXT, a, st) : NEFES_E_UNSUPPORTED;
-    if (desc->width == 256) return cls == 0 ? launch_bwd_h3<256, 2, NEFES_XYZ_FREQ10>(a, st) : nefes_bwd_h3_launch_part5(BWD_H3_FULL, a, st);
-    if (desc->width == 128 && !ext) return cls == 1 ? nefes_bwd_h3_launch_part2(BWD_H3_FULL, a, st) : nefes_bwd_h3_launch_part6(BWD_H3_FULL, a, st);
+    if (fh) return nefes_bwd_h3_launch_part6(BWD_H3_FH | F, a, st);
+    if (desc->width == 256 && fused_grid) return cls == 0 ? nefes_bwd_h3_launch_part1(BWD_H3_HG | F, a, st) : NEFES_E_UNSUPPORTED;
+    if (desc->width == 256 && ext) return cls == 0 ? nefes_bwd_h3_launch_part1(BWD_H3_EXT | F, a, st) : NEFES_E_UNSUPPORTED;
+    if (desc->width == 256 && cls != 0) return nefes_bwd_h3_launch_part5(BWD_H3_FULL | F, a, st);
+    if (desc->width == 256) return NEFES_H3B_FOLDED(F != 0, 256, 2, NEFES_XYZ_FREQ10, true, false);
+    if (desc->width == 128 && !ext) return cls == 1 ? nefes_bwd_h3_launch_part2(BWD_H3_FULL | F, a, st) : nefes_bwd_h3_launch_part6(BWD_H3_FULL | F, a, st);
     return NEFES_E_UNSUPPORTED;
 }
 
diff --git a/nefes_amd/csrc/field_fwd_h3.hip b/nefes_amd/csrc/field_fwd_h3.hip
--- a/nefes_amd/csrc/field_fwd_h3.hip
+++ b/nefes_amd/csrc/field_fwd_h3.hip
@@ -65,13 +65,15 @@
         }
 }
 
-template <int MODE, int ENC, int W = 256, int NTR = 1, bool TRAIN = false, bool FH = false>
-__global__ __launch_bounds__(256, W == 128 ? 2 : 1) void field_fwd_h3_kernel(FieldFwdH3Args a) {
+template <int MODE, int ENC, int W, int NTR, bool TRAIN, bool FH, bool FOLD>
+__device__ __forceinline__ void field_fwd_h3_body(const FieldFwdH3Args& a) {
+    static_assert(!FOLD || (MODE != NEFES_FIELD_SIGMA && !TRAIN), "the fold serves the inference instances that run the heads");
     static_assert(NEFES_SLAB_KIB == (W == 128 ? NEFES_H3_FWD_SLAB_KIB_128 : NEFES_H3_FWD_SLAB_KIB), "ring slab size != the packer's for this width");
     constexpr int NTW = W / 32, NTH = W / 64;
     constexpr int ES = ENC != NEFES_XYZ_FREQ10 ? NEFES_X_STEPS : NEFES_E_STEPS;
     constexpr int MW = 8 * (W / 64) + 4 * (W / 128), WT = (NTW + 1) / 2, WH = (NTH + 1) / 2;
-    constexpr int NSEG = MODE == NEFES_FIELD_SIGMA ? NEFES_H3F_SIG + 1 : (MODE == NEFES_FIELD_STATIC ? NEFES_H3F_N_STATIC : NEFES_H3F_N);
+    constexpr int NSEG = (MODE == NEFES_FIELD_SIGMA ? NEFES_H3F_SIG + 1 : (MODE == NEFES_FIELD_STATIC ? NEFES_H3F_N_STATIC : NEFES_H3F_N))
+                         - (FOLD ? 1 : 0);
     extern __shared__ __attribute__((aligned(16))) char smem[];
     char* ring_base = smem;
     float* bias_lds = (float*)(smem + NEFES_H3_SLOTS * NEFES_SLAB_BYTES);
@@ -90,11 +92,11 @@
     const char* bias_half = (const char*)bias_lds + 16 * h;
     const int* tab_i = (const int*)(bias_lds + a.scale_off);
     const float* tab_f = bias_lds + a.scale_off;
-    auto wexp = [&](int seg) { return tab_i[nefes_h3_tab_exp(seg)]; };
-    auto rowb = [&](int seg) { return tab_f[nefes_h3_tab_bound(seg)]; };
-    auto bmax = [&](int blk) { return tab_f[nefes_h3_tab_bias(NSEG, blk)]; };
+    auto wexp = [&](int seg) { return tab_i[nefes_h3_tab_exp(nefes_h3f_seg(seg, FOLD))]; };
+    auto rowb = [&](int seg) { return tab_f[nefes_h3_tab_bound(nefes_h3f_seg(seg, FOLD))]; };
+    auto bmax = [&](int blk) { return tab_f[nefes_h3_tab_bias(NSEG, nefes_h3bb_block(blk, FOLD))]; };
     ring.prime(ring_lane);
-    constexpr int B_SIG = 8 * W, B_FINAL = B_SIG + 32, B_DIR = B_FINAL + W, B_RGB = B_DIR + W / 2,
+    constexpr int B_SIG = 8 * W, B_FINAL = B_SIG + 32, B_DIR = B_FINAL + (FOLD ? 0 : W), B_RGB = B_DIR + W / 2,
                   B_T0 = B_RGB + 32 * NTR, B_T1 = B_T0 + W / 2, B_T2 = B_T1 + W / 2, B_TH = B_T2 + W / 2;
 #pragma unroll 1
     for (int tile = blockIdx.x; tile < a.n_tiles; tile += gridDim.x) {
@@ -224,7 +226,8 @@
             save_trunk(L1_, B, es_b);                                                                                          \
         }                                                                                                                      \
         put_masks(bits, WT);
-        constexpr int NPAIRS = MODE == NEFES_FIELD_SIGMA ? 3 : 4;
+        constexpr bool TAIL8 = MODE == NEFES_FIELD_SIGMA || FOLD;
+        constexpr int NPAIRS = TAIL8 ? 3 : 4;
 #pragma unroll 1
         for (int p = 0; p < NPAIRS; ++p) {
             const int l1 = 2 + 2 * p, l2 = l1 + 1;
@@ -254,9 +257,9 @@
             }
             put_masks(bits, WT);
         }
-        if constexpr (MODE == NEFES_FIELD_SIGMA) { NEFES_FWD_EVEN_LAYER(8, NEFES_H3F_L8) }
+        if constexpr (TAIL8) { NEFES_FWD_EVEN_LAYER(8, NEFES_H3F_L8) }
 #undef NEFES_FWD_EVEN_LAYER
-        if constexpr (MODE == NEFES_FIELD_SIGMA) sigma_head(B, es_b, tau_of(M, wexp(NEFES_H3F_SIG)));
+        if constexpr (TAIL8) sigma_head(B, es_b, tau_of(M, wexp(NEFES_H3F_SIG)));
         if constexpr (MODE != NEFES_FIELD_SIGMA) {
             constexpr bool FULL = MODE == NEFES_FIELD_FULL;
             constexpr int NDT = FULL ? 2 * NTH : NTH;
@@ -296,6 +299,21 @@
                 const int tau = tau_of(fmaxf(M, mD), ew);
                 float mx = 0.f;
                 es_dt = tau + ew;
+                if constexpr (FOLD) {
+                    clear_bits();
+                    if constexpr (CB) {
+                        const char* bp8 = bias_half + 7 * W * 4;
+                        nbias = ReluBiasSplitH<true, NTW, WT>::prime(bp8);
+                        const ReluBiasSplitH<true, NTW, WT> src8{B, bits, pow2i(tau - es_b), mx, bp8, pow2i(es_b), nbias};
+                        if constexpr (FULL) mma_run_h3<NDT, W / 16, 0, true>(ring, ring_lane, src8, Bias2{bias_at(B_DIR, es_dt), bias_at(B_T0, es_dt)}, dt);
+                        else mma_run_h3<NDT, W / 16, 0, true>(ring, ring_lane, src8, bias_at(B_DIR, es_dt), dt);
+                    } else if constexpr (FULL)
+                        mma_run_h3<NDT, W / 16, 0, true>(ring, ring_lane, ReluSplitH<true, NTW, WT>{B, bits, pow2i(tau - es_b), mx},
+                                                         Bias2{bias_at(B_DIR, es_dt), bias_at(B_T0, es_dt)}, dt);
+                    else
+                        mma_run_h3<NDT, W / 16, 0, true>(ring, ring_lane, ReluSplitH<true, NTW, WT>{B, bits, pow2i(tau - es_b), mx}, bias_at(B_DIR, es_dt), dt);
+                    put_masks(bits, WT);
+                } else
                 if constexpr (CB) {
                     const char* bpf = bias_half + B_FINAL * 4;
                     nbias = ReluBiasSplitH<false, 1, 1>::prime(bpf);
@@ -308,7 +326,7 @@
                 else
                     mma_run_h3<NDT, W / 16, 0, true>(ring, ring_lane, IdentSplitH<NTW, 0>{A, pow2i(tau - es_a), mx}, bias_at(B_DIR, es_dt), dt);
                 mma_run_h3<NDT, 2, 0, false>(ring, ring_lane, ArraySplitH<16>{Dv, pow2i(tau)}, ZeroInit{}, dt);
-                M = rowb(NEFES_H3F_DT_H) * (pair_max(mx) * pow2i(-es_a)) + rowb(NEFES_H3F_DT_D) * mD
+                M = rowb(NEFES_H3F_DT_H) * (pair_max(mx) * pow2i(-(FOLD ? es_b : es_a))) + rowb(NEFES_H3F_DT_D) * mD
                     + (FULL ? fmaxf(bmax(NEFES_H3BB_DIR), bmax(NEFES_H3BB_T0)) : bmax(NEFES_H3BB_DIR));
                 if constexpr (TRAIN) {
                     train_save_h3<NTH, 0>(act_tile, act_voff, nefes_train_row(W, 0, NEFES_TB_DIR), dt, pow2i(-es_dt));
@@ -414,6 +432,15 @@
     }
 }
 
+template <int MODE, int ENC, int W = 256, int NTR = 1, bool TRAIN = false, bool FH = false>
+__global__ __launch_bounds__(256, W == 128 ? 2 : 1) void field_fwd_h3_kernel(FieldFwdH3Args a) {
+    field_fwd_h3_body<MODE, ENC, W, NTR, TRAIN, FH, false>(a);
+}
+template <int MODE, int ENC, int W = 256, int NTR = 1, bool FH = false>
+__global__ __launch_bounds__(256, W == 128 ? 2 : 1) void field_fwd_h3_fold_kernel(FieldFwdH3Args a) {
+    field_fwd_h3_body<MODE, ENC, W, NTR, false, FH, true>(a);
+}
+
 static void magic_div(uint32_t d, uint32_t& magic, uint32_t& shift) {
     if (d == 1) { magic = 0; shift = 0; return; }
     uint32_t l = 0;
@@ -423,13 +450,15 @@
     shift = (uint32_t)(p - 32);
 }
 
-template <int MODE, int ENC, int W = 256, int NTR = 1, bool TRAIN = false, bool FH = false>
+template <int MODE, int ENC, int W = 256, int NTR = 1, bool TRAIN = false, bool FH = false, bool FOLD = false>
 static int launch_h3(const FieldFwdH3Args& a, hipStream_t st) {
     constexpr int ES_ = ENC != NEFES_XYZ_FREQ10 ? NEFES_X_STEPS : NEFES_E_STEPS;
     const size_t lds = (size_t)NEFES_H3_SLOTS * NEFES_SLAB_BYTES + ((a.bias_floats + 63) / 64) * 256 + (size_t)4 * ES_ * 64 * 4
                        + (ENC == NEFES_XYZ_HASHGRID_FUSED ? 512 : 0);
     static_assert(sizeof(HgGeom) <= 512, "the level geometry's LDS slot");
-    auto k = field_fwd_h3_kernel<MODE, ENC, W, NTR, TRAIN, FH>;
+    void (*k)(FieldFwdH3Args);
+    if constexpr (FOLD) k = field_fwd_h3_fold_kernel<MODE, ENC, W, NTR, FH>;
+    else k = field_fwd_h3_kernel<MODE, ENC, W, NTR, TRAIN, FH>;
     hipError_t e = hipFuncSetAttribute((const void*)k, hipFuncAttributeMaxDynamicSharedMemorySize, (int)lds);
     if (e != hipSuccess) return (int)e;
     int dev = 0, cus = 256;
@@ -449,7 +478,10 @@
 #define NEFES_TU_PART 0
 #endif
 enum { H3_EXT_SIGMA = 0, H3_EXT_FULL, H3_SIGMA, H3_FULL, H3_TRAIN_STATIC, H3_TRAIN_FULL, H3_STATIC, H3_HG_SIGMA, H3_HG_FULL, H3_FH_FULL,
-       H3_TRAIN_EXT_STATIC, H3_TRAIN_EXT_FULL };
+       H3_TRAIN_EXT_STATIC, H3_TRAIN_EXT_FULL,
+       H3_FOLD = 0x100  };
+#define NEFES_H3_FOLDED(fold, MODE, ENC, W, NTR, FH) \
+    ((fold) ? launch_h3<MODE, ENC, W, NTR, false, FH, true>(a, st) : launch_h3<MODE, ENC, W, NTR, false, FH>(a, st))
 int nefes_fwd_h3_launch_part1(int which, const FieldFwdH3Args& a, hipStream_t st);
 int nefes_fwd_h3_launch_part2(int which, const FieldFwdH3Args& a, hipStream_t st);
 int nefes_fwd_h3_launch_part3(int which, const FieldFwdH3Args& a, hipStream_t st);
@@ -462,21 +494,23 @@
 
 #if NEFES_TU_PART == 1
 int nefes_fwd_h3_launch_part1(int which, const FieldFwdH3Args& a, hipStream_t st) {
-    switch (which) {
+    const bool fold = (which & H3_FOLD) != 0;
+    switch (which & ~H3_FOLD) {
         case H3_EXT_SIGMA: return launch_h3<NEFES_FIELD_SIGMA, NEFES_XYZ_EXTERNAL32>(a, st);
-        case H3_EXT_FULL: return launch_h3<NEFES_FIELD_FULL, NEFES_XYZ_EXTERNAL32>(a, st);
-        case H3_STATIC: return launch_h3<NEFES_FIELD_STATIC, NEFES_XYZ_FREQ10, 256, 1>(a, st);
+        case H3_EXT_FULL: return NEFES_H3_FOLDED(fold, NEFES_FIELD_FULL, NEFES_XYZ_EXTERNAL32, 256, 1, false);
+        case H3_STATIC: return NEFES_H3_FOLDED(fold, NEFES_FIELD_STATIC, NEFES_XYZ_FREQ10, 256, 1, false);
         case H3_HG_SIGMA: return launch_h3<NEFES_FIELD_SIGMA, NEFES_XYZ_HASHGRID_FUSED>(a, st);
-        case H3_HG_FULL: return launch_h3<NEFES_FIELD_FULL, NEFES_XYZ_HASHGRID_FUSED>(a, st);
+        case H3_HG_FULL: return NEFES_H3_FOLDED(fold, NEFES_FIELD_FULL, NEFES_XYZ_HASHGRID_FUSED, 256, 1, false);
     }
     return NEFES_E_UNSUPPORTED;
 }
 #elif NEFES_TU_PART == 2
 int nefes_fwd_h3_launch_part2(int which, const FieldFwdH3Args& a, hipStream_t st) {
-    switch (which) {
+    const bool fold = (which & H3_FOLD) != 0;
+    switch (which & ~H3_FOLD) {
         case H3_SIGMA: return launch_h3<NEFES_FIELD_SIGMA, NEFES_XYZ_FREQ10, 128, 5>(a, st);
-        case H3_FULL: return launch_h3<NEFES_FIELD_FULL, NEFES_XYZ_FREQ10, 128, 5>(a, st);
-        case H3_STATIC: return launch_h3<NEFES_FIELD_STATIC, NEFES_XYZ_FREQ10, 128, 5>(a, st);
+        case H3_FULL: return NEFES_H3_FOLDED(fold, NEFES_FIELD_FULL, NEFES_XYZ_FREQ10, 128, 5, false);
+        case H3_STATIC: return NEFES_H3_FOLDED(fold, NEFES_FIELD_STATIC, NEFES_XYZ_FREQ10, 128, 5, false);
     }
     return NEFES_E_UNSUPPORTED;
 }
@@ -500,15 +534,19 @@
 }
 #elif NEFES_TU_PART == 5
 int nefes_fwd_h3_launch_part5(int which, const FieldFwdH3Args& a, hipStream_t st) {
-    if (which == H3_FULL) return launch_h3<NEFES_FIELD_FULL, NEFES_XYZ_FREQ10, 256, 5>(a, st);
-    if (which == H3_STATIC) return launch_h3<NEFES_FIELD_STATIC, NEFES_XYZ_FREQ10, 256, 5>(a, st);
+    const bool fold = (which & H3_FOLD) != 0;
+    which &= ~H3_FOLD;
+    if (which == H3_FULL) return NEFES_H3_FOLDED(fold, NEFES_FIELD_FULL, NEFES_XYZ_FREQ10, 256, 5, false);
+    if (which == H3_STATIC) return NEFES_H3_FOLDED(fold, NEFES_FIELD_STATIC, NEFES_XYZ_FREQ10, 256, 5, false);
     return NEFES_E_UNSUPPORTED;
 }
 #elif NEFES_TU_PART == 6
 int nefes_fwd_h3_launch_part6(int which, const FieldFwdH3Args& a, hipStream_t st) {
-    if (which == H3_FULL) return launch_h3<NEFES_FIELD_FULL, NEFES_XYZ_FREQ10, 128, 1>(a, st);
-    if (which == H3_STATIC) return launch_h3<NEFES_FIELD_STATIC, NEFES_XYZ_FREQ10, 128, 1>(a, st);
-    if (which == H3_FH_FULL) return launch_h3<NEFES_FIELD_FULL, NEFES_XYZ_FREQ10, 128, 1, false, true>(a, st);
+    const bool fold = (which & H3_FOLD) != 0;
+    which &= ~H3_FOLD;
+    if (which == H3_FULL) return NEFES_H3_FOLDED(fold, NEFES_FIELD_FULL, NEFES_XYZ_FREQ10, 128, 1, false);
+    if (which == H3_STATIC) return NEFES_H3_FOLDED(fold, NEFES_FIELD_STATIC, NEFES_XYZ_FREQ10, 128, 1, false);
+    if (which == H3_FH_FULL) return NEFES_H3_FOLDED(fold, NEFES_FIELD_FULL, NEFES_XYZ_FREQ10, 128, 1, true);
     return NEFES_E_UNSUPPORTED;
 }
 #elif NEFES_TU_PART == 7
@@ -535,6 +573,7 @@
     if (!desc || !packed || !raw_t || !acts || !viewdirs || N <= 0 || S <= 0) return NEFES_E_BADARG;
     if (!pts && !(rays_o && rays_d && z)) return NEFES_E_BADARG;
     if (mode != NEFES_FIELD_STATIC && mode != NEFES_FIELD_FULL) return NEFES_E_UNSUPPORTED;
+    if (desc->fold_final) return NEFES_E_UNSUPPORTED;
     if (mode == NEFES_FIELD_FULL && !desc->has_transient) return NEFES_E_BADARG;
     const int cls = nefes_head_class(desc->feat_dim);
     if ((desc->width != 256 && desc->width != 128) || cls < 0 || desc->xyz_encoding != NEFES_XYZ_FREQ10) return NEFES_E_UNSUPPORTED;
@@ -566,6 +605,7 @@
                                             const float* viewdirs, float* raw_t, float* acts, uint32_t* masks, void* stream) {
     if (!desc || !packed || !xyz_enc || !raw_t || !acts || !viewdirs || N <= 0 || S <= 0) return NEFES_E_BADARG;
     if (mode != NEFES_FIELD_STATIC && mode != NEFES_FIELD_FULL) return NEFES_E_UNSUPPORTED;
+    if (desc->fold_final) return NEFES_E_UNSUPPORTED;
     if (mode == NEFES_FIELD_FULL && !desc->has_transient) return NEFES_E_BADARG;
     if (desc->width != 256 || nefes_head_class(desc->feat_dim) != 0 || desc->xyz_encoding != NEFES_XYZ_EXTERNAL32) return NEFES_E_UNSUPPORTED;
     NefesBlobInfo info;
@@ -635,19 +675,21 @@
     a.n_tiles = (int)((a.M + 127) / 128);
     magic_div((uint32_t)S, a.s_magic, a.s_shift);
     hipStream_t st = (hipStream_t)stream;
-    if (fh) return nefes_fwd_h3_launch_part6(H3_FH_FULL, a, st);
+    const int F = (desc->fold_final && mode != NEFES_FIELD_SIGMA) ? H3_FOLD : 0;
+    if (fh) return nefes_fwd_h3_launch_part6(H3_FH_FULL | F, a, st);
     if (mode == NEFES_FIELD_STATIC) {
-        if (big) return cls == 0 ? nefes_fwd_h3_launch_part1(H3_STATIC, a, st) : nefes_fwd_h3_launch_part5(H3_STATIC, a, st);
-        return cls == 1 ? nefes_fwd_h3_launch_part2(H3_STATIC, a, st) : nefes_fwd_h3_launch_part6(H3_STATIC, a, st);
-    }
-    if (fused_grid) return nefes_fwd_h3_launch_part1(mode == NEFES_FIELD_SIGMA ? H3_HG_SIGMA : H3_HG_FULL, a, st);
-    if (ext) return nefes_fwd_h3_launch_part1(mode == NEFES_FIELD_SIGMA ? H3_EXT_SIGMA : H3_EXT_FULL, a, st);
+        if (big) return cls == 0 ? nefes_fwd_h3_launch_part1(H3_STATIC | F, a, st) : nefes_fwd_h3_launch_part5(H3_STATIC | F, a, st);
+        return cls == 1 ? nefes_fwd_h3_launch_part2(H3_STATIC | F, a, st) : nefes_fwd_h3_launch_part6(H3_STATIC | F, a, st);
+    }
+    if (fused_grid) return nefes_fwd_h3_launch_part1(mode == NEFES_FIELD_SIGMA ? H3_HG_SIGMA : (H3_HG_FULL | F), a, st);
+    if (ext) return nefes_fwd_h3_launch_part1(mode == NEFES_FIELD_SIGMA ? H3_EXT_SIGMA : (H3_EXT_FULL | F), a, st);
     if (small) {
         if (mode == NEFES_FIELD_SIGMA) return nefes_fwd_h3_launch_part2(H3_SIGMA, a, st);
-        return cls == 1 ? nefes_fwd_h3_launch_part2(H3_FULL, a, st) : nefes_fwd_h3_launch_part6(H3_FULL, a, st);
+        return cls == 1 ? nefes_fwd_h3_launch_part2(H3_FULL | F, a, st) : nefes_fwd_h3_launch_part6(H3_FULL | F, a, st);
     }
     if (mode == NEFES_FIELD_SIGMA) return launch_h3<NEFES_FIELD_SIGMA, NEFES_XYZ_FREQ10>(a, st);
-    return cls == 0 ? launch_h3<NEFES_FIELD_FULL, NEFES_XYZ_FREQ10>(a, st) : nefes_fwd_h3_launch_part5(H3_FULL, a, st);
+    if (cls != 0) return nefes_fwd_h3_launch_part5(H3_FULL | F, a, st);
+    return NEFES_H3_FOLDED(F != 0, NEFES_FIELD_FULL, NEFES_XYZ_FREQ10, 256, 1, false);
 }
 
 extern "C" int nefes_field_fwd_h3(const NefesNetDesc* desc, const void* packed, int mode, int N, int S, const float* rays_o,
diff --git a/nefes_amd/csrc/layout.h b/nefes_amd/csrc/layout.h
--- a/nefes_amd/csrc/layout.h
+++ b/nefes_amd/csrc/layout.h
@@ -79,7 +79,11 @@
        NEFES_H3B_N };
 #define NEFES_H3F_N_STATIC (NEFES_H3F_RGB + 1)
 #define NEFES_H3B_N_STATIC (NEFES_H3B_N - 4)
-NEFES_HD int nefes_h3b_seg(int has_transient, int seg) { return (has_transient || seg == NEFES_H3B_RGB) ? seg : seg - 4; }
+NEFES_HD int nefes_h3b_seg(int has_transient, int seg, int folded = 0) {
+    return ((has_transient || seg == NEFES_H3B_RGB) ? seg : seg - 4) - ((folded && seg > NEFES_H3B_FINAL) ? 1 : 0);
+}
+NEFES_HD int nefes_h3f_seg(int seg, int folded) { return seg - ((folded && seg > NEFES_H3F_FINAL) ? 1 : 0); }
+NEFES_HD int nefes_h3bb_block(int block, int folded) { return block - ((folded && block > NEFES_H3BB_FINAL) ? 1 : 0); }
 
 NEFES_HD int nefes_mask_words(int W) { return 8 * (W / 64) + 4 * (W / 128); }
 
diff --git a/nefes_amd/csrc/pack.cpp b/nefes_amd/csrc/pack.cpp
--- a/nefes_amd/csrc/pack.cpp
+++ b/nefes_amd/csrc/pack.cpp
@@ -176,6 +176,7 @@
 struct Net {
     int W, W2, C, NTW, NTH, NTR;
     bool transient;
+    bool fold;
     bool ext;
     int in_xyz, e_steps;
     const float* const* t;
@@ -244,9 +245,11 @@
 
 void add_static_head_h3(const Net& n, Stream& st) {
     const int W = n.W, W2 = n.W2;
-    st.segs.push_back(seg(n.NTW, W / 2, k_natural(W / 2, 0), rows_natural(n.NTW, W), n.w(L_FINAL), W));
-    mark(st.segs.back(), 2);
-    st.bias.push_back({n.b(L_FINAL), rows_natural(n.NTW, W)});
+    if (!n.fold) {
+        st.segs.push_back(seg(n.NTW, W / 2, k_natural(W / 2, 0), rows_natural(n.NTW, W), n.w(L_FINAL), W));
+        mark(st.segs.back(), 2);
+        st.bias.push_back({n.b(L_FINAL), rows_natural(n.NTW, W)});
+    }
     st.segs.push_back(seg(n.NTH, W / 2, k_natural(W / 2, 0), rows_natural(n.NTH, W2), n.w(L_DIR), W + 27));
     mark(st.segs.back(), 2);
     st.segs.push_back(seg(n.NTH, 16, k_emb(4, 16, W), rows_natural(n.NTH, W2), n.w(L_DIR), W + 27));
@@ -259,9 +262,11 @@
 
 void add_heads_x6(const Net& n, Stream& st, int kind = 1) {
     const int W = n.W, W2 = n.W2;
-    st.segs.push_back(seg(n.NTW, W / 2, k_natural(W / 2, 0), rows_natural(n.NTW, W), n.w(L_FINAL), W));
-    mark(st.segs.back(), kind);
-    st.bias.push_back({n.b(L_FINAL), rows_natural(n.NTW, W)});
+    if (!n.fold) {
+        st.segs.push_back(seg(n.NTW, W / 2, k_natural(W / 2, 0), rows_natural(n.NTW, W), n.w(L_FINAL), W));
+        mark(st.segs.back(), kind);
+        st.bias.push_back({n.b(L_FINAL), rows_natural(n.NTW, W)});
+    }
     st.segs.push_back(seg(2 * n.NTH, W / 2, k_natural(W / 2, 0), rows_natural(2 * n.NTH, 2 * W2), n.dt_w.data(), W + 27));
     mark(st.segs.back(), kind);
     st.segs.push_back(seg(2 * n.NTH, 16, k_emb(4, 16, W), rows_natural(2 * n.NTH, 2 * W2), n.dt_w.data(), W + 27));
@@ -321,8 +326,10 @@
     }
     st.segs.push_back(seg(NTW + 1, W2 / 2, k_natural(W2 / 2, 0), rows_fd, n.w(L_DIR), W + 27, true));
     mark(st.segs.back(), x6);
-    st.segs.push_back(seg(NTW, W / 2, k_natural(W / 2, 0), rows_natural(NTW, W), n.w(L_FINAL), W, true));
-    mark(st.segs.back(), x6);
+    if (!n.fold) {
+        st.segs.push_back(seg(NTW, W / 2, k_natural(W / 2, 0), rows_natural(NTW, W), n.w(L_FINAL), W, true));
+        mark(st.segs.back(), x6);
+    }
     st.segs.push_back(seg(NTW, 1, k_compact(1, 1), rows_natural(NTW, W), n.w(L_SIGMA), W, true));
     for (int l = 7; l >= 0; --l) {
         if (l == 4) {
@@ -394,6 +401,7 @@
     n.NTW = n.W / 32; n.NTH = n.W2 / 32; n.NTR = nefes_head_ntr(n.C);
     n.transient = d->has_transient != 0;
     n.ext = d->xyz_encoding == NEFES_XYZ_EXTERNAL32;
+    n.fold = d->fold_final != 0;
     if (d->xyz_encoding != NEFES_XYZ_FREQ10 && !n.ext) return false;
     n.in_xyz = n.ext ? 32 : 63;
     n.e_steps = n.ext ? NEFES_X_STEPS : NEFES_E_STEPS;
@@ -417,6 +425,9 @@
     }
     static const float* dummy[36] = {nullptr};
     if (!tensors) n.t = dummy;
+    const bool h3_shape = !n.ext || (n.W == 256 && nefes_head_class(n.C) == 0);
+    if (n.fold && !h3_shape) return false;
+    if (!n.fold) {
     add_trunk(n, st[NEFES_STREAM_FWD_SIGMA]);
     add_trunk(n, st[NEFES_STREAM_FWD_STATIC]);
     add_static_head(n, st[NEFES_STREAM_FWD_STATIC]);
@@ -428,12 +439,12 @@
         add_backward(n, st[NEFES_STREAM_BWD_FULL]);
     }
     const bool big = n.W == 256, small = n.W == 128 && n.C == 128 && !n.ext;
-    const bool h3_shape = !n.ext || (n.W == 256 && nefes_head_class(n.C) == 0);
     if (big || small) add_trunk(n, st[NEFES_STREAM_FWD_SIGMA_X6], 1);
     if (n.transient && (big || small) && (small || n.C == 16)) {
         add_trunk(n, st[NEFES_STREAM_FWD_FULL_X6], 1);
         add_heads_x6(n, st[NEFES_STREAM_FWD_FULL_X6]);
         add_backward(n, st[NEFES_STREAM_BWD_FULL_X6], 1);
+    }
     }
     if (h3_shape) {
         add_trunk(n, st[NEFES_STREAM_FWD_SIGMA_H3], 2);
@@ -678,6 +689,7 @@
 
 extern "C" int nefes_pack_map(const NefesNetDesc* desc, uint32_t* map, size_t n_entries, int64_t* tensor_elems_out) {
     if (!desc || !map) return NEFES_E_BADARG;
+    if (desc->fold_final) return NEFES_E_UNSUPPORTED;
     Indexed x;
     const int rc = build_indexed(desc, x, tensor_elems_out);
     if (rc) return rc;
@@ -688,6 +700,7 @@
 
 extern "C" int nefes_pack_h3_plan(const NefesNetDesc* desc, int32_t* plan, size_t n_ints, size_t* needed) {
     if (!desc) return NEFES_E_BADARG;
+    if (desc->fold_final) return NEFES_E_UNSUPPORTED;
     Indexed x;
     const int rc = build_indexed(desc, x, nullptr);
     if (rc) return rc;
diff --git a/nefes_amd/field.py b/nefes_amd/field.py
--- a/nefes_amd/field.py
+++ b/nefes_amd/field.py
@@ -228,23 +228,48 @@
             self._pk_key = key
         return self._pk
 
+    def _frozen(self):
+        return not any(p.requires_grad for n, p in self.named_parameters() if not n.startswith(("fusion_net", "exposure_embedding")))
+
+    def fold_final_ok(self):
+        return ops.FOLD_FINAL and ops.SPLIT == "h3" and ops.USE_X6 and self._supported() and self._frozen()
+
+    def packed_folded(self) -> ops.PackedField:
+        names = ops.PackedField.LAYERS_FINE if self.encode_transient else ops.PackedField.LAYERS_COARSE
+        sd = dict(self.named_parameters())
+        prm = [sd[n + s] for n in names for s in (".weight", ".bias")]
+        key = tuple((p.data_ptr(), p._version, str(p.device)) for p in prm)
+        if getattr(self, "_pk_fold", None) is None or key != self._pk_fold_key:
+            dev = prm[0].device if prm[0].is_cuda else torch.device("cuda")
+            enc = L.XYZ_EXTERNAL32 if self.in_channels_xyz == 32 else L.XYZ_FREQ10
+            ksd = ops.fold_final_state(self._kernel_params({n: p.detach() for n, p in sd.items()}), self.W, self.encode_transient)
+            self._pk_fold = ops.PackedField(ksd, self.W, self.W_features, self.encode_transient, dev, enc, fold_final=True)
+            self._pk_fold_key = key
+        return self._pk_fold
+
+    def packed_for(self, mode, n_samples=0) -> ops.PackedField:
+        if mode != L.FIELD_SIGMA and n_samples < (1 << 31) - 256 and self.fold_final_ok():
+            return self.packed_folded()
+        return self.packed()
+
     def factored_head_ok(self):
         return (ops.FACTORED_HEAD and self.encode_transient and self.W == 128 and self.in_channels_xyz != 32 and self._supported()
-                and 3 + self.W_features > 3 + self.W // 2 + 1 and ops.SPLIT == "h3"
-                and not any(p.requires_grad for n, p in self.named_parameters()
-                            if not n.startswith(("fusion_net", "exposure_embedding"))))
+                and 3 + self.W_features > 3 + self.W // 2 + 1 and ops.SPLIT == "h3" and self._frozen())
 
     def packed_fh(self):
         names = ops.PackedField.LAYERS_FINE
         sd = dict(self.named_parameters())
         prm = [sd[n + s] for n in names for s in (".weight", ".bias")]
-        key = tuple((p.data_ptr(), p._version, str(p.device)) for p in prm)
+        fold = self.fold_final_ok()
+        key = tuple((p.data_ptr(), p._version, str(p.device)) for p in prm) + (fold,)
         if getattr(self, "_pk_fh", None) is None or key != self._pk_fh_key:
             dev = prm[0].device if prm[0].is_cuda else torch.device("cuda")
             ksd = dict(self._kernel_params({n: p.detach() for n, p in sd.items()}))
             w, b = ksd["static_rgb.0.weight"], ksd["static_rgb.0.bias"]
             ksd["static_rgb.0.weight"], ksd["static_rgb.0.bias"] = w[:3].contiguous(), b[:3].contiguous()
-            pk = ops.PackedField(ksd, self.W, 0, True, dev, L.XYZ_FREQ10)
+            if fold:
+                ksd = ops.fold_final_state(ksd, self.W, True)
+            pk = ops.PackedField(ksd, self.W, 0, True, dev, L.XYZ_FREQ10, fold_final=fold)
             w_f = w[3:].to(dev, torch.float32).contiguous()
             self._pk_fh = (pk, w_f, w_f.t().contiguous(), b[3:].to(dev, torch.float32).contiguous())
             self._pk_fh_key = key
@@ -295,13 +320,13 @@
 
 def run_network_NeRFH_NFF(inputs, viewdirs, ts, fn, embed_fn=None, embeddirs_fn=None, typ='coarse', output_transient=False,
                           netchunk=1024 * 64, test_time=False, store_rgb=False):
-    pk = fn.packed()
     if typ == 'coarse' and test_time:
         mode = L.FIELD_SIGMA
     elif typ == 'coarse' or not output_transient:
         mode = L.FIELD_STATIC
     else:
         mode = L.FIELD_FULL
+    pk = fn.packed_for(mode, inputs.shape[0] * inputs.shape[1])
     dev = pk.blob.device
     raw_t = ops.FieldFromPoints.apply(inputs.to(dev), None if viewdirs is None else viewdirs.to(dev), pk, mode)
     return raw_t.permute(0, 2, 1)
diff --git a/nefes_amd/lib.py b/nefes_amd/lib.py
--- a/nefes_amd/lib.py
+++ b/nefes_amd/lib.py
@@ -8,7 +8,8 @@
 
 
 class NefesNetDesc(C.Structure):
-    _fields_ = [("width", C.c_int32), ("feat_dim", C.c_int32), ("has_transient", C.c_int32), ("xyz_encoding", C.c_int32)]
+    _fields_ = [("width", C.c_int32), ("feat_dim", C.c_int32), ("has_transient", C.c_int32), ("xyz_encoding", C.c_int32),
+                ("fold_final", C.c_int32)]
 
 
 class NefesStreamInfo(C.Structure):
@@ -25,7 +26,7 @@
                 ("base_resolution", C.c_int32), ("per_level_scale", C.c_float), ("bound", C.c_float)]
 
 
-ABI_VERSION = 15
+ABI_VERSION = 16
 STREAM_FWD_SIGMA, STREAM_FWD_STATIC, STREAM_FWD_FULL, STREAM_BWD_FULL, STREAM_FWD_SIGMA_X6, STREAM_FWD_FULL_X6, STREAM_BWD_FULL_X6, STREAM_BWD_STATIC = 0, 1, 2, 3, 4, 5, 6, 7
 STREAM_FWD_SIGMA_H3, STREAM_FWD_FULL_H3, STREAM_BWD_FULL_H3, STREAM_FWD_STATIC_H3, STREAM_BWD_STATIC_H3 = 8, 9, 10, 11, 12
 FIELD_SIGMA, FIELD_STATIC, FIELD_FULL = 0, 1, 2
diff --git a/nefes_amd/ops.py b/nefes_amd/ops.py
--- a/nefes_amd/ops.py
+++ b/nefes_amd/ops.py
@@ -225,9 +225,10 @@
     LAYERS_FINE = LAYERS_COARSE + ["transient_encoding.0", "transient_encoding.2", "transient_encoding.4",
                                    "transient_sigma.0", "transient_rgb.0", "transient_beta.0"]
 
-    def __init__(self, state_dict, width, feat_dim, has_transient, device, xyz_encoding=0):
+    def __init__(self, state_dict, width, feat_dim, has_transient, device, xyz_encoding=0, fold_final=False):
         lib = L.load()
-        self.desc = L.NefesNetDesc(int(width), int(feat_dim), 1 if has_transient else 0, int(xyz_encoding))
+        self.desc = L.NefesNetDesc(int(width), int(feat_dim), 1 if has_transient else 0, int(xyz_encoding), 1 if fold_final else 0)
+        self.fold_final = bool(fold_final)
         self.xyz_encoding = int(xyz_encoding)
         self.width, self.feat_dim, self.has_transient = int(width), int(feat_dim), bool(has_transient)
         info = L.NefesBlobInfo()
@@ -249,6 +250,8 @@
 
     def repack(self, params):
         lib = L.load()
+        if self.fold_final:
+            raise RuntimeError("nefes_amd: a network packed with xyz_encoding_final folded is frozen; it is re-packed from its state dict")
         if self._map is None:
             n = self.info.total_bytes // 2
             host_map = torch.zeros(n, dtype=torch.int32)
@@ -297,9 +300,23 @@
         return 1 if mode == L.FIELD_SIGMA else (3 + self.feat_dim + (1 if mode == L.FIELD_STATIC else 6))
 
 
+def fold_final_state(state_dict, width, has_transient):
+    out = dict(state_dict)
+    wf = state_dict["xyz_encoding_final.weight"].detach().double().cpu()
+    bf = state_dict["xyz_encoding_final.bias"].detach().double().cpu()
+    for name in ("dir_encoding.0",) + (("transient_encoding.0",) if has_transient else ()):
+        w = state_dict[name + ".weight"].detach().double().cpu()
+        b = state_dict[name + ".bias"].detach().double().cpu()
+        out[name + ".weight"] = torch.cat([w[:, :width] @ wf, w[:, width:]], 1).float().contiguous()
+        out[name + ".bias"] = (b + w[:, :width] @ bf).float().contiguous()
+    return out
+
+
 def field_fwd(pk: PackedField, mode, N, S, rays_o=None, rays_d=None, z=None, pts=None, viewdirs=None, want_masks=False,
               xyz_enc=None):
     dev = pk.blob.device
+    if pk.fold_final:
+        raise RuntimeError("nefes_amd: a network packed with xyz_encoding_final folded runs on the fp16 two-part instances only")
     if not canonical_shape(pk):
         raise RuntimeError(f"nefes_amd: the {('sigma', 'static', 'full')[mode]} forward of W={pk.width}, f_dim={pk.feat_dim} was routed to "
                            f"the fp32-MFMA instances (NEFES_SPLIT={SPLIT}; or a frozen network's static head with test_time=False), "
@@ -320,6 +337,7 @@
 REPACK_H3 = os.environ.get("NEFES_REPACK_H3", "1") != "0"
 USE_X6 = os.environ.get("NEFES_X6", "1") != "0"
 FUSED_COARSE = os.environ.get("NEFES_FUSED_COARSE", "1") != "0"
+FOLD_FINAL = os.environ.get("NEFES_FOLD_FINAL", "1") != "0"
 
 
 HEAD_MAX_C = 141
@@ -372,6 +390,7 @@
     raw_t = torch.empty(N, pk.n_raw(mode), S, device=dev)
     masks = torch.empty(pk.mask_bytes(N * S) // 4, dtype=torch.int32, device=dev) if want_masks else None
     h3 = _h3(pk) and h3_shape(pk) and N * S < (1 << 31) - 256
+    _tap("fold_final", pk.fold_final)
     if mode == L.FIELD_STATIC and not h3:
         return field_fwd(pk, mode, N, S, rays_o=rays_o, rays_d=rays_d, z=z, pts=pts, viewdirs=viewdirs, want_masks=want_masks, xyz_enc=xyz_enc)
     if not h3 and not canonical_shape(pk):
@@ -521,6 +540,7 @@
                                                    _chk(masks, "masks", torch.int32), _stream()), "nefes_field_fwd_h3_fh")
         if masks is not None:
             _tap("masks", (masks, N, S, pk.width, L.FIELD_FULL))
+            _tap("fold_final", pk.fold_final)
         ctx.pk, ctx.have, ctx.pk_gen = pk, need, pk.generation
         if need:
             ctx.save_for_backward(rays_o, rays_d, viewdirs, z, raw_t, masks)
@@ -560,6 +580,7 @@
                                                    _chk(masks, "masks", torch.int32), _stream()), "nefes_field_fwd_h3_fh")
         if masks is not None:
             _tap("masks", (masks, N, S, pk.width, L.FIELD_FULL))
+            _tap("fold_final", pk.fold_final)
         rgb, gmap, disp, acc, _, _, _ = composite_fwd(raw_t, z, Cg + 1, flags, beta_min)
         if emit_gmap:
             feat = gmap
@@ -810,6 +831,7 @@
                     "nefes_field_fwd_h3_hashgrid")
         if masks is not None:
             _tap("masks", (masks, N, S, pk.width, mode))
+            _tap("fold_final", pk.fold_final)
         ctx.pk, ctx.grid, ctx.have, ctx.pk_gen = pk, grid, need, pk.generation
         if need:
             ctx.save_for_backward(rays_o, rays_d, viewdirs, z, raw_t, masks)
diff --git a/nefes_amd/render.py b/nefes_amd/render.py
--- a/nefes_amd/render.py
+++ b/nefes_amd/render.py
@@ -98,7 +98,7 @@
             if cfg.xyz_encoder is not None:
                 return T.field_train_encoded(net, mode, cfg.xyz_encoder, rays_o, rays_d, viewdirs, z_)
             return T.field_train(net, mode, rays_o, rays_d, viewdirs, z_)
-        return _field(pk, mode, rays_o, rays_d, viewdirs, z_, cfg.xyz_encoder)
+        return _field(net.packed_for(mode, z_.shape[0] * z_.shape[1]), mode, rays_o, rays_d, viewdirs, z_, cfg.xyz_encoder)
 
     pk_c = network_fn.packed()
     C = pk_c.feat_dim
```
